# humansensinglab/AGenDA

Measured on AMD Instinct MI355X. Metric: 512x512 images/sec + DAAM heatmaps, 50 DDIM steps, SD-1.5, higher is better.
Workload: dtype bf16

## Files before the change

### agenda_amd/_lib.py

```python
from __future__ import annotations

import ctypes as C
import os

_HERE = os.path.dirname(os.path.abspath(__file__))
LIB_PATH = os.environ.get("AGD_LIB") or os.path.join(_HERE, "libagenda_hip.so")
AGD_MAX_LEVELS = 8
AGD_N_CLASSES = 11


class AgdConfig(C.Structure):
    _fields_ = [
        ("struct_size", C.c_int),
        ("in_channels", C.c_int), ("out_channels", C.c_int), ("n_levels", C.c_int),
        ("block_out_channels", C.c_int * AGD_MAX_LEVELS),
        ("down_cross", C.c_int * AGD_MAX_LEVELS),
        ("num_heads", C.c_int * AGD_MAX_LEVELS),
        ("layers_per_block", C.c_int), ("cross_attention_dim", C.c_int),
        ("use_linear_projection", C.c_int), ("norm_num_groups", C.c_int),
        ("vae_latent_channels", C.c_int), ("vae_out_channels", C.c_int), ("vae_n_levels", C.c_int),
        ("vae_block_out_channels", C.c_int * AGD_MAX_LEVELS),
        ("vae_layers_per_block", C.c_int), ("vae_norm_num_groups", C.c_int),
        ("vae_scaling_factor", C.c_float),
        ("max_tokens", C.c_int),
# ... 135 lines not shown
    "agd_cfg_ddim_step": (C.c_int, [_P, _P, _P, C.c_int, C.c_int, C.c_float, C.c_float, C.c_float, _P]),
    "agd_denoise": (C.c_int, [_P, _P, C.c_int, C.c_int, C.c_int, C.POINTER(C.c_float), C.POINTER(C.c_float),
                              C.POINTER(C.c_float), C.c_float, _P]),
    "agd_denoise_plms": (C.c_int, [_P, _P, C.c_int, C.c_int, C.c_int, C.POINTER(C.c_float), C.POINTER(C.c_float),
                                   C.POINTER(C.c_float), C.c_float, _P]),
    "agd_denoise_dpm": (C.c_int, [_P, _P, C.c_int, C.c_int, C.c_int, C.POINTER(C.c_float), C.POINTER(C.c_float), C.c_float, _P]),
    "agd_vae_decode": (C.c_int, [_P, _P, C.c_int, C.c_int, _P, _P, _P]),
    "agd_vae_encode": (C.c_int, [_P, _P, C.c_int, C.c_int, _P, _P, _P]),
    "agd_safety_scores_hw": (C.c_int, [_P, _P, C.c_int, C.c_int, C.c_int, _P, _P, _P]),
    "agd_controlnet_set_cond_hw": (C.c_int, [_P, _P, C.c_int, C.c_int, C.c_int, C.c_int, _P]),
    "agd_controlnet_residuals_hw": (C.c_int, [_P, _P, C.c_int, C.c_int, C.c_int, C.c_float, C.c_float, C.c_int, _P, C.POINTER(C.c_longlong), _P]),
    "agd_inpaint_prepare_hw": (C.c_int, [_P, _P, C.c_int, _P, C.c_int, C.c_int, C.c_int, C.c_int, _P, _P, _P, _P]),
    "agd_inpaint_set_hw": (C.c_int, [_P, _P, C.c_int, _P, C.c_int, _P, C.c_int, C.c_int, C.c_int, _P]),
    "agd_unet_forward_hw": (C.c_int, [_P, _P, C.c_int, C.c_int, C.c_int, C.c_float, _P, _P]),
    "agd_unet_forward_ts_hw": (C.c_int, [_P, _P, C.c_int, C.c_int, C.c_int, C.POINTER(C.c_float), _P, _P]),
    "agd_cfg_ddim_step_hw": (C.c_int, [_P, _P, _P, C.c_int, C.c_int, C.c_int, C.c_float, C.c_float, C.c_float, _P]),
    "agd_denoise_hw": (C.c_int, [_P, _P, C.c_int, C.c_int, C.c_int, C.c_int, C.POINTER(C.c_float), C.POINTER(C.c_float),
                                 C.POINTER(C.c_float), C.c_float, _P]),
    "agd_denoise_plms_hw": (C.c_int, [_P, _P, C.c_int, C.c_int, C.c_int, C.c_int, C.POINTER(C.c_float), C.POINTER(C.c_float),
                                      C.POINTER(C.c_float), C.c_float, _P]),
    "agd_denoise_dpm_hw": (C.c_int, [_P, _P, C.c_int, C.c_int, C.c_int, C.c_int, C.POINTER(C.c_float), C.POINTER(C.c_float), C.c_float, _P]),
    "agd_vae_decode_hw": (C.c_int, [_P, _P, C.c_int, C.c_int, C.c_int, _P, _P, _P]),
    "agd_vae_encode_hw": (C.c_int, [_P, _P, C.c_int, C.c_int, C.c_int, _P, _P, _P]),
    "agd_record_reset_hw": (C.c_int, [_P, C.c_int, C.c_int, C.c_int, _P]),
    "agd_set_option": (C.c_int, [_P, C.c_char_p, C.c_int]),
    "agd_record_config": (C.c_int, [_P, C.c_int, C.c_int, C.c_int]),
    "agd_record_reset": (C.c_int, [_P, C.c_int, C.c_int, _P]),
    "agd_daam_global": (C.c_int, [_P, C.c_int, C.c_int, _P, _P]),
    "agd_hook_global": (C.c_int, [_P, _P, _P]),
    "agd_hook_count": (C.c_int, [_P]),
    "agd_hook_last_map": (C.c_int, [_P, _P, C.c_int, _P]),
    "agd_cross_attn": (C.c_int, [_P, C.c_char_p, _P, _P, C.c_int, C.c_int, C.c_int, _P, C.c_int, _P]),
    "agd_attn_processor": (C.c_int, [_P, C.c_char_p, _P, _P, _P, C.c_int, C.c_int, C.c_int, _P, C.c_int, _P]),
    "agd_hook_reset": (C.c_int, [_P, C.c_int, C.c_int, _P]),
    "agd_hook_num_maps": (C.c_int, [_P]),
    "agd_hook_map_dims": (C.c_int, [_P, C.c_int, C.POINTER(C.c_int)]),
    "agd_hook_map": (C.c_int, [_P, C.c_int, _P, _P]),
    "agd_op_attn_reg_loss": (C.c_int, [_P, C.c_int, C.c_int, C.c_int, _P, _P, _P, C.c_float, _P, _P, _P]),
    "agd_attn_processor_backward": (C.c_int, [_P, C.c_char_p, _P, _P, _P, _P, C.c_int, C.c_int, C.c_int, C.c_int, _P, _P, _P]),
    "agd_op_conv2d": (C.c_int, [_P, _P, _P, _P] + [C.c_int] * 9 + [_P]),
    "agd_op_conv2d_ex": (C.c_int, [_P, _P, _P, _P] + [C.c_int] * 10 + [_P]),
    "agd_op_linear": (C.c_int, [_P, _P, _P, _P, _P, C.c_int, C.c_int, C.c_int, C.c_int, _P]),
    "agd_op_groupnorm": (C.c_int, [_P, _P, _P, _P, C.c_int, C.c_int, C.c_int, C.c_int, C.c_float, C.c_int, _P]),
    "agd_op_groupnorm_ex": (C.c_int, [_P] * 5 + [C.c_int] * 5 + [C.c_float, C.c_int, _P, C.c_int, _P, C.c_int, C.POINTER(C.c_int), _P]),
    "agd_op_gn_fold": (C.c_int, [_P, _P] + [C.c_int] * 5 + [C.c_float] + [_P] * 4 + [C.c_int, C.c_int] + [_P] * 5 + [_P]),
    "agd_op_conv_groupnorm": (C.c_int, [_P] * 6 + [C.c_int] * 6 + [C.c_float, C.c_int, C.c_int, _P]),
    "agd_op_igemm": (C.c_int, [C.POINTER(AgdIgemmDesc), _P]),
    "agd_op_layernorm": (C.c_int, [_P, _P, _P, _P, C.c_int, C.c_int, C.c_float, _P]),
    "agd_op_layernorm_ex": (C.c_int, [_P, _P, _P, _P, C.c_int, C.c_int, C.c_float, C.POINTER(C.c_int), _P]),
    "agd_op_ff_fused": (C.c_int, [_P] * 8 + [C.c_int, C.c_int, C.c_float, _P]),
    "agd_op_attn_chain": (C.c_int, [_P] * 9 + [C.c_int] * 5 + [C.c_float, _P]),
    "agd_op_ff_fused_ex": (C.c_int, [_P] * 8 + [C.c_int, C.c_int, C.c_float, _P, _P, _P, C.c_int, _P, C.c_int, _P, C.c_int, _P]),
    "agd_op_attn_chain_ex": (C.c_int, [_P] * 8 + [C.c_int] * 5 + [C.c_float] + [_P] * 4 + [C.c_int, _P, _P] + [C.c_int] * 6 + [_P]),
    "agd_op_qkv_chain": (C.c_int, [_P] * 3 + [C.c_int, C.c_float, _P, C.c_int] + [_P] * 4 + [C.c_float] + [_P] * 3 + [C.c_int] * 4 + [_P]),
    "agd_op_xattn_premul": (C.c_int, [_P] * 9 + [C.c_int] * 5 + [C.c_float, _P]),
    "agd_op_attention": (C.c_int, [_P, _P, _P, _P, C.c_int, C.c_int, C.c_int, C.c_int, C.c_int, C.c_float, _P, _P]),
    "agd_op_attention_ex": (C.c_int, [_P, _P, _P, _P] + [C.c_int] * 5 + [C.c_float, C.c_int, _P, _P, _P, C.c_int, C.c_int, _P, C.c_int, C.c_int, C.c_int, _P]),
    "agd_op_attention_long": (C.c_int, [_P, _P, _P, _P] + [C.c_int] * 5 + [C.c_float, C.c_int, _P, C.c_int, C.c_int, _P]),
    "agd_op_attention_headsum": (C.c_int, [_P, _P, _P, _P, C.c_int, C.c_int, C.c_int, C.c_int, C.c_int, C.c_float, _P, _P]),
    "agd_op_attention_backward": (C.c_int, [_P, _P, _P, _P] + [C.c_int] * 6 + [C.c_float, _P, _P, _P]),
    "agd_op_hook_headmean": (C.c_int, [_P, C.c_int, C.c_int, C.c_int, C.c_int, _P, _P]),
    "agd_op_bicubic_clamp_mean": (C.c_int, [_P, C.c_int, C.c_int, C.c_int, C.c_int, _P, _P]),
    "agd_op_heatmap_u8": (C.c_int, [_P, C.c_int, C.c_int, _P, _P]),
    "agd_op_resize_u8_pil": (C.c_int, [_P, C.c_int, C.c_int, C.c_int, C.c_int, C.c_int, C.c_int, _P, _P]),
    "agd_op_stack_heatmaps": (C.c_int, [_P, _P, _P, C.c_longlong, _P, _P, _P]),
    "agd_op_window_gather": (C.c_int, [_P, _P] + [C.c_int] * 8 + [_P]),
    "agd_op_window_mean": (C.c_int, [_P, _P] + [C.c_int] * 6 + [_P]),
    "agd_denoise_panorama": (C.c_int, [_P, _P] + [C.c_int] * 7 + [C.POINTER(C.c_float)] * 3 + [C.c_float, _P]),
    "agd_daam_global_panorama": (C.c_int, [_P, C.c_int, C.c_int, _P, _P]),
    "agd_op_region_masks": (C.c_int, [_P, C.c_int, C.c_int, _P] + [C.c_int] * 6 + [_P]),
    "agd_op_region_spread": (C.c_int, [_P] * 5 + [C.c_int] * 6 + [C.POINTER(C.c_int), C.c_float, C.c_float, _P]),
    "agd_op_region_mean": (C.c_int, [_P, _P, _P] + [C.c_int] * 5 + [_P]),
    "agd_denoise_regions": (C.c_int, [_P, _P, C.c_int, C.c_int, C.c_int, C.POINTER(AgdRegionsDesc), C.c_int] + [C.POINTER(C.c_float)] * 3 + [C.c_float, _P]),
    "agd_freeu_set": (C.c_int, [_P] + [C.c_float] * 4),
    "agd_freeu_clear": (C.c_int, [_P]),
    "agd_freeu_counts": (C.c_int, [_P, C.POINTER(C.c_longlong)]),
    "agd_op_freeu": (C.c_int, [_P, _P, _P, _P] + [C.c_int] * 5 + [C.c_float, C.c_float, _P]),
    "agd_guidance_rescale_set": (C.c_int, [_P, C.c_float]),
    "agd_guidance_rescale_clear": (C.c_int, [_P]),
    "agd_guidance_rescale_counts": (C.c_int, [_P, C.POINTER(C.c_longlong)]),
    "agd_op_guidance_rescale": (C.c_int, [_P, _P] + [C.c_int] * 4 + [C.c_float, C.c_float, _P, _P]),
    "agd_pag_set": (C.c_int, [_P, C.POINTER(C.c_float), C.c_int, C.POINTER(C.c_char_p), C.c_int]),
    "agd_pag_clear": (C.c_int, [_P]),
    "agd_pag_counts": (C.c_int, [_P, C.POINTER(C.c_longlong), C.POINTER(C.c_longlong)]),
    "agd_op_pag_v_rows": (C.c_int, [_P, _P, _P, C.c_int, C.c_int, _P]),
    "agd_op_pag_fold": (C.c_int, [_P, _P, C.c_longlong, C.c_float, _P]),
    "agd_sega_set": (C.c_int, [_P, C.POINTER(AgdSegaDesc)]),
    "agd_sega_clear": (C.c_int, [_P]),
    "agd_sega_counts": (C.c_int, [_P, C.POINTER(C.c_longlong), C.POINTER(C.c_longlong)]),
    "agd_op_sega_threshold": (C.c_int, [_P, _P, C.c_int, C.c_int, C.c_int, C.POINTER(C.c_float), C.POINTER(C.c_double), _P, _P]),
    "agd_op_sega_fold": (C.c_int, [_P, _P, _P, _P, C.c_int, C.c_int, C.c_int, C.POINTER(C.c_float), C.POINTER(C.c_float), C.POINTER(C.c_float),
                                   C.c_float, C.c_float, C.c_float, _P]),
    "agd_deepcache_set": (C.c_int, [_P, C.POINTER(C.c_int), C.c_int, C.c_int]),
    "agd_deepcache_clear": (C.c_int, [_P]),
    "agd_deepcache_counts": (C.c_int, [_P, C.POINTER(C.c_longlong)]),
    "agd_deepcache_forward_hw": (C.c_int, [_P, _P, C.c_int, C.c_int, C.c_int, C.c_float, C.c_int, C.c_int, _P, _P]),
    "agd_op_deepcache_capture": (C.c_int, [_P, _P, _P, C.c_longlong, _P, _P, C.c_longlong, _P]),
    "agd_profile_begin": (C.c_int, [_P]),
    "agd_profile_end": (C.c_int, [_P, C.POINTER(C.c_double), C.POINTER(C.c_double), C.POINTER(C.c_longlong)]),
    "agd_profile_end_ex": (C.c_int, [_P, C.c_double, C.c_double] + [C.POINTER(C.c_double)] * 5 + [C.POINTER(C.c_longlong)]),
    "agd_profile_class_name": (C.c_char_p, [C.c_int]),
    "agd_version": (C.c_char_p, []),
}

EXPORTS = tuple(_SIGS.keys())
_lib = None
# ... 36 lines not shown
```

### agenda_amd/csrc/kernels.h

```cpp
#pragma once
#include "common.h"
#include "../../include/agenda_hip.h"

#define AGD_MAX_DEVICES 16
struct SplitKWs { float* p = nullptr; size_t cap = 0; };

struct IgemmP {
  const bf16_t* sc0 = nullptr; const bf16_t* sc1 = nullptr; int sc_C0 = 0, sc_C1 = 0;
  int ups4 = 0;
  const bf16_t* src0; const bf16_t* src1;
  int C0, C1;
  int Hin, Win, Hout, Wout;
  int ksize, stride, pad, up;
  const bf16_t* W;
  const float* bias; int bias_mode;
  const float* rowadd; int rowadd_ld;
  const bf16_t* residual; int ldr;
  void* out; int out_f32; int ldo;
  int M, N, K;
  float alpha;
  int geglu;
  int act;
  int batch;
  long long sA0, sA1, sW, sO, sR;
// ... 20 lines not shown
  int pc;
  int stagger;
  int dbg;
  int* ran;
};
enum { IGEMM_RAN_NONE = 0, IGEMM_RAN_GENERAL = 1, IGEMM_RAN_HALO = 2, IGEMM_RAN_PCH = 3, IGEMM_RAN_PC = 4, IGEMM_RAN_8P = 5, IGEMM_RAN_SMAP = 6, IGEMM_RAN_WREG = 7 };
enum { IGEMM_SLAB_NONE = 0, IGEMM_SLAB_PLAIN = 1, IGEMM_SLAB_GN = 2 };
int launch_igemm(const IgemmP& p, hipStream_t st);
int igemm_query(const IgemmP& p, int* cfg3);

struct AttnP {
  const bf16_t* q; const bf16_t* k; const bf16_t* v; bf16_t* o;
  int ldq, ldk, ldv, ldo;
  long long sq, sk, sv, so;
  int B, H, D, Nq, Nk;
  float scale;
  int record_mode; int rec_b0;
  float* rec; long long rec_img_stride; long long rec_head_stride;
  int rec_T;
  int rec_hpb;
  int nqt;
  int causal;
  const float* mask;
  const bf16_t* k2; const bf16_t* v2; int ldk2, ldv2; long long sk2, sv2; int Nk2;
};
int launch_attention(const AttnP& p, hipStream_t st);
constexpr int ATTN_LONG_MAX_KEYS = 320;
int launch_attention_long(const AttnP& p, hipStream_t st);

struct FFusedP {
  const bf16_t* h; bf16_t* out;
  const bf16_t* w1f;
  const float* cs1; const float* b1;
  const bf16_t* w2f;
  const float* b2;
  int M; float ln_eps;
  const bf16_t* wpf; const float* bp; const bf16_t* xres; bf16_t* pout; float* colstat;
  int xres_rows;
  int premul;
};
int launch_ff_fused(const FFusedP& p, int C, hipStream_t st);
struct AttnChainP {
  const bf16_t* h; bf16_t* out;
  const float* gamma; const float* beta; float ln_eps;
  const bf16_t* wqf;
  const bf16_t* wof; const float* bo;
  const bf16_t* kv; int ldkv; long long skv;
  int M, HW, T; float scale;
  int record; float* rec; long long rec_img_stride, rec_head_stride; int rec_T, rec_b0, rec_hpb;
  float* rowstat_out;
  const bf16_t* o1; const bf16_t* wo1f; const float* bo1;
  int rows32;
  int src_rows;
};
int launch_attn_chain(const AttnChainP& p, int C, int heads, hipStream_t st);
struct QkvChainP {
  const bf16_t* x;
  const bf16_t* wbf; long long wb_stride; const float* rowadd;
  bf16_t* h;
  const float* gamma; const float* beta; float ln_eps;
  const bf16_t* wqkvf;
  bf16_t* qkv;
  int M, HW;
  long long rowadd_stride;
  const float* gn_part; int gn_bm, gn_groups; float gn_eps; const float* gn_gamma; const float* gn_beta;
  int rows64;
  int sched2;
};
int launch_qkv_chain(const QkvChainP& p, int C, hipStream_t st);
int launch_frag_order_w1(const bf16_t* src, bf16_t* dst, int C, int HID, hipStream_t st);
int launch_frag_order_w(const bf16_t* src, bf16_t* dst, int N, int K, int NI, int KC, hipStream_t st);

#define XATTN_TP 80
struct XattnPremulP {
  const bf16_t* kv; int ldkv; long long skv;
  const bf16_t* wqT;
  const bf16_t* wo;
  const float* gamma; const float* wqb;
  int B, T, C, H; float scale;
  bf16_t* kpp; float* kcs; float* kbs; bf16_t* vpp;
};
int launch_xattn_premul(const XattnPremulP& p, hipStream_t st);
struct XattnSP {
  const bf16_t* x;
  const float* ln_stats; int ln_slots; float ln_invC, ln_eps;
  const bf16_t* kpp; const float* kcs; const float* kbs;
  bf16_t* P;
  int M, HW, C, H, T;
  float* rec; long long rec_img_stride, rec_head_stride; int rec_T, rec_b0;
};
int launch_xattn_s(const XattnSP& p, hipStream_t st);
int launch_matvec_bf16(const bf16_t* W, const float* v, float* out, int N, int K, hipStream_t st);
int launch_rowstat_bf16(const bf16_t* x, float* out, int M, int C, hipStream_t st);

struct GroupNormP {
  const bf16_t* x0; const bf16_t* x1; int C0, C1;
  bf16_t* y;
  const float* gamma; const float* beta;
  int B, HW, groups; float eps; int silu;
  float* ws;
  const float* part0; const float* part1; int bm0, bm1;
  int* path;
};
int groupnorm_check(int B, int C0, int C1, int HW, int groups);
int layernorm_check(int rows, int C);
int launch_groupnorm(const GroupNormP& p, hipStream_t st);
int launch_gn_fold_weight(const float* part, int bm, int B, int HW, int C, int groups, float eps, const float* gamma, const float* beta,
                          const bf16_t* W, const float* bias, int N, bf16_t* Wb, float* rowadd, hipStream_t st, int frag_ni = 0);
// ... 129 lines not shown
```

### agenda_amd/csrc/model.hip

```cpp
#include "../../include/agenda_hip.h"
#include "kernels.h"

#include <algorithm>
#include <cmath>
#include <cstdarg>
#include <cstdio>
#include <cstring>
#include <functional>
#include <string>
#include <unordered_map>
#include <unordered_set>
#include <vector>

static thread_local char g_err[2048] = "";
#define AGD_API extern "C" __attribute__((visibility("default")))
extern "C" void agd_set_error(const char* fmt, ...) {
  va_list ap; va_start(ap, fmt); vsnprintf(g_err, sizeof(g_err), fmt, ap); va_end(ap);
}
#define CK(expr) do { if ((expr) != 0) return -1; } while (0)
#define FAIL(...) do { agd_set_error(__VA_ARGS__); return -1; } while (0)

struct WMat { bf16_t* w = nullptr; int N = 0, Cin = 0, Cpad = 0, taps = 0;
              int sc_cols = 0;
              bf16_t* wfrag = nullptr; int wfrag_ni = 0; };
struct Act { bf16_t* p = nullptr; int B = 0, H = 0, W = 0, C = 0; float* cpart = nullptr; int cpart_bm = 0;
             bf16_t* normed = nullptr; const float* normed_gamma = nullptr;
             long long n() const { return (long long)B * H * W * C; } };
struct NextGn { const float* gamma = nullptr; const float* beta = nullptr; float eps = 0.f; int silu = 0; };

struct Arena {
  char* base = nullptr; size_t cap = 0, off = 0, peak = 0;
  void* alloc(size_t bytes) {
    size_t a = (off + 255) & ~(size_t)255;
    if (a + bytes > cap) { agd_set_error("activation arena exhausted: need %zu + %zu > %zu bytes (raise workspace_bytes)", a, bytes, cap); return nullptr; }
    off = a + bytes; if (off > peak) peak = off;
    return base + a;
  }
  size_t mark() const { return off; }
  void release(size_t m) { off = m; }
};

enum { PC_CONV3 = 0, PC_GEMM, PC_ATTN_SELF, PC_ATTN_CROSS, PC_GN, PC_LN, PC_ELEM, PC_HEAT, PC_VAE_ATTN, PC_OTHER, PC_TOUCH };
static const char* kClassNames[AGD_N_CLASSES] = {"igemm_conv3x3", "igemm_linear_1x1", "attn_self_flash", "attn_cross_daam",
                                                 "groupnorm", "layernorm", "elementwise", "heatmap", "vae_attn_softmax", "other", "weight_touch"};

struct DBuf {
  void* p = nullptr; size_t cap = 0;
  template <typename T> T* as() const { return (T*)p; }
  int ensure(size_t bytes) {
    if (p && bytes <= cap) return 0;
    if (p) { (void)hipDeviceSynchronize(); (void)hipFree(p); p = nullptr; cap = 0; }
    const size_t want = bytes ? bytes : 256;
    if (hipMalloc(&p, want) != hipSuccess) { p = nullptr; agd_set_error("hipMalloc(%zu) failed", want); return -1; }
    cap = want;
    return 0;
  }
  void release() { if (p) (void)hipFree(p); p = nullptr; cap = 0; }
};

struct XLayer {
  std::string name; int C = 0, heads = 0, level = 0; bool mid = false;
  bool cn = false;
  WMat wkv; DBuf kvb; bf16_t* kv = nullptr; DBuf accb; float* acc = nullptr; int acc_h = 0, acc_w = 0;
  int acc_heads = 0;
  DBuf wqTb, wkvTb, woTb; WMat wqT, wkvT, woT;
  bf16_t* pm_wqT = nullptr; float* pm_wqb = nullptr; bool pm_ready = false;
  DBuf pm_kppb, pm_vppb, pm_csb; bf16_t* pm_kpp = nullptr; bf16_t* pm_vpp = nullptr; float* pm_kcs = nullptr; float* pm_kbs = nullptr;
};

struct Fuser {
  std::string pre; int C = 0, heads = 0;
  WMat wqkv, wkv; float ta = 0.f, td = 0.f; float* bo_s = nullptr; float* b2_s = nullptr;
  DBuf gkvb;
};

struct IpaLayer {
  std::string pre; int C = 0, heads = 0, cols = 0;
  DBuf wk, wv, kppb, vppb, csbsb;
};

enum : int {
  TBF_FF            = 1 << 0,
  TBF_ATTN2         = 1 << 1,
  TBF_ATTN1_OUT     = 1 << 2,
  TBF_FF_PROJ       = 1 << 3,
  TBF_QKV           = 1 << 4,
  TBF_ATTN2_640     = 1 << 5,
  TBF_LAZY_DUP      = 1 << 6,
  TBF_QKV_GN        = 1 << 7,
  TBF_QKV_640       = 1 << 8,
  TBF_FF_PREMUL     = 1 << 9,
  TBF_ATTN2_ROWS32  = 1 << 10,
  TBF_QKV_ROWS64    = 1 << 11,
  TBF_QKV_SCHED2    = 1 << 12,
  TBF_DEFAULT       = 0x1fff & ~TBF_QKV_640,
};

struct ProfEv { int cls; double flops, bytes; hipEvent_t a, b; };

struct EvalCond {
  float cn_scale = 0.f;
  bool grounded = false;
  float ad_scale = 0.f;
  bool ipa = false;
  bool pag = false;
  int dc = 0;
  int dc_branch = 0;
};
enum : int { DC_CAPTURE = 1, DC_SHALLOW = 2 };

struct agd_ctx {
  int device = 0; agd_config cfg{}; std::string err;
  std::unordered_map<std::string, WMat> W;
  std::unordered_map<std::string, float*> V;
  std::unordered_map<std::string, int> Vn;
  std::vector<void*> owned;
  Arena arena; bf16_t* zero_page = nullptr;
  float* stage = nullptr; size_t stage_bytes = 0;
  bool finalized = false;
  WMat tproj_all; float* tproj_bias = nullptr; float* tproj_out = nullptr; int tproj_total = 0;
  const float* tproj_cur = nullptr;
  int tproj_cur_ld = 0;
  float* tsteps_buf = nullptr; int tsteps_cap = 0;
  std::unordered_map<std::string, int> tproj_off;
  float* temb_buf = nullptr;
  float* t_dev = nullptr;
  std::vector<XLayer> xl; std::unordered_map<std::string, int> xl_idx;
  DBuf ctxb; bf16_t* ctx_bf16 = nullptr; int ctx_B2 = 0, ctx_T = 0;
  int rec_mode = 0, rec_is_train = 0, rec_T_cfg = 0, rec_T = 0, rec_B = 0, rec_L = 0, rec_Lh = 0, rec_Lw = 0;
  DBuf hook_sumb, hook_scratchb, hook_headsb, hook_storeb;
  struct HookRec { size_t off; int Bp, T, N; };
  std::vector<HookRec> hook_recs; size_t hook_store_used = 0;
  DBuf bwd_wsb;
  float* hook_sum = nullptr; float* hook_scratch = nullptr; int hook_count = 0, hook_Bp = 0, hook_T = 0;
  int rec_base = 0, rec_call = 0;
  int pano_B = 0, pano_Lh = 0, pano_Lw = 0, pano_stride = 0;
  DBuf pano_ctxb;
  DBuf reg_xb;
  DBuf pano_viewb, pano_hmb;
  DBuf latb, epsb, vae_imgb, plmsb, dpmb;
  bf16_t* lat_bf16 = nullptr; float* eps_nhwc = nullptr;
  SplitKWs splitk;
  int opt_cfg_share = 1;
  int opt_ln_fold = 1;
  int opt_gn_fused = 1;
  int opt_warm = 3;
  int opt_gn_proj_fold = 1;
  int opt_p8 = 1;
// ... 402 lines not shown
  if (B != c->gl_B2) FAIL("gligen: the grounding objects are set for %d rows, this forward has %d (agd_gligen_set)", c->gl_B2, B);
  const std::string t = f.pre + "transformer_blocks.0.fuser.";
  bf16_t* n = (bf16_t*)c->arena.alloc((size_t)M * C * 2); bf16_t* ff = (bf16_t*)c->arena.alloc((size_t)M * 4 * C * 2);
  if (!n || !ff) return -1;
  GETV(g1, t + "norm1.weight"); GETV(b1, t + "norm1.bias"); GETV(g2, t + "norm2.weight"); GETV(b2, t + "norm2.bias");
  GETW(wo, t + "attn.to_out.0.weight"); GETW(w1, t + "ff.net.0.proj.weight"); GETV(bb1, t + "ff.net.0.proj.bias"); GETW(w2, t + "ff.net.2.weight");
  { ProfScope ps(c, st, PC_LN, 0, 4.0 * M * (double)C); CK(launch_layernorm(h, n, g1, b1, M, C, 1e-5f, st)); }
  { GemmOpt o; CK(run_conv(c, st, n, C, nullptr, 0, 1, 1, M, f.wqkv, 1, qkv, o, c->zero_page)); }
  AttnP a{}; a.q = qkv; a.k = qkv + C; a.v = qkv + 2 * C; a.o = att;
  a.ldq = a.ldk = a.ldv = 3 * C; a.ldo = C; a.sq = a.sk = a.sv = (long long)HW * 3 * C; a.so = (long long)HW * C;
  a.B = B; a.H = f.heads; a.D = D; a.Nq = HW; a.Nk = HW; a.scale = 1.0f / sqrtf((float)D);
  a.k2 = f.gkvb.as<bf16_t>(); a.v2 = a.k2 + C; a.ldk2 = a.ldv2 = 2 * C; a.sk2 = a.sv2 = (long long)NO * 2 * C; a.Nk2 = NO;
  { const double fl = 4.0 * B * f.heads * (double)HW * (HW + NO) * D, by = 2.0 * B * (double)C * (4.0 * HW + 2.0 * NO);
    ProfScope ps(c, st, PC_ATTN_SELF, fl, by); CK(launch_attention(a, st)); }
  { GemmOpt o; o.bias = f.bo_s; o.alpha = f.ta; o.residual = h; CK(run_conv(c, st, att, C, nullptr, 0, 1, 1, M, *wo, 1, h, o, c->zero_page)); }
  { ProfScope ps(c, st, PC_LN, 0, 4.0 * M * (double)C); CK(launch_layernorm(h, n, g2, b2, M, C, 1e-5f, st)); }
  { GemmOpt o; o.bias = bb1; o.geglu = 1; CK(run_conv(c, st, n, C, nullptr, 0, 1, 1, M, *w1, 1, ff, o, c->zero_page)); }
  GemmOpt o; o.bias = f.b2_s; o.alpha = f.td; o.residual = h;
  return last(ff, 4 * C, *w2, o);
}

static int dup_half(agd_ctx* c, hipStream_t st, bf16_t* p, long long half_elems) {
  ProfScope ps(c, st, PC_ELEM, 0);
  if (hipMemcpyAsync(p + half_elems, p, (size_t)half_elems * 2, hipMemcpyDeviceToDevice, st) != hipSuccess) FAIL("dup_half copy failed");
  return 0;
}

enum TbHead  { HEAD_GN,
               HEAD_FOLD,
               HEAD_QKV,
               HEAD_QKV_GN };
enum TbDup   { DUP_NONE, DUP_COPY,
               DUP_LAZY };
enum TbAttn2 { ATTN2_CHAIN,
               ATTN2_PREMUL,
               ATTN2_KERNELS };
enum TbFf    { FF_FUSED,
               FF_FUSED_PROJ,
               FF_FUSED_PREMUL,
               FF_FFPROJ,
               FF_PLAIN };

struct TBlockPlan {
  bool fold;
  bool x_normed;
  bool gfold;
  TbHead head; int qkv_rows64, qkv_sched2;
  bool attn1_in_chain;
  TbDup dup;
  const Fuser* fuser;
  const IpaLayer* ipa;
  XLayer* xl;
  TbAttn2 attn2; int chain_rows32;
  bool daam;
  TbFf ff;
  bool wreg_proj;
  bool stats_head, stats_attn1, stats_attn2;
  bool stats_ipa;
};

static const float kTbLnEps = 1e-5f;

struct TBlock {
  agd_ctx* c; hipStream_t st; const std::string& pre; const std::string t; const Act& x; Act& out; int heads, groups;
  int C, HW, Bs, B;
  const float* gn_g = nullptr; const float* gn_b = nullptr; const WMat* w_in = nullptr; const float* b_in = nullptr;
  bf16_t* ln = nullptr;
  bf16_t* h = nullptr; bf16_t* qkv = nullptr; bf16_t* att = nullptr;
  const bf16_t* xres;
  int M; const int Mshared;
  float* stats = nullptr; int slots = 0;
  bf16_t* ipaP = nullptr;
  TBlock(agd_ctx* c_, hipStream_t st_, const std::string& pre_, const Act& x_, Act& out_, int heads_, int groups_, int dup)
    : c(c_), st(st_), pre(pre_), t(pre_ + "transformer_blocks.0."), x(x_), out(out_), heads(heads_), groups(groups_), C(x_.C), HW(x_.H * x_.W),
      Bs(x_.B), B(dup ? 2 * x_.B : x_.B), xres(x_.p), M(x_.B * x_.H * x_.W), Mshared(M) {}

  int produce(const bf16_t* A, int K, const WMat& w, GemmOpt o, bool shaped, bool want_stats) {
    const int gb_ = shaped ? M / HW : 1, gh_ = shaped ? x.H : 1, gw_ = shaped ? x.W : M;
    stats = nullptr; slots = 0;
    if (want_stats) {
      int cfg[3] = {0, 0, 0}; GemmOpt qo = o; qo.query_cfg = cfg; qo.want_rowstat = 1;
      CK(run_conv(c, st, A, K, nullptr, 0, gb_, gh_, gw_, w, 1, h, qo, c->zero_page));
      slots = (w.N + cfg[1] - 1) / cfg[1];
      stats = (float*)c->arena.alloc((size_t)B * HW * slots * 2 * sizeof(float)); if (!stats) return -1;
      o.rowstat_out = stats; o.rowstat_slots = slots;
    }
    return run_conv(c, st, A, K, nullptr, 0, gb_, gh_, gw_, w, 1, h, o, c->zero_page);
  }
  int consume(bool fold, const std::string& lnkey, const std::string& wkey, const float* bias, int geglu, bf16_t* outp) {
    if (fold) {
      const std::string k = wkey + ".lnfold";
      GETW(wf, k); GETV(cs, k + ".cs"); GETV(bf, k + ".bias");
      GemmOpt o; o.bias = bf; o.geglu = geglu; o.ln_stats = stats; o.ln_slots = slots; o.ln_cs = cs; o.ln_invC = 1.0f / (float)C; o.ln_eps = kTbLnEps;
      if (geglu && C == 1280 && M >= 1024 && M <= 4096 && (c->opt_wreg & 1) && wf->wfrag) o.wreg = 2;
      return run_conv(c, st, h, C, nullptr, 0, 1, 1, M, *wf, 1, outp, o, c->zero_page);
    }
    GETV(g, lnkey + ".weight"); GETV(b, lnkey + ".bias");
    { ProfScope ps(c, st, PC_LN, 0, 4.0 * M * (double)C); CK(launch_layernorm(h, ln, g, b, M, C, kTbLnEps, st)); }
    GETW(w, wkey); GemmOpt o; o.bias = bias; o.geglu = geglu;
    return run_conv(c, st, ln, C, nullptr, 0, 1, 1, M, *w, 1, outp, o, c->zero_page);
  }
};

static TBlockPlan tblock_plan(const TBlock& s, int dup) {
  agd_ctx* c = s.c; const Act& x = s.x; const std::string& pre = s.pre; const std::string& t = s.t;
  const int C = s.C, HW = s.HW, heads = s.heads, groups = s.groups;
  auto tb = [c](int bit) { return (c->opt_tb_fuse & bit) != 0; };
  auto has = [c](const std::string& key) { return c->W.count(key) != 0; };
  TBlockPlan p{};
  p.fold = c->opt_ln_fold == 1 || (c->opt_ln_fold == 2 && C <= 320) || (c->opt_ln_fold == 3 && C <= 640);
  p.x_normed = x.normed && x.normed_gamma == s.gn_g;
  p.wreg_proj = C == 640 && (c->opt_wreg & 2);
  const bool sums = c->opt_gn_fused && x.cpart && x.cpart_bm > 0 && HW % x.cpart_bm == 0;
  p.gfold = c->opt_gn_proj_fold && sums && C <= (c->opt_gn_proj_fold >= 2 ? 640 : 320) && HW % 128 == 0;
  if (p.gfold) {
    const bool qkv = tb(TBF_QKV) && C == 320 && s.w_in->N == C && has(t + "attn1.qkv.frag");
    const bool gn_inside = qkv && tb(TBF_QKV_GN) && groups <= 32 && has(pre + "proj_in.frag");
    p.head = gn_inside ? HEAD_QKV_GN : qkv ? HEAD_QKV : HEAD_FOLD;
    p.qkv_rows64 = qkv && tb(TBF_QKV_ROWS64) && HW % 64 == 0;
  } else if (C == 640 && tb(TBF_QKV) && tb(TBF_QKV_640) && tb(TBF_QKV_GN) && sums && HW % 64 == 0 && groups <= 32 && !p.x_normed && !dup &&
             has(pre + "proj_in.frag") && has(t + "attn1.qkv.frag")) {
    p.head = HEAD_QKV_GN;
  } else p.head = HEAD_GN;
  p.qkv_sched2 = tb(TBF_QKV_SCHED2);
  const bool ff_fused = tb(TBF_FF) && p.fold && C == 320 && has(t + "ff.w1.frag");
  if (ff_fused) {
    const bool proj = tb(TBF_FF_PROJ) && has(pre + "proj_out.frag");
    p.ff = !proj ? FF_FUSED : tb(TBF_FF_PREMUL) && has(t + "ff.w2p.frag") ? FF_FUSED_PREMUL : FF_FUSED_PROJ;
  } else p.ff = c->opt_ffproj && has(pre + "ffproj.weight") ? FF_FFPROJ : FF_PLAIN;
  auto itx = c->xl_idx.find(t + "attn2");
  p.xl = itx == c->xl_idx.end() ? nullptr : &c->xl[itx->second];
  p.daam = p.xl && daam_records(c, *p.xl, s.B, x.H, x.W);
  const bool premul = p.xl && p.xl->pm_ready && c->opt_xpre && p.fold && HW % 64 == 0 && c->rec_mode != 2 && c->ctx_T <= XATTN_TP && !dup &&
                      (!p.daam || p.xl->acc_heads == p.xl->heads);
  const bool chain = !premul && tb(TBF_ATTN2) && (C == 320 || (C == 640 && tb(TBF_ATTN2_640))) && heads == 8 && HW % (C == 320 ? 128 : 64) == 0 &&
                     c->ctx_T <= 96 && c->rec_mode != 2 && has(t + "attn2.to_q.frag");
  p.attn2 = premul ? ATTN2_PREMUL : chain ? ATTN2_CHAIN : ATTN2_KERNELS;
  p.chain_rows32 = tb(TBF_ATTN2_ROWS32);
  if (c->cur.grounded) { auto itf = c->gl_idx.find(pre); if (itf != c->gl_idx.end()) p.fuser = &c->gl_f[itf->second]; }
  if (c->cur.ipa) { auto iti = c->ipa_idx.find(pre); if (iti != c->ipa_idx.end()) p.ipa = &c->ipa_l[iti->second]; }
  const bool lazy = dup && tb(TBF_LAZY_DUP) && chain && C == 320 && (p.ff == FF_FUSED_PROJ || p.ff == FF_FUSED_PREMUL) && !p.fuser && !p.ipa;
  p.dup = !dup ? DUP_NONE : lazy ? DUP_LAZY : DUP_COPY;
  p.attn1_in_chain = chain && tb(TBF_ATTN1_OUT) && p.dup != DUP_COPY && has(t + "attn1.to_out.frag") && !p.fuser && !p.ipa;
  p.stats_head = p.fold; p.stats_attn1 = p.fold && !chain; p.stats_attn2 = p.fold && !ff_fused && !p.ipa; p.stats_ipa = p.fold && !ff_fused && p.ipa;
  return p;
}

static int qkv_chain_params(const TBlock& s, const TBlockPlan& p, const bf16_t* wb, const float* radd, QkvChainP& qp) {
  agd_ctx* c = s.c; const Act& x = s.x; const int C = s.C;
  GETW(fqkv, s.t + "attn1.qkv.frag"); GETV(g1, s.t + "norm1.weight"); GETV(b1, s.t + "norm1.bias");
  qp.x = x.p; qp.wbf = wb; qp.wb_stride = (long long)s.w_in->N * C; qp.rowadd = radd; qp.rowadd_stride = C; qp.h = s.h; qp.gamma = g1; qp.beta = b1; qp.ln_eps = kTbLnEps;
  qp.wqkvf = fqkv->w; qp.qkv = s.qkv; qp.M = s.M; qp.HW = s.HW; qp.rows64 = p.qkv_rows64; qp.sched2 = p.qkv_sched2;
  if (p.head == HEAD_QKV_GN) {
    GETW(fpi, s.pre + "proj_in.frag");
    if (!s.b_in) FAIL("proj_in without bias");
    qp.wbf = fpi->w; qp.wb_stride = 0; qp.rowadd = s.b_in; qp.rowadd_stride = 0;
    qp.gn_part = x.cpart; qp.gn_bm = x.cpart_bm; qp.gn_groups = s.groups; qp.gn_eps = 1e-6f; qp.gn_gamma = s.gn_g; qp.gn_beta = s.gn_b;
  }
  return 0;
}

static int tb_head(TBlock& s, const TBlockPlan& p) {
  agd_ctx* c = s.c; hipStream_t st = s.st; const Act& x = s.x; const WMat* w = s.w_in; const int C = s.C;
  if (p.head == HEAD_GN) {
    if (p.x_normed) s.ln = x.normed;
    else CK(run_gn(c, st, x.p, C, nullptr, 0, s.Bs, s.HW, s.gn_g, s.gn_b, s.groups, 1e-6f, 0, s.ln, &x));
    GemmOpt o; o.bias = s.b_in;
    if (p.wreg_proj) o.wreg = 1;
    return s.produce(s.ln, C, *w, o, false, p.stats_head);
  }
  if (p.gfold) { if (w->taps != 1 || w->Cpad != C) FAIL("gn_proj_fold: proj_in weight [N=%d taps=%d Cpad=%d] is not a 1x1 over %d channels", w->N, w->taps, w->Cpad, C); }
  else if (w->taps != 1 || w->Cpad != C || w->N != C || !s.b_in) FAIL("qkv chain: proj_in weight [N=%d taps=%d Cpad=%d] is not a biased 1x1 over %d channels", w->N, w->taps, w->Cpad, C);
  bf16_t* wb = nullptr; float* radd = nullptr;
  if (p.head != HEAD_QKV_GN) {
    wb = (bf16_t*)c->arena.alloc((size_t)s.Bs * w->N * C * 2);
    radd = (float*)c->arena.alloc((size_t)s.Bs * w->N * sizeof(float));
    if (!wb || !radd) return -1;
    ProfScope ps(c, st, PC_GN, 0, 2.0 * s.Bs * (double)w->N * C * 2);
    CK(launch_gn_fold_weight(x.cpart, x.cpart_bm, s.Bs, s.HW, C, s.groups, 1e-6f, s.gn_g, s.gn_b, w->w, s.b_in, w->N, wb, radd, st, p.head == HEAD_QKV ? C / 64 : 0));
  }
  if (p.head == HEAD_FOLD) {
    WMat wi = *w; wi.w = wb;
    GemmOpt o; o.rowadd = radd; o.rowadd_ld = w->N; o.w_per_image = 1;
    return s.produce(x.p, C, wi, o, true, p.stats_head);
  }
  QkvChainP qp{}; CK(qkv_chain_params(s, p, wb, radd, qp));
  s.stats = nullptr; s.slots = 0;
  ProfScope ps(c, st, PC_GEMM, 8.0 * s.M * (double)C * C, 2.0 * s.M * (double)C * 5.0 + 2.0 * (p.gfold ? s.Bs + 3.0 : 4.0) * C * (double)C);
  return launch_qkv_chain(qp, C, st);
}

// ... 43 lines not shown
  const double M = (double)B * HW;
  ProfScope ps(c, st, PC_ATTN_CROSS, 2.0 * M * l.cols * l.C, 2.0 * M * l.C + 2.0 * B * (double)l.cols * l.C + 2.0 * M * l.cols);
  return launch_ipa_scores(sp, st);
}
static int ipa_add_rows(agd_ctx* c, hipStream_t st, const IpaLayer& l, bf16_t* h, int B, int HW, const bf16_t* P) {
  IpaAddP ap{}; ap.h = h; ap.P = P; ap.vpp = l.vppb.as<bf16_t>(); ap.B = B; ap.HW = HW; ap.C = l.C; ap.colsP = l.cols; ap.s = c->ipa_scale;
  const double M = (double)B * HW;
  ProfScope ps(c, st, PC_ATTN_CROSS, 2.0 * M * l.cols * l.C, 4.0 * M * l.C + 2.0 * B * (double)l.cols * l.C + 2.0 * M * l.cols);
  return launch_ipa_add(ap, st);
}
static int tb_ip_adapter_scores(TBlock& s, const TBlockPlan& p) {
  agd_ctx* c = s.c;
  if (s.C != p.ipa->C) FAIL("ip_adapter: %s has %d channels, its to_k_ip / to_v_ip were loaded for %d", s.pre.c_str(), s.C, p.ipa->C);
  s.ipaP = (bf16_t*)c->arena.alloc((size_t)s.M * p.ipa->cols * 2); if (!s.ipaP) return -1;
  CK(ipa_scores_rows(c, s.st, *p.ipa, s.h, s.B, s.HW, s.ipaP));
  c->ipa_counts[0]++;
  return 0;
}
static int tb_ip_adapter_add(TBlock& s, const TBlockPlan& p) {
  agd_ctx* c = s.c;
  CK(ipa_add_rows(c, s.st, *p.ipa, s.h, s.B, s.HW, s.ipaP));
  c->ipa_counts[1]++;
  if (p.stats_ipa) {
    s.slots = 1; s.stats = (float*)c->arena.alloc((size_t)s.M * 2 * sizeof(float)); if (!s.stats) return -1;
    ProfScope ps(c, s.st, PC_LN, 0, 2.0 * s.M * (double)s.C);
    CK(launch_rowstat_bf16(s.h, s.stats, s.M, s.C, s.st));
  }
  return 0;
}

static int tb_attn2_chain(TBlock& s, const TBlockPlan& p) {
  agd_ctx* c = s.c; const std::string& t = s.t; const XLayer& xl = *p.xl; const int C = s.C, HW = s.HW, B = s.B, M = s.M, heads = s.heads;
  GETW(fq, t + "attn2.to_q.frag"); GETW(fo, t + "attn2.to_out.frag");
  GETV(g2, t + "norm2.weight"); GETV(b2, t + "norm2.bias"); GETV(bo, t + "attn2.to_out.0.bias");
  const int T = c->ctx_T, D = C / heads;
  AttnChainP ap{}; ap.h = s.h; ap.out = s.h; ap.gamma = g2; ap.beta = b2; ap.ln_eps = kTbLnEps; ap.wqf = fq->w; ap.wof = fo->w; ap.bo = bo;
  ap.kv = xl.kv; ap.ldkv = 2 * C; ap.skv = (long long)T * 2 * C; ap.M = M; ap.HW = HW; ap.T = T; ap.scale = 1.0f / sqrtf((float)D);
  double rec_bytes = 0;
  if (p.daam) {
    ap.record = 1; ap.rec_b0 = B / 2; ap.rec_T = c->rec_T; ap.rec_hpb = heads / xl.acc_heads;
    ap.rec_head_stride = (long long)c->rec_T * HW; ap.rec_img_stride = ap.rec_head_stride * xl.acc_heads;
    ap.rec = xl.acc + (size_t)c->rec_base * ap.rec_img_stride;
    rec_bytes = 8.0 * (B - ap.rec_b0) * xl.acc_heads * (double)c->rec_T * HW;
  }
  if (p.attn1_in_chain || p.dup == DUP_LAZY) {
    ap.out = (bf16_t*)c->arena.alloc((size_t)M * C * 2); if (!ap.out) return -1;
  }
  if (p.attn1_in_chain) {
    GETW(f1o, t + "attn1.to_out.frag"); GETV(bo1, t + "attn1.to_out.0.bias");
    ap.o1 = s.att; ap.wo1f = f1o->w; ap.bo1 = bo1;
  }
  if (p.dup == DUP_LAZY) ap.src_rows = s.Mshared;
  ap.rows32 = p.chain_rows32;
  if (p.stats_attn2) {
    s.slots = 1; s.stats = (float*)c->arena.alloc((size_t)M * 2 * sizeof(float)); if (!s.stats) return -1;
    ap.rowstat_out = s.stats;
  }
  const double gemms = p.attn1_in_chain ? 6.0 : 4.0;
  ProfScope ps(c, s.st, PC_ATTN_CROSS, gemms * M * (double)C * C + 4.0 * B * heads * (double)HW * T * D, gemms * M * (double)C + gemms * C * (double)C + 4.0 * B * (double)T * C + rec_bytes);
  CK(launch_attn_chain(ap, C, heads, s.st));
  s.h = ap.out;
  return 0;
}

static int tb_attn2_premul(TBlock& s, const TBlockPlan& p) {
  agd_ctx* c = s.c; const XLayer& xl = *p.xl; const int C = s.C, HW = s.HW, B = s.B, M = s.M, heads = s.heads;
  if (!s.stats || s.slots <= 0) FAIL("attn2_premul: the GEMM in front of attn2 left no row statistics for norm2");
  GETV(bo, s.t + "attn2.to_out.0.bias");
  const int HT = heads * XATTN_TP;
  bf16_t* P = (bf16_t*)c->arena.alloc((size_t)M * HT * 2); if (!P) return -1;
  XattnSP sp{}; sp.x = s.h; sp.ln_stats = s.stats; sp.ln_slots = s.slots; sp.ln_invC = 1.0f / (float)C; sp.ln_eps = kTbLnEps;
  sp.kpp = xl.pm_kpp; sp.kcs = xl.pm_kcs; sp.kbs = xl.pm_kbs; sp.P = P; sp.M = M; sp.HW = HW; sp.C = C; sp.H = heads; sp.T = c->ctx_T;
  double rec_bytes = 0;
  if (p.daam) {
    sp.rec_b0 = B / 2; sp.rec_T = c->rec_T; sp.rec_head_stride = (long long)c->rec_T * HW; sp.rec_img_stride = sp.rec_head_stride * xl.acc_heads;
    sp.rec = xl.acc + (size_t)c->rec_base * sp.rec_img_stride;
    rec_bytes = 8.0 * (B - sp.rec_b0) * heads * (double)c->rec_T * HW;
  }
  { ProfScope ps(c, s.st, PC_ATTN_CROSS, 2.0 * M * (double)HT * C, 2.0 * M * (double)C + 2.0 * B * (double)HT * C + 2.0 * M * (double)HT + rec_bytes);
    CK(launch_xattn_s(sp, s.st)); }
  WMat wv; wv.w = xl.pm_vpp; wv.N = C; wv.Cin = HT; wv.Cpad = HT; wv.taps = 1;
  GemmOpt oo; oo.bias = bo; oo.residual = s.h; oo.w_per_image = 1;
  return s.produce(P, HT, wv, oo, true, p.stats_attn2);
}

static int tb_attn2(TBlock& s, const TBlockPlan& p) {
  agd_ctx* c = s.c; const std::string& t = s.t;
  if (!p.xl) FAIL("cross-attn layer %s not registered", (t + "attn2").c_str());
  if (c->ctx_B2 != s.B) FAIL("context batch %d != unet batch %d (call agd_set_context)", c->ctx_B2, s.B);
  if (p.attn2 == ATTN2_CHAIN) return tb_attn2_chain(s, p);
  if (p.attn2 == ATTN2_PREMUL) return tb_attn2_premul(s, p);
  CK(s.consume(p.fold, t + "norm2", t + "attn2.to_q.weight", nullptr, 0, s.qkv));
  CK(cross_attention(c, s.st, *p.xl, s.qkv, s.B, s.HW, s.x.H, s.x.W, s.att, true));
  GETW(wo, t + "attn2.to_out.0.weight"); GETV(bo, t + "attn2.to_out.0.bias");
  GemmOpt oo; oo.bias = bo; oo.residual = s.h;
  return s.produce(s.att, s.C, *wo, oo, false, p.stats_attn2);
}

static int tb_ff_fused(TBlock& s, const TBlockPlan& p) {
  agd_ctx* c = s.c; const std::string& t = s.t; Act& out = s.out; const int C = s.C, M = s.M;
  GETW(f1, t + "ff.w1.frag"); GETW(f2, t + "ff.w2.frag");
  const std::string k = t + "ff.net.0.proj.weight.lnfold";
  GETV(cs, k + ".cs"); GETV(bf, k + ".bias"); GETV(b2, t + "ff.net.2.bias");
  FFusedP fp{}; fp.h = s.h; fp.out = s.h; fp.w1f = f1->w; fp.cs1 = cs; fp.b1 = bf; fp.w2f = f2->w; fp.b2 = b2; fp.M = M; fp.ln_eps = kTbLnEps;
  const bool proj = p.ff != FF_FUSED;
  if (proj) {
// ... 427 lines not shown
      const std::string k = v + "encoder.down_blocks." + std::to_string(i) + ".downsamplers.0.conv.";
      GETW(w, k + "weight"); GETV(b, k + "bias");
      Act d = alloc_act(c, B, h.H / 2, h.W / 2, co, true); if (!d.p) return -1;
      GemmOpt o; o.bias = b; o.stride = 2; o.pad = 0; o.hout = h.H / 2; o.wout = h.W / 2; o.out_act = &d;
      CK(run_conv(c, st, h.p, co, nullptr, 0, B, h.H, h.W, *w, 3, d.p, o, c->zero_page));
      h = d;
    }
  }
  const int top = g.vae_block_out_channels[nl - 1], Lh = h.H, Lw = h.W;
  { Act r; CK(resnet(c, st, v + "encoder.mid_block.resnets.0.", h, nullptr, top, 1e-6f, false, G, r)); h = r; }
  CK(vae_mid_attention(c, st, v + "encoder.mid_block.attentions.0.", G, B, Lh, Lw, top, h));
  { Act r; CK(resnet(c, st, v + "encoder.mid_block.resnets.1.", h, nullptr, top, 1e-6f, false, G, r)); h = r; }
  Act n = alloc_act(c, B, Lh, Lw, top); if (!n.p) return -1;
  GETV(gg, v + "encoder.conv_norm_out.weight"); GETV(gb, v + "encoder.conv_norm_out.bias");
  CK(run_gn(c, st, h.p, top, nullptr, 0, B, Lh * Lw, gg, gb, G, 1e-6f, 1, n.p, &h));
  bf16_t* co64 = (bf16_t*)c->arena.alloc((size_t)B * Lh * Lw * 64 * 2); if (!co64) return -1;
  if (hipMemsetAsync(co64, 0, (size_t)B * Lh * Lw * 64 * 2, st) != hipSuccess) FAIL("memset enc");
  { GETW(w, v + "encoder.conv_out.weight"); GETV(b, v + "encoder.conv_out.bias"); GemmOpt o; o.bias = b; o.ldo = 64;
    CK(run_conv(c, st, n.p, top, nullptr, 0, B, Lh, Lw, *w, 3, co64, o, c->zero_page)); }
  { GETW(w, v + "quant_conv.weight"); GETV(b, v + "quant_conv.bias"); GemmOpt o; o.bias = b; o.out_f32 = 1; o.ldo = 2 * lc;
    CK(run_conv(c, st, co64, 64, nullptr, 0, B, Lh, Lw, *w, 1, moments, o, c->zero_page)); }
  return 0;
}

AGD_API const char* agd_version(void) { return "agenda_hip 0.1 (gfx950)"; }
AGD_API const char* agd_last_error(agd_ctx* c) { return (c && !c->err.empty()) ? c->err.c_str() : g_err; }
AGD_API const char* agd_profile_class_name(int cls) { return (cls >= 0 && cls < AGD_N_CLASSES) ? kClassNames[cls] : ""; }

AGD_API agd_ctx* agd_create(int device_id, const agd_config* cfg) {
  if (!cfg || cfg->struct_size != (int)sizeof(agd_config)) { agd_set_error("agd_create: bad config (struct_size %d != %zu)", cfg ? cfg->struct_size : -1, sizeof(agd_config)); return nullptr; }
  if (cfg->n_levels < 1 || cfg->n_levels > AGD_MAX_LEVELS || cfg->vae_n_levels < 1 || cfg->vae_n_levels > AGD_MAX_LEVELS) { agd_set_error("agd_create: bad level count"); return nullptr; }
  for (int i = 0; i < cfg->n_levels; ++i)
    if (cfg->block_out_channels[i] % 64) { agd_set_error("agd_create: UNet channels must be multiples of 64"); return nullptr; }
  for (int i = 0; i < cfg->vae_n_levels; ++i)
    if (cfg->vae_block_out_channels[i] % 64) { agd_set_error("agd_create: VAE channels must be multiples of 64"); return nullptr; }
  if (cfg->cross_attention_dim % 64) { agd_set_error("agd_create: cross_attention_dim must be a multiple of 64"); return nullptr; }
  if (hipSetDevice(device_id) != hipSuccess) { agd_set_error("hipSetDevice(%d) failed", device_id); return nullptr; }
  agd_ctx* c = new agd_ctx(); c->device = device_id; c->cfg = *cfg;
  const size_t ws = cfg->workspace_bytes > 0 ? (size_t)cfg->workspace_bytes : ((size_t)8 << 30);
  if (hipMalloc((void**)&c->arena.base, ws) != hipSuccess) { agd_set_error("arena hipMalloc(%zu) failed", ws); delete c; return nullptr; }
  c->arena.cap = ws;
  c->zero_page = dmalloc<bf16_t>(c, 2048);
  c->t_dev = dmalloc<float>(c, 64);
  if (!c->zero_page || !c->t_dev) { delete c; return nullptr; }
  hipMemset(c->zero_page, 0, 4096);
  return c;
}

AGD_API void agd_destroy(agd_ctx* c) {
  if (!c) return;
  hipSetDevice(c->device);
  hipDeviceSynchronize();
  for (void* p : c->owned) hipFree(p);
  for (auto& xl : c->xl) { xl.kvb.release(); xl.accb.release(); }
  c->pano_viewb.release(); c->pano_hmb.release(); c->reg_xb.release(); c->pano_ctxb.release(); c->i2_latb.release();
  c->ctxb.release(); c->hook_sumb.release(); c->hook_scratchb.release(); c->hook_headsb.release(); c->hook_storeb.release(); c->bwd_wsb.release();
  for (auto& xl : c->xl) { xl.wqTb.release(); xl.wkvTb.release(); xl.woTb.release(); xl.pm_kppb.release(); xl.pm_vppb.release(); xl.pm_csb.release(); }
  c->latb.release(); c->epsb.release(); c->vae_imgb.release(); c->plmsb.release(); c->dpmb.release(); c->gr_factb.release(); c->sega_momb.release(); c->sega_thrb.release(); c->dc_buf.release(); c->cn_embb.release(); c->lora_descb.release();
  for (auto& f : c->gl_f) f.gkvb.release();
  c->gl_objb.release();
  for (auto& b : c->ad_featb) b.release();
  ipa_release(c);
  if (c->side) { hipStreamDestroy(c->side); hipEventDestroy(c->ev_fork); hipEventDestroy(c->ev_join); }
  if (c->splitk.p) hipFree(c->splitk.p);
  if (c->arena.base) hipFree(c->arena.base);
  if (c->stage) hipFree(c->stage);
  if (c->tsteps_buf) hipFree(c->tsteps_buf);
  for (auto e : c->ev_pool) hipEventDestroy(e);
  delete c;
}

static bool ends_with(const std::string& s, const char* suf) { const size_t n = strlen(suf); return s.size() >= n && s.compare(s.size() - n, n, suf) == 0; }

AGD_API int agd_load_tensor(agd_ctx* c, const char* name, const void* ptr, int dtype, int ndim, const long long* shape) {
  if (!c || !name || !ptr || !shape) { agd_set_error("agd_load_tensor: null argument"); return fail_ctx(c); }
  if (dtype != 0) { agd_set_error("agd_load_tensor: only float32 (dtype 0) supported"); return fail_ctx(c); }
  hipSetDevice(c->device);
  long long n = 1; for (int i = 0; i < ndim; ++i) n *= shape[i];
  const size_t bytes = (size_t)n * 4;
  if (bytes > c->stage_bytes) {
    if (c->stage) hipFree(c->stage);
    if (hipMalloc((void**)&c->stage, bytes) != hipSuccess) { c->stage = nullptr; c->stage_bytes = 0; agd_set_error("stage alloc failed"); return fail_ctx(c); }
    c->stage_bytes = bytes;
  }
  if (hipMemcpy(c->stage, ptr, bytes, hipMemcpyDefault) != hipSuccess) { agd_set_error("copy of '%s' failed", name); return fail_ctx(c); }
  const std::string k(name);
  if (k.compare(0, 11, "controlnet.") == 0 && !c->cn_on) { agd_set_error("'%s': call agd_controlnet_configure before loading ControlNet weights", name); return fail_ctx(c); }
  if (k.compare(0, 8, "adapter.") == 0 && !c->ad_on) { agd_set_error("'%s': call agd_adapter_configure before loading T2I-Adapter weights", name); return fail_ctx(c); }
  if ((k.compare(0, 18, "unet.position_net.") == 0 || k.find(".fuser.") != std::string::npos) && !c->gl_on) {
    agd_set_error("'%s': call agd_gligen_configure before loading GLIGEN weights", name); return fail_ctx(c); }
  const bool vis_f32 = (k.compare(0, 7, "safety.") == 0 || k.compare(0, 14, "image_encoder.") == 0) && !(ndim == 2 && k.find(".encoder.layers.") != std::string::npos);
  if (ndim == 1 || vis_f32 || (ndim == 0 && c->gl_on)) {
    float* d = dmalloc<float>(c, (size_t)n); if (!d) return fail_ctx(c);
    hipMemcpy(d, c->stage, bytes, hipMemcpyDeviceToDevice);
    c->V[k] = d; c->Vn[k] = (int)n;
  } else if (ndim == 2 || ndim == 4) {
    WMat w; w.N = (int)shape[0]; w.Cin = (int)shape[1]; w.taps = ndim == 4 ? (int)(shape[2] * shape[3]) : 1;
    if (w.taps != 1 && w.taps != 9) { agd_set_error("'%s': only 1x1 / 3x3 kernels", name); return fail_ctx(c); }
    w.Cpad = (w.Cin + 63) / 64 * 64;
    const bool is_tok_emb = ends_with(k, "token_embedding.weight");
    w.w = dmalloc<bf16_t>(c, (size_t)(w.N + (is_tok_emb ? kTextExtraRows : 0)) * w.taps * w.Cpad); if (!w.w) return fail_ctx(c);
    if (is_tok_emb) hipMemset(w.w + (size_t)w.N * w.Cpad, 0, (size_t)kTextExtraRows * w.Cpad * 2);
    const int geglu_bn = ends_with(k, "ff.net.0.proj.weight") ? 16 : 0;
    if (geglu_bn && (w.N % 256)) { agd_set_error("'%s': GEGLU projection rows %d not a multiple of 256", name, w.N); return fail_ctx(c); }
    API_CK(c, launch_convert_weight(c->stage, w.w, w.N, w.Cin, w.taps, w.Cpad, geglu_bn, 0));
    hipDeviceSynchronize();
    c->W[k] = w;
// ... 452 lines not shown
    if (cn && !c->cn_on) break;
    WMat& all = cn ? c->cn_tproj_all : c->tproj_all; float*& bias = cn ? c->cn_tproj_bias : c->tproj_bias;
    float*& out = cn ? c->cn_tproj_out : c->tproj_out; int& total_out = cn ? c->cn_tproj_total : c->tproj_total;
    std::vector<const WMat*> parts; std::vector<std::string> pres; int total = 0;
    for (auto& kv : c->W)
      if (ends_with(kv.first, "time_emb_proj.weight") && (kv.first.compare(0, 11, "controlnet.") == 0) == cn) pres.push_back(kv.first.substr(0, kv.first.size() - strlen("time_emb_proj.weight")));
    std::sort(pres.begin(), pres.end());
    for (auto& p : pres) { const WMat* w = getW(c, p + "time_emb_proj.weight"); parts.push_back(w); c->tproj_off[p] = total; total += w->N; }
    if (!parts.empty()) {
      API_CK(c, concat_rows(c, parts, all)); total_out = total;
      bias = dmalloc<float>(c, total); out = dmalloc<float>(c, total);
      if (!bias || !out) return fail_ctx(c);
      for (auto& p : pres) { const float* b = getV(c, p + "time_emb_proj.bias"); if (!b) return fail_ctx(c);
        hipMemcpy(bias + c->tproj_off[p], b, (size_t)c->Vn[p + "time_emb_proj.bias"] * 4, hipMemcpyDeviceToDevice); }
    } else if (cn) { agd_set_error("finalize: the ControlNet has no time_emb_proj weights"); return fail_ctx(c); }
  }
  { const int dim = g.block_out_channels[0];
    c->temb_buf = dmalloc<float>(c, (size_t)dim * 9); if (!c->temb_buf) return fail_ctx(c); }
  API_CK(c, fuse_clip_qkv(c, "text.encoder.layers.", g.text_layers));
  if (c->vis_on) API_CK(c, finalize_safety(c));
  if (c->cn_on) API_CK(c, finalize_controlnet(c));
  if (c->gl_on) API_CK(c, finalize_gligen(c));
  if (c->ad_on) API_CK(c, finalize_adapter(c));
  hipDeviceSynchronize();
  c->finalized = true;
  return 0;
}

static hipStream_t S(void* s) { return (hipStream_t)s; }
static int need_final(agd_ctx* c) { if (!c) { agd_set_error("null ctx"); return -1; } if (!c->finalized) { agd_set_error("agd_finalize not called"); return -1; } hipSetDevice(c->device); return 0; }

static int project_context(agd_ctx* c, hipStream_t st, int batch2, int tokens);
AGD_API int agd_set_context(agd_ctx* c, const float* ctx_emb, int batch2, int tokens, void* stream) {
  API_CK(c, need_final(c));
  hipStream_t st = S(stream);
  const int Dc = c->cfg.cross_attention_dim;
  if (tokens > AGD_MAX_CONTEXT_TOKENS) { agd_set_error("set_context: tokens %d > %d unsupported", tokens, AGD_MAX_CONTEXT_TOKENS); return fail_ctx(c); }
  if (batch2 < 1 || tokens < 1) { agd_set_error("set_context: batch2 %d tokens %d", batch2, tokens); return fail_ctx(c); }
  API_CK(c, c->ctxb.ensure((size_t)batch2 * tokens * Dc * 2)); c->ctx_bf16 = c->ctxb.as<bf16_t>();
  for (auto& xl : c->xl) { API_CK(c, xl.kvb.ensure((size_t)batch2 * tokens * 2 * xl.C * 2)); xl.kv = xl.kvb.as<bf16_t>(); }
  c->ctx_B2 = batch2; c->ctx_T = tokens;
  deepcache_invalidate(c);
  API_CK(c, launch_f32_to_bf16(ctx_emb, c->ctx_bf16, (long long)batch2 * tokens * Dc, st));
  API_CK(c, project_context(c, st, batch2, tokens));
  return 0;
}
static int project_context(agd_ctx* c, hipStream_t st, int batch2, int tokens) {
  const int Dc = c->cfg.cross_attention_dim;
  for (auto& xl : c->xl) { API_CK(c, xl.kvb.ensure((size_t)batch2 * tokens * 2 * xl.C * 2)); xl.kv = xl.kvb.as<bf16_t>(); }
  c->ctx_B2 = batch2; c->ctx_T = tokens;
  for (auto& xl : c->xl) {
    GemmOpt o;
    API_CK(c, run_conv(c, st, c->ctx_bf16, Dc, nullptr, 0, 1, 1, batch2 * tokens, xl.wkv, 1, xl.kv, o, c->zero_page));
    xl.pm_ready = false;
    if (c->opt_xpre && xl.pm_wqT && tokens <= XATTN_TP && ((c->opt_xpre & 2) || xl.heads * XATTN_TP * 2 <= xl.C)) {
      const std::string t = xl.name.substr(0, xl.name.size() - 5);
      const WMat* wo2 = getW(c, t + "attn2.to_out.0.weight"); const float* g2 = getV(c, t + "norm2.weight");
      if (!wo2 || !g2) { agd_set_error("%s: pre-multiplied form without attn2.to_out.0.weight / norm2.weight", xl.name.c_str()); return fail_ctx(c); }
      const size_t HT = (size_t)xl.heads * XATTN_TP;
      API_CK(c, xl.pm_kppb.ensure((size_t)batch2 * HT * xl.C * 2)); API_CK(c, xl.pm_vppb.ensure((size_t)batch2 * HT * xl.C * 2)); API_CK(c, xl.pm_csb.ensure((size_t)batch2 * HT * 2 * sizeof(float)));
      xl.pm_kpp = xl.pm_kppb.as<bf16_t>(); xl.pm_vpp = xl.pm_vppb.as<bf16_t>(); xl.pm_kcs = xl.pm_csb.as<float>(); xl.pm_kbs = xl.pm_kcs + (size_t)batch2 * HT;
      XattnPremulP pm{}; pm.kv = xl.kv; pm.ldkv = 2 * xl.C; pm.skv = (long long)tokens * 2 * xl.C; pm.wqT = xl.pm_wqT; pm.wo = wo2->w; pm.gamma = g2; pm.wqb = xl.pm_wqb;
      pm.B = batch2; pm.T = tokens; pm.C = xl.C; pm.H = xl.heads; pm.scale = 1.0f / sqrtf((float)(xl.C / xl.heads));
      pm.kpp = xl.pm_kpp; pm.kcs = xl.pm_kcs; pm.kbs = xl.pm_kbs; pm.vpp = xl.pm_vpp;
      { ProfScope ps(c, st, PC_ATTN_CROSS, 8.0 * batch2 * (double)HT * xl.C * (xl.C / xl.heads) / 2.0, 4.0 * batch2 * (double)HT * xl.C);
        API_CK(c, launch_xattn_premul(pm, st)); }
      xl.pm_ready = true;
    }
  }
  c->ctx_stale = false;
  return 0;
}

static int ensure_lat(agd_ctx* c, int B2, int Lh, int Lw) {
  const size_t need = (size_t)B2 * Lh * Lw * 64;
  const int oc = c->cfg.out_channels > 4 ? c->cfg.out_channels : 4;
  CK(c->latb.ensure(need * 2)); CK(c->epsb.ensure((size_t)B2 * Lh * Lw * oc * 4));
  c->lat_bf16 = c->latb.as<bf16_t>(); c->eps_nhwc = c->epsb.as<float>();
  return 0;
}

static int embed_all_timesteps(agd_ctx* c, hipStream_t st, const float* timesteps, int n, const float** out);
struct CallCond {
  const float* cn = nullptr; const int* gl = nullptr; const float* ad = nullptr; const float* blend = nullptr; bool ipa = false;
  const float* pag = nullptr;
  const int* dc = nullptr; int dc_n = 0, dc_b = 0;
  bool sega = false;
  EvalCond at(int i) const {
    EvalCond e; e.cn_scale = cn ? cn[i] : 0.f; e.grounded = gl && gl[i]; e.ad_scale = ad ? ad[i] : 0.f; e.ipa = ipa;
    if (dc) { e.dc = !dc[i] ? DC_SHALLOW : (i + 1 < dc_n && !dc[i + 1]) ? DC_CAPTURE : 0; e.dc_branch = dc_b; }
    return e;
  }
};
enum Caller { CALL_UNET_FORWARD, CALL_UNET_FORWARD_TS, CALL_EVAL_LOOP, CALL_IP2P_LOOP, CALL_PANORAMA, CALL_DC_FORWARD, CALL_REGIONS };
enum CondState { ST_CN, ST_GL, ST_INP, ST_I2P, ST_AD, ST_IPA, ST_PAG, ST_DC, ST_SEGA, N_COND_STATES };
struct ConflictRow { int self; unsigned callers; const char* with[N_COND_STATES]; };
static const ConflictRow kConflicts[] = {
  { ST_INP, 1u << CALL_EVAL_LOOP, {
    "inpaint: a ControlNet schedule is set; ControlNet inpainting is not implemented", nullptr, nullptr, nullptr, nullptr, nullptr } },
  { ST_I2P, 1u << CALL_IP2P_LOOP, {
    "ip2p: a ControlNet schedule is set; ControlNet with InstructPix2Pix is not implemented (clear it first)",
    "ip2p: a GLIGEN schedule is set; GLIGEN with InstructPix2Pix is not implemented (clear it first)",
    "ip2p: an inpainting state is set; inpainting with InstructPix2Pix is not implemented (agd_inpaint_clear first)",
    nullptr,
    "ip2p: a T2I-Adapter schedule is set; the T2I-Adapter with InstructPix2Pix is not implemented (clear it first)",
    "ip2p: an IP-Adapter image is set; ip2p runs without it (agd_ip_adapter_clear first)" } },
// ... 1281 lines not shown
AGD_API int agd_op_layernorm(const float* x, const float* gamma, const float* beta, float* y, int rows, int C, float eps, void* stream) {
  return agd_op_layernorm_ex(x, gamma, beta, y, rows, C, eps, nullptr, stream);
}

AGD_API int agd_op_ff_fused(const float* x, const float* gamma, const float* beta, const float* w1, const float* b1, const float* w2,
                            const float* b2, float* y, int M, int C, float eps, void* stream) {
  return agd_op_ff_fused_ex(x, gamma, beta, w1, b1, w2, b2, y, M, C, eps, nullptr, nullptr, nullptr, 0, nullptr, 0, nullptr, 0, stream);
}
AGD_API int agd_op_ff_fused_ex(const float* x, const float* gamma, const float* beta, const float* w1, const float* b1, const float* w2,
                               const float* b2, float* y, int M, int C, float eps, const float* wp, const float* bp, const float* xres,
                               int xres_rows, float* pout, int premul, float* colstat, int inplace, void* stream) {
  hipStream_t st = S(stream); Tmp tmp;
  if (C != 320) { agd_set_error("op_ff_fused: C = %d (320 only)", C); return -1; }
  if (M < 1 || xres_rows < 0 || !x || !gamma || !beta || !w1 || !b1 || !w2 || !b2 || (!wp && !y)) { agd_set_error("op_ff_fused: bad arguments (M %d xres_rows %d)", M, xres_rows); return -1; }
  if (colstat && !wp) { agd_set_error("op_ff_fused: colstat belongs to the proj_out stage"); return -1; }
  const int H8 = 8 * C, H4 = 4 * C;
  const long long xr_rows = xres_rows > 0 ? xres_rows : M;
  bf16_t* xb = tmp.get<bf16_t>((size_t)M * C); bf16_t* yb = tmp.get<bf16_t>((size_t)M * C);
  bf16_t* w1b = tmp.get<bf16_t>((size_t)H8 * C); bf16_t* w1l = tmp.get<bf16_t>((size_t)H8 * C); bf16_t* w1f = tmp.get<bf16_t>((size_t)H8 * C);
  bf16_t* w2b = tmp.get<bf16_t>((size_t)C * H4); bf16_t* w2f = tmp.get<bf16_t>((size_t)C * H4);
  float* cs = tmp.get<float>(H8); float* bf = tmp.get<float>(H8);
  if (!xb || !yb || !w1b || !w1l || !w1f || !w2b || !w2f || !cs || !bf) return -1;
  CK(launch_f32_to_bf16(x, xb, (long long)M * C, st));
  CK(launch_convert_weight(w1, w1b, H8, C, 1, C, 16, st));
  CK(launch_ln_fold_weight(w1b, gamma, beta, b1, H8, C, 16, w1l, cs, bf, st));
  CK(launch_frag_order_w1(w1l, w1f, C, H4, st));
  CK(launch_convert_weight(w2, w2b, C, H4, 1, H4, 0, st));
  CK(launch_frag_order_w(w2b, w2f, C, H4, C / 64, 128, st));
  FFusedP fp{}; fp.h = xb; fp.out = inplace ? xb : yb; fp.w1f = w1f; fp.cs1 = cs; fp.b1 = bf; fp.w2f = w2f; fp.b2 = b2; fp.M = M; fp.ln_eps = eps;
  bf16_t* pb = nullptr;
  fp.premul = premul ? 1 : 0; fp.xres_rows = xres_rows; fp.colstat = colstat; fp.bp = bp;
  if (wp) {
    bf16_t* wpb = tmp.get<bf16_t>((size_t)C * C); bf16_t* wpf = tmp.get<bf16_t>((size_t)C * C); pb = tmp.get<bf16_t>((size_t)M * C);
    if (!wpb || !wpf || !pb) return -1;
    CK(launch_convert_weight(wp, wpb, C, C, 1, C, 0, st));
    CK(launch_frag_order_w(wpb, wpf, C, C, C / 64, C, st));
    fp.wpf = wpf; fp.pout = pout ? pb : nullptr;
    if (xres) {
      bf16_t* xrb = tmp.get<bf16_t>((size_t)xr_rows * C); if (!xrb) return -1;
      CK(launch_f32_to_bf16(xres, xrb, xr_rows * C, st));
      fp.xres = xrb;
    }
  }
  CK(launch_ff_fused(fp, C, st));
  if (wp) CK(launch_bf16_to_f32(pb, pout, (long long)M * C, st));
  else CK(launch_bf16_to_f32(fp.out, y, (long long)M * C, st));
  hipStreamSynchronize(st);
  return 0;
}

AGD_API int agd_op_attn_chain(const float* x, const float* gamma, const float* beta, const float* wq, const float* kv, const float* wo,
                              const float* bo, float* y, float* probs_sum, int B, int HW, int T, int C, int heads, float eps, void* stream) {
  hipStream_t st = S(stream);
  const int rows32 = (heads >> 8) & 1; heads &= 255;
  if (probs_sum && B > 0 && T > 0 && HW > 0 && hipMemsetAsync(probs_sum, 0, (size_t)B * T * HW * 4, st) != hipSuccess) { agd_set_error("memset probs"); return -1; }
  return agd_op_attn_chain_ex(x, gamma, beta, wq, kv, wo, bo, y, B, HW, T, C, heads, eps, nullptr, nullptr, nullptr, nullptr, 0, nullptr, probs_sum, 8, 0, T, T,
                              rows32, 0, stream);
}
AGD_API int agd_op_attn_chain_ex(const float* x, const float* gamma, const float* beta, const float* wq, const float* kv, const float* wo,
                                 const float* bo, float* y, int B, int HW, int T, int C, int heads, float eps, const float* o1, const float* wo1,
                                 const float* bo1, float* h1, int src_rows, float* rowstat, float* rec, int rec_hpb, int rec_b0, int rec_T,
                                 int rec_rows, int rows32, int inplace, void* stream) {
  hipStream_t st = S(stream); Tmp tmp;
  if (C != 320 && C != 640) { agd_set_error("op_attn_chain: C %d", C); return -1; }
  if (B < 1 || HW < 1 || (long long)B * HW >= (1LL << 31) || T < 0 || src_rows < 0 || !x || !gamma || !beta || !wq || !kv || !wo || !bo || !y) { agd_set_error("op_attn_chain: bad arguments (B %d HW %d T %d src_rows %d)", B, HW, T, src_rows); return -1; }
  if (o1 && (!wo1 || !bo1)) { agd_set_error("op_attn_chain: the prologue needs wo1 and bo1"); return -1; }
  if (h1 && !o1) { agd_set_error("op_attn_chain: h1 is the prologue's"); return -1; }
  if (rec && (rec_b0 < 0 || rec_b0 > B || rec_T < 1 || rec_T > rec_rows)) { agd_set_error("op_attn_chain: recorder rows b0 %d T %d of %d", rec_b0, rec_T, rec_rows); return -1; }
  const long long M = (long long)B * HW, Min = src_rows > 0 ? src_rows : M;
  bf16_t* xb = tmp.get<bf16_t>((size_t)Min * C); bf16_t* yb = tmp.get<bf16_t>((size_t)M * C); bf16_t* kvb = tmp.get<bf16_t>((size_t)B * T * 2 * C);
  bf16_t* wqb = tmp.get<bf16_t>((size_t)C * C); bf16_t* wqf = tmp.get<bf16_t>((size_t)C * C);
  bf16_t* wob = tmp.get<bf16_t>((size_t)C * C); bf16_t* wof = tmp.get<bf16_t>((size_t)C * C);
  if (!xb || !yb || !kvb || !wqb || !wqf || !wob || !wof) return -1;
  CK(launch_f32_to_bf16(x, xb, Min * C, st));
  if (T > 0) CK(launch_f32_to_bf16(kv, kvb, (long long)B * T * 2 * C, st));
  CK(launch_convert_weight(wq, wqb, C, C, 1, C, 0, st)); CK(launch_frag_order_w(wqb, wqf, C, C, 5, C, st));
  CK(launch_convert_weight(wo, wob, C, C, 1, C, 0, st)); CK(launch_frag_order_w(wob, wof, C, C, 5, C, st));
  AttnChainP ap{}; ap.h = xb; ap.out = inplace ? xb : yb; ap.gamma = gamma; ap.beta = beta; ap.ln_eps = eps; ap.wqf = wqf; ap.wof = wof; ap.bo = bo;
  ap.rows32 = rows32; ap.src_rows = src_rows;
  ap.kv = kvb; ap.ldkv = 2 * C; ap.skv = (long long)T * 2 * C; ap.M = (int)M; ap.HW = HW; ap.T = T; ap.scale = 1.0f / sqrtf((float)(heads > 0 ? C / heads : C));
  if (o1) {
    bf16_t* o1b = tmp.get<bf16_t>((size_t)Min * C); bf16_t* w1b = tmp.get<bf16_t>((size_t)C * C); bf16_t* w1f = tmp.get<bf16_t>((size_t)C * C);
    if (!o1b || !w1b || !w1f) return -1;
    CK(launch_f32_to_bf16(o1, o1b, Min * C, st));
    CK(launch_convert_weight(wo1, w1b, C, C, 1, C, 0, st)); CK(launch_frag_order_w(w1b, w1f, C, C, 5, C, st));
    ap.o1 = o1b; ap.wo1f = w1f; ap.bo1 = bo1;
  }
  if (h1) {
    bf16_t* zw = tmp.get<bf16_t>((size_t)C * C); float* zb = tmp.get<float>(C); bf16_t* hb = tmp.get<bf16_t>((size_t)M * C);
    if (!zw || !zb || !hb) return -1;
    if (hipMemsetAsync(zw, 0, (size_t)C * C * 2, st) != hipSuccess || hipMemsetAsync(zb, 0, (size_t)C * 4, st) != hipSuccess) { agd_set_error("op_attn_chain: memset"); return -1; }
    AttnChainP a1 = ap; a1.wof = zw; a1.bo = zb; a1.out = inplace ? xb : hb;
    CK(launch_attn_chain(a1, C, heads, st));
    CK(launch_bf16_to_f32(a1.out, h1, M * C, st));
  }
  ap.rowstat_out = rowstat;
  if (rec) {
    const int slices = (rec_hpb >= 1 && rec_hpb <= 8 && 8 % rec_hpb == 0) ? 8 / rec_hpb : 1;
    ap.record = 1; ap.rec = rec; ap.rec_b0 = rec_b0; ap.rec_T = rec_T; ap.rec_hpb = rec_hpb;
    ap.rec_head_stride = (long long)rec_rows * HW; ap.rec_img_stride = ap.rec_head_stride * slices;
  }
  CK(launch_attn_chain(ap, C, heads, st));
  CK(launch_bf16_to_f32(ap.out, y, M * C, st));
  hipStreamSynchronize(st);
  return 0;
}

AGD_API int agd_op_qkv_chain(const float* x, const float* gn_gamma, const float* gn_beta, int groups, float gn_eps, const float* part, int bm,
                             const float* w_in, const float* b_in, const float* gamma, const float* beta, float ln_eps, const float* wqkv, float* h,
                             float* qkv, int M, int HW, int C, int flags, void* stream) {
  hipStream_t st = S(stream); Tmp tmp;
  if (M < 1 || HW < 1 || groups < 1 || bm < 1 || C < 64 || C > 1280 || C % 64) { agd_set_error("op_qkv_chain: bad shape (M %d HW %d C %d groups %d bm %d)", M, HW, C, groups, bm); return -1; }
  if (!x || !gn_gamma || !gn_beta || !part || !w_in || !b_in || !gamma || !beta || !wqkv || !h || !qkv) { agd_set_error("op_qkv_chain: bad arguments"); return -1; }
  const int B = M / HW > 0 ? M / HW : 1;
  const size_t MC = (size_t)M * C;
  bf16_t* xb = tmp.get<bf16_t>(MC); bf16_t* hb = tmp.get<bf16_t>(MC); bf16_t* qb = tmp.get<bf16_t>(3 * MC);
  bf16_t* wib = tmp.get<bf16_t>((size_t)C * C); bf16_t* wqb = tmp.get<bf16_t>((size_t)3 * C * C); bf16_t* wqf = tmp.get<bf16_t>((size_t)3 * C * C);
  if (!xb || !hb || !qb || !wib || !wqb || !wqf) return -1;
  CK(launch_f32_to_bf16(x, xb, (long long)MC, st));
  CK(launch_convert_weight(w_in, wib, C, C, 1, C, 0, st));
  CK(launch_convert_weight(wqkv, wqb, 3 * C, C, 1, C, 0, st));
  QkvChainP qp{}; qp.x = xb; qp.h = hb; qp.qkv = qb; qp.gamma = gamma; qp.beta = beta; qp.ln_eps = ln_eps; qp.M = M; qp.HW = HW;
  qp.rows64 = (flags >> 1) & 1; qp.sched2 = (flags >> 2) & 1;
  if (C != 320 && C != 640) return launch_qkv_chain(qp, C, st);
  CK(launch_frag_order_w(wqb, wqf, 3 * C, C, 5, C, st));
  qp.wqkvf = wqf;
  if (flags & 1) {
    bf16_t* wif = tmp.get<bf16_t>((size_t)C * C); if (!wif) return -1;
    CK(launch_frag_order_w(wib, wif, C, C, 5, C, st));
    qp.wbf = wif; qp.wb_stride = 0; qp.rowadd = b_in; qp.rowadd_stride = 0;
    qp.gn_part = part; qp.gn_bm = bm; qp.gn_groups = groups; qp.gn_eps = gn_eps; qp.gn_gamma = gn_gamma; qp.gn_beta = gn_beta;
  } else {
    bf16_t* wb = tmp.get<bf16_t>((size_t)B * C * C); float* radd = tmp.get<float>((size_t)B * C); if (!wb || !radd) return -1;
    CK(launch_gn_fold_weight(part, bm, B, HW, C, groups, gn_eps, gn_gamma, gn_beta, wib, b_in, C, wb, radd, st, 5));
    qp.wbf = wb; qp.wb_stride = (long long)C * C; qp.rowadd = radd; qp.rowadd_stride = C;
  }
  CK(launch_qkv_chain(qp, C, st));
  CK(launch_bf16_to_f32(hb, h, (long long)MC, st));
  CK(launch_bf16_to_f32(qb, qkv, (long long)(3 * MC), st));
  hipStreamSynchronize(st);
  return 0;
}

AGD_API int agd_op_xattn_premul(const float* x, const float* gamma, const float* beta, const float* wq, const float* kv, const float* wo,
                                const float* bo, float* y, float* probs, int B, int HW, int T, int C, int heads, float eps, void* stream) {
  hipStream_t st = S(stream); Tmp tmp;
  const long long M = (long long)B * HW;
  if (heads < 1 || C % heads || (C / heads) % 8 || C % 160 || C % 64 || HW % 64 || T < 1 || T > XATTN_TP || (heads * XATTN_TP) % 64) { agd_set_error("op_xattn_premul: C %d heads %d HW %d T %d", C, heads, HW, T); return -1; }
  const size_t HT = (size_t)heads * XATTN_TP;
  bf16_t* xb = tmp.get<bf16_t>((size_t)M * C); bf16_t* yb = tmp.get<bf16_t>((size_t)M * C); bf16_t* kvb = tmp.get<bf16_t>((size_t)B * T * 2 * C);
  bf16_t* wqb = tmp.get<bf16_t>((size_t)C * C); bf16_t* wqT = tmp.get<bf16_t>((size_t)C * C); bf16_t* wob = tmp.get<bf16_t>((size_t)C * C);
  float* wqbeta = tmp.get<float>(C); float* rst = tmp.get<float>((size_t)M * 2);
  bf16_t* kpp = tmp.get<bf16_t>((size_t)B * HT * C); bf16_t* vpp = tmp.get<bf16_t>((size_t)B * HT * C); float* kcs = tmp.get<float>((size_t)B * HT * 2);
  bf16_t* P = tmp.get<bf16_t>((size_t)M * HT);
  if (!xb || !yb || !kvb || !wqb || !wqT || !wob || !wqbeta || !rst || !kpp || !vpp || !kcs || !P) return -1;
  CK(launch_f32_to_bf16(x, xb, M * C, st));
// ... 290 lines not shown
  hipEvent_t a, b; hipEventCreate(&a); hipEventCreate(&b);
  for (int i = 0; i < 2; ++i) CK(run_conv(nullptr, 0, x0, C0, x1, C1, B, H, W, wm, ksize, y, o, op_zero_page()));
  hipEventRecord(a, 0);
  for (int i = 0; i < iters; ++i) CK(run_conv(nullptr, 0, x0, C0, x1, C1, B, H, W, wm, ksize, y, o, op_zero_page()));
  hipEventRecord(b, 0); hipEventSynchronize(b);
  float t = 0; hipEventElapsedTime(&t, a, b);
  *ms_out = t / iters;
  hipEventDestroy(a); hipEventDestroy(b);
  return 0;
}

AGD_API int agd_bench_conv_cold(int B, int H, int W, int C0, int Cout, int ksize, int geglu, int with_residual, int warm, int iters, double* ms_out) {
  Tmp tmp;
  const int taps = ksize * ksize;
  const long long M = (long long)B * H * W;
  const int Nout = geglu ? Cout / 2 : Cout;
  const size_t xn = (size_t)M * C0, wn = (size_t)Cout * taps * C0, flush_bytes = (size_t)1 << 30;
  bf16_t* x0 = tmp.get<bf16_t>(xn); bf16_t* xs = tmp.get<bf16_t>(xn); bf16_t* w = tmp.get<bf16_t>(wn); bf16_t* y = tmp.get<bf16_t>((size_t)M * Nout);
  bf16_t* r = with_residual ? tmp.get<bf16_t>((size_t)M * Nout) : nullptr;
  float* bias = tmp.get<float>(Cout); char* scratch = tmp.get<char>(flush_bytes); unsigned* sink = tmp.get<unsigned>(64);
  if (!x0 || !xs || !w || !y || !bias || !scratch || !sink || (with_residual && !r)) return -1;
  fill_rand(xs, (long long)xn, 1, 1.0f); fill_rand(w, (long long)wn, 3, 0.05f); if (r) fill_rand(r, M * Nout, 4, 1.0f);
  hipMemset(bias, 0, Cout * 4);
  WMat wm; wm.w = w; wm.N = Cout; wm.Cin = C0; wm.Cpad = C0; wm.taps = taps;
  GemmOpt o; o.bias = bias; o.geglu = geglu; o.residual = r; o.warm = warm == 3 ? 3 : 0;
  o.halo = 1; o.p8 = 1; o.smap = 1;
  bf16_t* ix = tmp.get<bf16_t>((size_t)8 * 1024 * 640); bf16_t* iy = tmp.get<bf16_t>((size_t)8 * 1024 * 640); bf16_t* iw = tmp.get<bf16_t>((size_t)640 * 9 * 640);
  if (!ix || !iy || !iw) return -1;
  fill_rand(ix, (long long)8 * 1024 * 640, 11, 1.0f); fill_rand(iw, (long long)640 * 9 * 640, 12, 0.05f);
  WMat iwm; iwm.w = iw; iwm.N = 640; iwm.Cin = 640; iwm.Cpad = 640; iwm.taps = 9;
  GemmOpt io; io.bias = bias;
  hipEvent_t a, b; hipEventCreate(&a); hipEventCreate(&b);
  double tot = 0;
  for (int i = 0; i < iters + 1; ++i) {
    hipMemsetAsync(scratch, i, flush_bytes, 0);
    hipMemcpyAsync(x0, xs, xn * 2, hipMemcpyDeviceToDevice, 0);
    if (r) hipMemcpyAsync(y, r, (size_t)M * Nout * 2, hipMemcpyDeviceToDevice, 0);
    if (warm == 2 || warm >= 4) hipLaunchKernelGGL(touch_kernel, dim3(1024), dim3(256), 0, 0, (const u32x4*)w, (long long)(wn * 2 / 16), sink);
    for (int k = 0; k < (warm == 4 ? 1 : warm == 5 ? 2 : warm == 6 ? 4 : 0); ++k) CK(run_conv(nullptr, 0, ix, 640, nullptr, 0, 8, 32, 32, iwm, 3, iy, io, op_zero_page()));
    hipEventRecord(a, 0);
    if (warm == 1) hipLaunchKernelGGL(touch_kernel, dim3(1024), dim3(256), 0, 0, (const u32x4*)w, (long long)(wn * 2 / 16), sink);
    CK(run_conv(nullptr, 0, x0, C0, nullptr, 0, B, H, W, wm, ksize, y, o, op_zero_page()));
    hipEventRecord(b, 0); hipEventSynchronize(b);
    float t = 0; hipEventElapsedTime(&t, a, b);
    if (i > 0) tot += t;
  }
  *ms_out = tot / iters;
  hipEventDestroy(a); hipEventDestroy(b);
  return 0;
}

AGD_API int agd_bench_tblock(int kind, int B, int HW, int iters, double* ms_out) {
  Tmp tmp;
  const int C = (kind == 4 || kind == 5) ? 640 : 320, T = 77; const long long M = (long long)B * HW;
  if (kind == 4 || kind == 5) kind = kind == 4 ? 1 : 3;
  bf16_t* h = tmp.get<bf16_t>((size_t)M * C); bf16_t* o = tmp.get<bf16_t>((size_t)M * C);
  bf16_t* w1 = tmp.get<bf16_t>((size_t)8 * C * C); bf16_t* w1f = tmp.get<bf16_t>((size_t)8 * C * C);
  bf16_t* w2 = tmp.get<bf16_t>((size_t)4 * C * C); bf16_t* w2f = tmp.get<bf16_t>((size_t)4 * C * C);
  bf16_t* kv = tmp.get<bf16_t>((size_t)B * T * 2 * C);
  const int rslices = C == 640 ? 8 : 1;
  float* vec = tmp.get<float>((size_t)16 * C + 64); float* rec = tmp.get<float>((size_t)B * rslices * T * HW);
  if (!h || !o || !w1 || !w1f || !w2 || !w2f || !kv || !vec || !rec) return -1;
  fill_rand(h, M * C, 1, 1.0f); fill_rand(w1, 8LL * C * C, 2, 0.05f); fill_rand(w2, 4LL * C * C, 3, 0.03f); fill_rand(kv, (long long)B * T * 2 * C, 4, 1.0f);
  hipMemset(vec, 0, ((size_t)16 * C + 64) * 4); hipMemset(rec, 0, (size_t)B * rslices * T * HW * 4);
  FFusedP fp{}; AttnChainP ap{};
  if (kind == 0) {
    CK(launch_frag_order_w1(w1, w1f, C, 4 * C, 0)); CK(launch_frag_order_w(w2, w2f, C, 4 * C, C / 64, 128, 0));
    fp.h = h; fp.out = o; fp.w1f = w1f; fp.cs1 = vec; fp.b1 = vec + 8 * C; fp.w2f = w2f; fp.b2 = vec; fp.M = (int)M; fp.ln_eps = 1e-5f;
  } else {
    CK(launch_frag_order_w(w1, w1f, C, C, 5, C, 0)); CK(launch_frag_order_w(w2, w2f, C, C, 5, C, 0));
    ap.h = h; ap.out = o; ap.gamma = vec; ap.beta = vec; ap.ln_eps = 1e-5f; ap.wqf = w1f; ap.wof = w2f; ap.bo = vec; ap.kv = kv; ap.ldkv = 2 * C; ap.skv = (long long)T * 2 * C;
    ap.M = (int)M; ap.HW = HW; ap.T = T; ap.scale = 1.0f / sqrtf((float)(C / 8));
    ap.record = 1; ap.rec = rec; ap.rec_b0 = B / 2; ap.rec_T = T; ap.rec_hpb = 8 / rslices; ap.rec_head_stride = (long long)T * HW; ap.rec_img_stride = (long long)rslices * T * HW;
  }
  bf16_t* o2 = nullptr; float* cst = nullptr;
  if (kind == 2) {
    o2 = tmp.get<bf16_t>((size_t)M * C); cst = tmp.get<float>((size_t)(M / 128 + 1) * C * 2); if (!o2 || !cst) return -1;
    bf16_t* wpf = tmp.get<bf16_t>((size_t)C * C); if (!wpf) return -1;
    CK(launch_frag_order_w(w2, wpf, C, C, C / 64, C, 0));
    CK(launch_frag_order_w1(w1, w1f, C, 4 * C, 0)); CK(launch_frag_order_w(w2, w2f, C, 4 * C, C / 64, 128, 0));
    fp.h = h; fp.out = o; fp.w1f = w1f; fp.cs1 = vec; fp.b1 = vec + 8 * C; fp.w2f = w2f; fp.b2 = vec; fp.M = (int)M; fp.ln_eps = 1e-5f;
    fp.wpf = wpf; fp.bp = vec; fp.xres = o2; fp.pout = o; fp.colstat = cst;
  }
  if (kind == 3) {
    o2 = tmp.get<bf16_t>((size_t)M * C); bf16_t* wo1f = tmp.get<bf16_t>((size_t)C * C); if (!o2 || !wo1f) return -1;
    fill_rand(o2, M * C, 9, 1.0f);
    CK(launch_frag_order_w(w2, wo1f, C, C, 5, C, 0));
    ap.o1 = o2; ap.wo1f = wo1f; ap.bo1 = vec;
  }
  QkvChainP qp{};
  const bool qkvk = kind >= 6 && kind <= 9;
  if (qkvk) {
    bf16_t* qkv = tmp.get<bf16_t>((size_t)M * 3 * C); float* part = tmp.get<float>((size_t)B * (HW / 128) * C * 2); float* gv = tmp.get<float>((size_t)4 * C);
    if (!qkv || !part || !gv) return -1;
    hipMemset(part, 0x3C, (size_t)B * (HW / 128) * C * 2 * 4); hipMemset(gv, 0x3C, (size_t)4 * C * 4);
    CK(launch_frag_order_w(w2, w2f, C, C, 5, C, 0)); CK(launch_frag_order_w(w1, w1f, 3 * C, C, 5, C, 0));
    qp.x = h; qp.wbf = w2f; qp.wb_stride = 0; qp.rowadd = gv; qp.rowadd_stride = 0; qp.h = o; qp.gamma = gv + C; qp.beta = gv + 2 * C; qp.ln_eps = 1e-5f;
    qp.wqkvf = w1f; qp.qkv = qkv; qp.M = (int)M; qp.HW = HW; qp.rows64 = kind == 7 || kind == 9; qp.sched2 = kind >= 8;
    qp.gn_part = part; qp.gn_bm = 128; qp.gn_groups = 32; qp.gn_eps = 1e-6f; qp.gn_gamma = gv + 3 * C; qp.gn_beta = gv;
  }
  auto run = [&]() { return qkvk ? launch_qkv_chain(qp, C, 0) : (kind == 0 || kind == 2) ? launch_ff_fused(fp, C, 0) : launch_attn_chain(ap, C, 8, 0); };
  hipEvent_t a, b; hipEventCreate(&a); hipEventCreate(&b);
  for (int i = 0; i < 2; ++i) CK(run());
  hipEventRecord(a, 0);
  for (int i = 0; i < iters; ++i) CK(run());
  hipEventRecord(b, 0); hipEventSynchronize(b);
  float t = 0; hipEventElapsedTime(&t, a, b);
  *ms_out = t / iters;
  hipEventDestroy(a); hipEventDestroy(b);
  return 0;
}

AGD_API int agd_bench_attention(int B, int H, int D, int Nq, int Nk, int record, int iters, double* ms_out) {
  Tmp tmp;
  const int C = H * D;
  const bool self = (Nq == Nk);
  bf16_t* q = tmp.get<bf16_t>((size_t)B * Nq * (self ? 3 * C : C)); bf16_t* kv = self ? nullptr : tmp.get<bf16_t>((size_t)B * Nk * 2 * C);
  bf16_t* o = tmp.get<bf16_t>((size_t)B * Nq * C);
  float* rec = record ? tmp.get<float>((size_t)B * H * Nk * Nq) : nullptr;
  if (!q || !o || (!self && !kv) || (record && !rec)) return -1;
  fill_rand(q, (long long)B * Nq * (self ? 3 * C : C), 5, 1.0f); if (kv) fill_rand(kv, (long long)B * Nk * 2 * C, 6, 1.0f);
  if (rec) hipMemset(rec, 0, (size_t)B * H * Nk * Nq * 4);
  AttnP a{};
  if (self) { a.q = q; a.k = q + C; a.v = q + 2 * C; a.ldq = a.ldk = a.ldv = 3 * C; a.sq = a.sk = a.sv = (long long)Nq * 3 * C; }
  else { a.q = q; a.k = kv; a.v = kv + C; a.ldq = C; a.ldk = a.ldv = 2 * C; a.sq = (long long)Nq * C; a.sk = a.sv = (long long)Nk * 2 * C; }
  a.o = o; a.ldo = C; a.so = (long long)Nq * C; a.B = B; a.H = H; a.D = D; a.Nq = Nq; a.Nk = Nk; a.scale = 1.0f / sqrtf((float)D);
// ... 1311 lines not shown
```

### agenda_amd/csrc/tblock.hip

```cpp
#include "kernels.h"
#include <type_traits>

typedef __attribute__((ext_vector_type(2))) float f32x2_t;
#ifdef AGD_EXPERIMENTS
int g_tb_variant = 0;
extern "C" __attribute__((visibility("default"))) void agd_set_tb_variant(int v) { g_tb_variant = v; }
#endif
#ifdef AGD_STAMPS
__device__ unsigned long long g_tb_ts[256];
__device__ int g_tb_ts_sel[2] = {-1, 0};
extern "C" __attribute__((visibility("default"))) int agd_tb_ts(int wg, int wave, unsigned long long* out) {
  if (out) return hipMemcpyFromSymbol(out, HIP_SYMBOL(g_tb_ts), 256 * 8) == hipSuccess ? 0 : -1;
  const int sel[2] = {wg, wave};
  return hipMemcpyToSymbol(HIP_SYMBOL(g_tb_ts_sel), sel, 8) == hipSuccess ? 0 : -1;
}
#define TB_TS_DECL const bool ts_on = (int)blockIdx.x == g_tb_ts_sel[0] && (int)threadIdx.x == g_tb_ts_sel[1] * 64; int ts_n = 0; if (ts_on) g_tb_ts[250] = __builtin_amdgcn_s_memrealtime();
#define TB_TS(k) do { if (ts_on && ts_n < 240) g_tb_ts[ts_n++] = ((unsigned long long)(k) << 56) | (__builtin_amdgcn_s_memtime() & 0x00FFFFFFFFFFFFFFull); } while (0)
#define TB_TS_END do { if (ts_on) { asm volatile("s_waitcnt vmcnt(0)" ::: "memory"); TB_TS(99); g_tb_ts[255] = ts_n; g_tb_ts[251] = __builtin_amdgcn_s_memrealtime(); } } while (0)
#else
#define TB_TS_DECL
#define TB_TS(k) do { } while (0)
#define TB_TS_END do { } while (0)
#endif

__global__ __launch_bounds__(256) void frag_order_w1_kernel(const bf16_t* __restrict__ src, bf16_t* __restrict__ dst, int C, int HID) {
  const int KS1 = C / 32, NCH = HID / 128;
  const long long total = (long long)NCH * 4 * KS1 * 4 * 64;
  for (long long idx = (long long)blockIdx.x * 256 + threadIdx.x; idx < total; idx += (long long)gridDim.x * 256) {
    const int l = (int)(idx & 63); long long f = idx >> 6;
    const int j = (int)(f & 3); f >>= 2;
    const int ks = (int)(f % KS1); f /= KS1;
    const int nq = (int)(f & 3); const int c = (int)(f >> 2);
    const int rho = l & 15, g = l >> 4, qp = rho >> 2, rp = rho & 3;
    const int gate = j >> 1, jj = j & 1;
    const int hcol = 128 * c + 32 * nq + 8 * qp + 4 * jj + rp;
    const long long row = 16LL * (hcol >> 3) + 8 * gate + (hcol & 7);
    *(u32x4*)(dst + idx * 8) = *(const u32x4*)(src + row * C + 32 * ks + 8 * g);
  }
}
__global__ __launch_bounds__(256) void frag_order_w_kernel(const bf16_t* __restrict__ src, bf16_t* __restrict__ dst, int N, int K, int NI, int KC) {
  const int NQ = N / (NI * 16), KSC = KC / 32, NCH = K / KC;
  const long long total = (long long)NCH * NQ * KSC * NI * 64;
  for (long long idx = (long long)blockIdx.x * 256 + threadIdx.x; idx < total; idx += (long long)gridDim.x * 256) {
    const int l = (int)(idx & 63); long long f = idx >> 6;
    const int j = (int)(f % NI); f /= NI;
    const int ks = (int)(f % KSC); f /= KSC;
    const int nq = (int)(f % NQ); const int c = (int)(f / NQ);
    const int rho = l & 15, g = l >> 4, qp = rho >> 2, rp = rho & 3;
    const long long n = (long long)nq * NI * 16 + qp * 4 * NI + 4 * j + rp;
    *(u32x4*)(dst + idx * 8) = *(const u32x4*)(src + n * K + (long long)c * KC + 32 * ks + 8 * g);
  }
}
int launch_frag_order_w1(const bf16_t* src, bf16_t* dst, int C, int HID, hipStream_t st) {
  if (C % 32 || HID % 128) { agd_set_error("frag_order_w1: C %d / hidden %d", C, HID); return -1; }
  hipLaunchKernelGGL(frag_order_w1_kernel, dim3(1024), dim3(256), 0, st, src, dst, C, HID);
  HIP_CHECK_RET(hipGetLastError());
  return 0;
}
int launch_frag_order_w(const bf16_t* src, bf16_t* dst, int N, int K, int NI, int KC, hipStream_t st) {
  if (N % (NI * 16) || K % KC || KC % 32) { agd_set_error("frag_order_w: N %d K %d NI %d KC %d", N, K, NI, KC); return -1; }
  hipLaunchKernelGGL(frag_order_w_kernel, dim3(1024), dim3(256), 0, st, src, dst, N, K, NI, KC);
  HIP_CHECK_RET(hipGetLastError());
  return 0;
}

#define TB_OOB 0x80000000u
template <int C> AGD_DEV int panel_swz(int ch, int row) {
  if constexpr ((C * 2) % 256 == 128) return (ch & ~7) | ((ch & 7) ^ ((row >> 1) & 7));
  else return (ch & ~15) | ((ch & 15) ^ (row & 15));
}
template <int C> struct XOff {
  static constexpr int XG = ((C * 2) % 256 == 128) ? 2 : 4;
  int xo[4];
  AGD_DEV XOff(int q, int px) {
#pragma unroll
    for (int t = 0; t < 4; ++t) xo[t] = ((C * 2) % 256 == 128) ? (((4 * (t & 1) + q) ^ ((px >> 1) & 7)) << 4) : (((4 * t + q) ^ px) << 4);
  }
  AGD_DEV int at(int ks) const { return (ks / XG) * (XG * 64) + xo[ks % XG]; }
};

template <int C, int BM = 128, int NW = 8>
AGD_DEV void panel_load_dma(const bf16_t* src, int m0, int M, char* panel, int wid, int lane) {
  constexpr int CHR = C / 8, PIECES = BM * CHR / 64;
  static_assert(PIECES % NW == 0, "pieces split evenly over the workgroup's waves");
#pragma unroll
  for (int i = 0; i < PIECES / NW; ++i) {
    const int piece = i * NW + wid, pos = piece * 64 + lane;
    const int row = pos / CHR, pc = pos - row * CHR;
    const int lc = panel_swz<C>(pc, row);
    const int m = m0 + row;
    const unsigned voff = m < M ? (unsigned)(((long long)m * C + lc * 8) * 2) : TB_OOB;
    bufdma16(src, panel + piece * 1024, voff, 0u);
  }
}

template <int C, int BM = 128>
AGD_DEV void panel_row_stats(const char* panel, float* lnst, int tid, float eps) {
  constexpr int CHR = C / 8, TPR = 512 / BM, PER = CHR / TPR;
  static_assert(CHR % TPR == 0, "chunks per row split over the row's threads");
  const int row = tid / TPR, part = tid % TPR;
  float S = 0.f, Q = 0.f;
#pragma unroll
  for (int cc = 0; cc < PER; ++cc) {
    const u32x4 v = *(const u32x4*)(panel + row * (C * 2) + panel_swz<C>(part * PER + cc, row) * 16);
#pragma unroll
    for (int e = 0; e < 4; ++e) {
      const float a = __uint_as_float(v[e] << 16), b = __uint_as_float(v[e] & 0xFFFF0000u);
      S += a + b; Q += a * a + b * b;
    }
  }
#pragma unroll
  for (int o = 1; o < TPR; o <<= 1) { S += __shfl_xor(S, o); Q += __shfl_xor(Q, o); }
  if (part == 0) {
    const float mu = S * (1.0f / C);
// ... 325 lines not shown
      pkk[t] = pk;
      if (live) {
        const float a0 = __uint_as_float(pk[0] << 16), a1 = __uint_as_float(pk[0] & 0xFFFF0000u), a2 = __uint_as_float(pk[1] << 16), a3 = __uint_as_float(pk[1] & 0xFFFF0000u);
        cs[4 * t] += a0; cs[4 * t + 1] += a1; cs[4 * t + 2] += a2; cs[4 * t + 3] += a3;
        cq[4 * t] += a0 * a0; cq[4 * t + 1] += a1 * a1; cq[4 * t + 2] += a2 * a2; cq[4 * t + 3] += a3 * a3;
      }
    }
    if (live) store_row_chunk<NI2>(p.pout + mo, pkk);
  }
  if (p.colstat) {
#pragma unroll
    for (int e = 0; e < NI2 * 4; ++e) {
#pragma unroll
      for (int o = 1; o < 16; o <<= 1) { cs[e] += __shfl_xor(cs[e], o); cq[e] += __shfl_xor(cq[e], o); }
    }
    float* stg = (float*)hbuf;
    if (px == 0) {
#pragma unroll
      for (int e = 0; e < NI2 * 4; ++e) { stg[(mh * C + ncol0 + e) * 2] = cs[e]; stg[(mh * C + ncol0 + e) * 2 + 1] = cq[e]; }
    }
    __syncthreads();
    if (tid < C) {
      float* op = p.colstat + ((long long)blockIdx.x * C + tid) * 2;
      op[0] = stg[tid * 2] + stg[(C + tid) * 2]; op[1] = stg[tid * 2 + 1] + stg[(C + tid) * 2 + 1];
    }
  }
  }
  TB_TS_END;
}

int launch_ff_fused(const FFusedP& p, int C, hipStream_t st) {
  if (C != 320) { agd_set_error("ff_fused: C = %d is not built (320 only)", C); return -1; }
  if (p.M < 1 || !p.h || !p.out || !p.w1f || !p.w2f || !p.cs1 || !p.b1 || !p.b2) { agd_set_error("ff_fused: bad arguments"); return -1; }
  if ((long long)p.M * C * 2 >= (1LL << 31)) { agd_set_error("ff_fused: activation too large for 32-bit offsets"); return -1; }
  constexpr int lds = 128 * 320 * 2 + 2 * 128 * 128 * 2 + 128 * 8 + 3 * 4 * 128 * 4;
  const void* kfn = p.wpf ? (p.premul ? (const void*)ff_fused_kernel<320, 0, 2> : (const void*)ff_fused_kernel<320, 0, 1>) : (const void*)ff_fused_kernel<320>;
  if (p.wpf && (!p.bp || !p.xres || !p.pout)) { agd_set_error("ff_fused: the proj_out stage needs bias, residual and output"); return -1; }
  if (p.premul && !p.wpf) { agd_set_error("ff_fused: the pre-multiplied form is the proj_out stage's"); return -1; }
#ifdef AGD_EXPERIMENTS
  static const void* const vars[16] = {(const void*)ff_fused_kernel<320, 0>, (const void*)ff_fused_kernel<320, 1>, (const void*)ff_fused_kernel<320, 2>, (const void*)ff_fused_kernel<320, 3>,
                                       (const void*)ff_fused_kernel<320, 4>, nullptr, (const void*)ff_fused_kernel<320, 6>, (const void*)ff_fused_kernel<320, 7>,
                                       (const void*)ff_fused_kernel<320, 8>, nullptr, (const void*)ff_fused_kernel<320, 10>, nullptr, nullptr, nullptr, (const void*)ff_fused_kernel<320, 14>, nullptr};
  if (!p.wpf && g_tb_variant > 0 && g_tb_variant < 16 && vars[g_tb_variant]) kfn = vars[g_tb_variant];
#endif
  int dev = 0; HIP_CHECK_RET(hipGetDevice(&dev));
  if (dev < 0 || dev >= AGD_MAX_DEVICES) { agd_set_error("ff_fused: device ordinal %d out of range", dev); return -1; }
  HIP_CHECK_RET(hipFuncSetAttribute(kfn, hipFuncAttributeMaxDynamicSharedMemorySize, lds));
  FFusedP pp = p;
  void* args[] = {&pp};
  HIP_CHECK_RET(hipLaunchKernel(kfn, dim3((p.M + 127) / 128), dim3(512), args, lds, st));
  return 0;
}

template <int C, int PRE, int MI = 4>
__global__ __launch_bounds__(512, 2) void attn_chain_kernel(const AttnChainP p) {
  TB_TS_DECL
  TB_TS(0);
  constexpr int NQ = C / 80, MH = 8 / NQ, BM = 16 * MI * MH, QBN = BM / 32;
  static_assert(MI == 4 || (MI == 2 && C == 640), "32-row panels: C = 640 only");
  constexpr int H = 8, D = C / H, KS = C / 32, NI = 5, PITCH = C * 2, CHR = C / 8;
  static_assert(C == 320 || C == 640, "8 heads of 40 / 80");
  constexpr int KB = 3, KEYS = 96, KSTEPS = (D + 15) / 16, DBLK = (D + 31) / 32, CH = D / 8;
  constexpr int KPITCH = ((2 * KSTEPS) | 1) * 16, VPITCH = (DBLK | 1) * 64;
  constexpr int KVSTAGE = KEYS * (KPITCH + VPITCH);
  constexpr int NCHUNK = KEYS * CH, LD_IT = (NCHUNK + 255) / 256;
  extern __shared__ __attribute__((aligned(16))) char smem[];
  char* panel = smem;
  char* kvs = smem + BM * PITCH;
  float* lnst = (float*)(kvs + 2 * KVSTAGE);
  float* pst = lnst + BM * 2;
  float* gbs = pst + NQ * BM * 2;

  const int tid = threadIdx.x, lane = tid & 63;
  const int wid = __builtin_amdgcn_readfirstlane(tid >> 6);
  const int mh = wid / NQ, nq = wid % NQ;
  const int q = lane >> 4, px = lane & 15;
  const int qb = wid & (QBN - 1), hhalf = wid >> 2;
  const bool attn_wave = QBN == 4 || (wid & 3) < QBN;
  const int c = lane & 31, hh = lane >> 5;
  const int m0 = blockIdx.x * BM;
  const int b = m0 / p.HW, pix0 = m0 - b * p.HW;
  const int m0s = p.src_rows > 0 ? m0 % p.src_rows : m0;
  TB_TS(1);
  const int gbi = tid < C / 2 ? tid : 0;
  const f32x4 gbv = *(const f32x4*)((gbi < C / 4 ? p.gamma : p.beta - C) + 4 * gbi);
  panel_load_dma<C, BM>(PRE ? p.o1 : p.h, m0s, p.src_rows > 0 ? p.src_rows : p.M, panel, wid, lane);
  TB_TS(40);

  char* sK = kvs + hhalf * KVSTAGE;
  char* sV = sK + KEYS * KPITCH;
  const int t4 = tid & 255;
  constexpr int KPADC = KPITCH / 16 - CH;
  for (int i = t4; i < KEYS * KPADC; i += 256) { const int r = i / KPADC, cc = CH + i % KPADC; *(u32x4*)(sK + r * KPITCH + cc * 16) = u32x4{0, 0, 0, 0}; }
  TB_TS(41);
  u32x4 kreg[LD_IT], vreg[LD_IT];
  unsigned kvoff[LD_IT];
#pragma unroll
  for (int it = 0; it < LD_IT; ++it) {
    const int idx = t4 + it * 256, r = idx / CH, cc = idx - r * CH;
    kvoff[it] = idx < NCHUNK ? (unsigned)((r * p.ldkv + cc * 8) * 2) : TB_OOB;
  }
  const unsigned kv_bytes = (unsigned)(((long long)(p.T - 1) * p.ldkv + D) * 2);
  const bf16_t* kvb = p.kv + (long long)b * p.skv;
  auto kv_load = [&](int h) {
    const auto krs = __builtin_amdgcn_make_buffer_rsrc((void*)(kvb + h * D), 0, kv_bytes, 0x00020000);
    const auto vrs = __builtin_amdgcn_make_buffer_rsrc((void*)(kvb + C + h * D), 0, kv_bytes, 0x00020000);
#pragma unroll
    for (int it = 0; it < LD_IT; ++it) {
      kreg[it] = __builtin_bit_cast(u32x4, __builtin_amdgcn_raw_buffer_load_b128(krs, kvoff[it], 0, 0));
      vreg[it] = __builtin_bit_cast(u32x4, __builtin_amdgcn_raw_buffer_load_b128(vrs, kvoff[it], 0, 0));
    }
  };
  auto kv_store = [&]() {
#pragma unroll
    for (int it = 0; it < LD_IT; ++it) {
      const int idx = t4 + it * 256, r = idx / CH, cc = idx - r * CH;
      if (idx < NCHUNK) { *(u32x4*)(sK + r * KPITCH + cc * 16) = kreg[it]; *(u32x4*)(sV + r * VPITCH + cc * 16) = vreg[it]; }
    }
  };
  kv_load(4 * hhalf);
  TB_TS(42);

  const int rbase = 16 * MI * mh + px;
  const XOff<C> xo(q, px);
  const char* xrow = panel + rbase * PITCH;
  f32x4 acc[MI][NI];
  u32x4 ring[TB_F];
  const unsigned lane16 = (unsigned)lane * 16u;
  const unsigned wbase = __builtin_amdgcn_readfirstlane((unsigned)(nq * KS * NI) * 1024u);
  auto gemm_head = [&](const bf16_t* wf) { panel_gemm_head<C>(ring, wf, wbase, lane16); };
  auto gemm_body = [&](const bf16_t* wf) { panel_gemm_body<C, true, MI>(ring, acc, wf, wbase, lane16, xrow, xo); };
  auto gemm_body_late = [&](const bf16_t* wf, auto&& late) __attribute__((always_inline)) { panel_gemm_body<C, true, MI>(ring, acc, wf, wbase, lane16, xrow, xo, (unsigned)(C * C * 2), late); };
  const int ncol0 = 16 * NI * nq + 4 * NI * q;

  if constexpr (PRE) gemm_head(p.wo1f);
  TB_TS(2);
  asm volatile("s_waitcnt vmcnt(0)" ::: "memory");
  if (tid < C / 2) *(f32x4*)(gbs + 4 * tid) = gbv;
  __syncthreads();
  TB_TS(3);
  kv_store();
  if constexpr (!PRE) {
    panel_row_stats<C, BM>(panel, lnst, tid, p.ln_eps);
    __syncthreads();
    gemm_head(p.wqf);
  }

  if constexpr (PRE) {
    u32x2 hr[MI][NI];
    auto ld_hr = [&]() __attribute__((always_inline)) {
#pragma unroll
      for (int i = 0; i < MI; ++i) load_row_chunk<NI>(p.h + (long long)(m0s + rbase + 16 * i) * C + ncol0, hr[i]);
    };
    gemm_body_late(p.wo1f, ld_hr);
    TB_TS(4);
    gemm_head(p.wqf);
    float bv1[NI * 4];
#pragma unroll
    for (int t = 0; t < NI; ++t) *(f32x4*)&bv1[4 * t] = *(const f32x4*)(p.bo1 + ncol0 + 4 * t);
    float rs1[MI], rq1[MI];
#pragma unroll
    for (int i = 0; i < MI; ++i) {
      const int m = m0 + rbase + 16 * i;
      bf16_t* op = p.out + (long long)m * C + ncol0;
      u32x2 pkk[NI];
      const u32x2 (&r)[NI] = hr[i];
      rs1[i] = 0.f; rq1[i] = 0.f;
#pragma unroll
      for (int t = 0; t < NI; ++t) {
        u32x2 pk;
        pk[0] = pack_bf2(acc[i][t][0] + bv1[4 * t] + __uint_as_float(r[t][0] << 16), acc[i][t][1] + bv1[4 * t + 1] + __uint_as_float(r[t][0] & 0xFFFF0000u));
        pk[1] = pack_bf2(acc[i][t][2] + bv1[4 * t + 2] + __uint_as_float(r[t][1] << 16), acc[i][t][3] + bv1[4 * t + 3] + __uint_as_float(r[t][1] & 0xFFFF0000u));
        pkk[t] = pk;
        acc[i][t] = f32x4{__uint_as_float(pk[0] << 16), __uint_as_float(pk[0] & 0xFFFF0000u), __uint_as_float(pk[1] << 16), __uint_as_float(pk[1] & 0xFFFF0000u)};
        rs1[i] += (acc[i][t][0] + acc[i][t][1]) + (acc[i][t][2] + acc[i][t][3]);
        rq1[i] += (acc[i][t][0] * acc[i][t][0] + acc[i][t][1] * acc[i][t][1]) + (acc[i][t][2] * acc[i][t][2] + acc[i][t][3] * acc[i][t][3]);
      }
      store_row_chunk<NI>(op, pkk);
      rs1[i] += __shfl_xor(rs1[i], 16); rs1[i] += __shfl_xor(rs1[i], 32);
      rq1[i] += __shfl_xor(rq1[i], 16); rq1[i] += __shfl_xor(rq1[i], 32);
      if (q == 0) *(f32x2_t*)(pst + (nq * BM + rbase + 16 * i) * 2) = f32x2_t{rs1[i], rq1[i]};
    }
    TB_TS(5);
    __syncthreads();
    float g2[NI * 4], b2[NI * 4];
#pragma unroll
    for (int t = 0; t < NI; ++t) { *(f32x4*)&g2[4 * t] = *(const f32x4*)(gbs + ncol0 + 4 * t); *(f32x4*)&b2[4 * t] = *(const f32x4*)(gbs + C + ncol0 + 4 * t); }
#pragma unroll
    for (int i = 0; i < MI; ++i) {
      const int row = rbase + 16 * i;
      float S = 0.f, Q = 0.f;
#pragma unroll
      for (int w = 0; w < NQ; ++w) { const f32x2_t v = *(const f32x2_t*)(pst + (w * BM + row) * 2); S += v[0]; Q += v[1]; }
      const float mu = S * (1.0f / C);
      float var = Q * (1.0f / C) - mu * mu; var = var < 0.f ? 0.f : var;
      const float rstd = rsqrtf(var + p.ln_eps);
#pragma unroll
      for (int t = 0; t < NI; ++t) {
        const int n = ncol0 + 4 * t;
        u32x2 pk;
        pk[0] = pack_bf2((acc[i][t][0] - mu) * rstd * g2[4 * t] + b2[4 * t], (acc[i][t][1] - mu) * rstd * g2[4 * t + 1] + b2[4 * t + 1]);
        pk[1] = pack_bf2((acc[i][t][2] - mu) * rstd * g2[4 * t + 2] + b2[4 * t + 2], (acc[i][t][3] - mu) * rstd * g2[4 * t + 3] + b2[4 * t + 3]);
        *(u32x2*)(panel + row * PITCH + panel_swz<C>(n >> 3, row) * 16 + (n & 7) * 2) = pk;
      }
    }
  } else {
#pragma unroll 2
  for (int i = 0; i < BM * CHR / 512; ++i) {
    const int pos = i * 512 + tid, row = pos / CHR, pc = pos - row * CHR, lc = panel_swz<C>(pc, row);
    u32x4 v = *(u32x4*)(panel + row * PITCH + pc * 16);
    const f32x2_t st = *(const f32x2_t*)(lnst + row * 2);
    const f32x4 g0 = *(const f32x4*)(gbs + lc * 8), g1 = *(const f32x4*)(gbs + lc * 8 + 4);
    const f32x4 b0 = *(const f32x4*)(gbs + C + lc * 8), b1 = *(const f32x4*)(gbs + C + lc * 8 + 4);
    float x[8];
#pragma unroll
    for (int e = 0; e < 4; ++e) { x[2 * e] = __uint_as_float(v[e] << 16); x[2 * e + 1] = __uint_as_float(v[e] & 0xFFFF0000u); }
#pragma unroll
    for (int e = 0; e < 4; ++e) { x[e] = (x[e] - st[0]) * st[1] * g0[e] + b0[e]; x[4 + e] = (x[4 + e] - st[0]) * st[1] * g1[e] + b1[e]; }
    v[0] = pack_bf2(x[0], x[1]); v[1] = pack_bf2(x[2], x[3]); v[2] = pack_bf2(x[4], x[5]); v[3] = pack_bf2(x[6], x[7]);
    *(u32x4*)(panel + row * PITCH + pc * 16) = v;
  }
  }
  TB_TS(6);
  __syncthreads();

  TB_TS(7);
  gemm_body(p.wqf);
  TB_TS(8);
  __syncthreads();
#pragma unroll
  for (int i = 0; i < MI; ++i) {
    const int row = rbase + 16 * i;
#pragma unroll
    for (int t = 0; t < NI; ++t) {
      const int n = ncol0 + 4 * t;
      u32x2 pk; pk[0] = pack_bf2(acc[i][t][0], acc[i][t][1]); pk[1] = pack_bf2(acc[i][t][2], acc[i][t][3]);
      *(u32x2*)(panel + row * PITCH + panel_swz<C>(n >> 3, row) * 16 + (n & 7) * 2) = pk;
    }
  }
  __syncthreads();
  TB_TS(9);

  {
    const int qr = 32 * qb + c;
    char* prow = panel + qr * PITCH;
    const float sc = p.scale * 1.44269504088896340736f;
    const bool recb = p.record && b >= p.rec_b0;
    const int hpb = p.rec_hpb;
    f32x16 pacc[KB];
#pragma unroll
    for (int kb = 0; kb < KB; ++kb)
#pragma unroll
      for (int j = 0; j < 16; ++j) pacc[kb][j] = 0.f;
    const int gi = lane & 15;
    const int tr_row = (gi >> 2) + 4 * hh;
    const int tr_col = ((lane >> 4) & 1) * 16 + (gi & 3) * 4;
    auto rec_rmw = [&](int slice, const f32x16 (&pa)[KB]) {
      float* base = p.rec + (long long)(b - p.rec_b0) * p.rec_img_stride + (long long)slice * p.rec_head_stride;
      const unsigned nbytes = (unsigned)p.rec_T * (unsigned)p.HW * 4u;
      const auto rsrc = __builtin_amdgcn_make_buffer_rsrc(base, 0, nbytes, 0x00020000);
      const unsigned rowb = (unsigned)p.HW * 4u;
      const unsigned voff0 = (unsigned)(pix0 + qr) * 4u + (unsigned)(4 * hh) * rowb;
      float old[KB][16];
#pragma unroll
      for (int kb = 0; kb < KB; ++kb)
#pragma unroll
        for (int i = 0; i < 16; ++i)
          old[kb][i] = __builtin_bit_cast(float, __builtin_amdgcn_raw_buffer_load_b32(rsrc, voff0 + (unsigned)(kb * 32 + (i & 3) + 8 * (i >> 2)) * rowb, 0, 0));
#pragma unroll
      for (int kb = 0; kb < KB; ++kb)
#pragma unroll
        for (int i = 0; i < 16; ++i)
          __builtin_amdgcn_raw_buffer_store_b32(__builtin_bit_cast(unsigned, old[kb][i] + pa[kb][i]), rsrc,
                                                voff0 + (unsigned)(kb * 32 + (i & 3) + 8 * (i >> 2)) * rowb, 0, 0);
    };

    for (int hi = 0; hi < 4; ++hi) {
      const int h = 4 * hhalf + hi;
      if (hi + 1 < 4) kv_load(h + 1);
      if (attn_wave) {
      bf16x8 qf[KSTEPS];
#pragma unroll
      for (int s = 0; s < KSTEPS; ++s) {
        const int d0 = 16 * s + 8 * hh;
        u32x4 v = u32x4{0, 0, 0, 0};
        if (d0 < D) v = *(const u32x4*)(prow + panel_swz<C>(CH * h + 2 * s + hh, qr) * 16);
        qf[s] = __builtin_bit_cast(bf16x8, v);
      }
      f32x16 sacc[KB];
#pragma unroll
      for (int kb = 0; kb < KB; ++kb)
#pragma unroll
        for (int s = 0; s < KSTEPS; ++s) {
          const bf16x8 a = *(const bf16x8*)(sK + (kb * 32 + c) * KPITCH + (2 * s + hh) * 16);
          if (s == 0) { const f32x16 z = {0.f, 0.f, 0.f, 0.f, 0.f, 0.f, 0.f, 0.f, 0.f, 0.f, 0.f, 0.f, 0.f, 0.f, 0.f, 0.f};
                        sacc[kb] = __builtin_amdgcn_mfma_f32_32x32x16_bf16(a, qf[s], z, 0, 0, 0); }
          else sacc[kb] = __builtin_amdgcn_mfma_f32_32x32x16_bf16(a, qf[s], sacc[kb], 0, 0, 0);
        }
#pragma unroll
      for (int kb = 0; kb < KB; ++kb)
#pragma unroll
        for (int i = 0; i < 16; ++i) {
          const int key = kb * 32 + (i & 3) + 8 * (i >> 2) + 4 * hh;
          if (key >= p.T) sacc[kb][i] = -INFINITY;
        }
      float mx = sacc[0][0];
#pragma unroll
      for (int kb = 0; kb < KB; ++kb)
#pragma unroll
        for (int i = 0; i < 16; ++i) mx = fmaxf(mx, sacc[kb][i]);
      mx = xhalf_max(mx) * sc;
      float rsum = 0.f;
#pragma unroll
      for (int kb = 0; kb < KB; ++kb)
#pragma unroll
        for (int i = 0; i < 16; ++i) { const float pv = __builtin_amdgcn_exp2f(fmaf(sacc[kb][i], sc, -mx)); sacc[kb][i] = pv; rsum += pv; }
      const float inv = 1.0f / xhalf_sum(rsum);
      if (recb) {
#pragma unroll
        for (int kb = 0; kb < KB; ++kb)
#pragma unroll
          for (int i = 0; i < 16; ++i) pacc[kb][i] += sacc[kb][i] * inv;
      }
      f32x16 oacc[DBLK];
#pragma unroll
      for (int db = 0; db < DBLK; ++db)
#pragma unroll
        for (int j = 0; j < 16; ++j) oacc[db][j] = 0.f;
#pragma unroll
      for (int kb = 0; kb < KB; ++kb)
#pragma unroll
        for (int s = 0; s < 2; ++s) {
          bf16x8 pf;
#pragma unroll
          for (int j = 0; j < 8; ++j) pf[j] = (__bf16)sacc[kb][8 * s + j];
          const char* vb = sV + (kb * 32 + 16 * s + tr_row) * VPITCH + tr_col * 2;
#pragma unroll
          for (int db = 0; db < DBLK; ++db) {
            const s16x4 lo = __builtin_amdgcn_ds_read_tr16_b64_v4i16((__attribute__((address_space(3))) s16x4*)(vb + db * 64));
            const s16x4 hi2 = __builtin_amdgcn_ds_read_tr16_b64_v4i16((__attribute__((address_space(3))) s16x4*)(vb + 8 * VPITCH + db * 64));
            const u32x2 l2 = __builtin_bit_cast(u32x2, lo), h2 = __builtin_bit_cast(u32x2, hi2);
            const u32x4 a4 = u32x4{l2[0], l2[1], h2[0], h2[1]};
            oacc[db] = __builtin_amdgcn_mfma_f32_32x32x16_bf16(__builtin_bit_cast(bf16x8, a4), pf, oacc[db], 0, 0, 0);
          }
        }
#pragma unroll
      for (int db = 0; db < DBLK; ++db)
#pragma unroll
        for (int g = 0; g < 4; ++g) {
          const int d0 = db * 32 + 8 * g + 4 * hh;
          if (d0 < D) {
            u32x2 pk;
            pk[0] = pack_bf2(oacc[db][4 * g + 0] * inv, oacc[db][4 * g + 1] * inv);
            pk[1] = pack_bf2(oacc[db][4 * g + 2] * inv, oacc[db][4 * g + 3] * inv);
            *(u32x2*)(prow + panel_swz<C>(CH * h + (d0 >> 3), qr) * 16 + (d0 & 7) * 2) = pk;
          }
        }
      if (recb && hpb < H && ((hi + 1) % hpb) == 0) {
        rec_rmw(h / hpb, pacc);
#pragma unroll
        for (int kb = 0; kb < KB; ++kb)
#pragma unroll
          for (int j = 0; j < 16; ++j) pacc[kb][j] = 0.f;
      }
      }
      TB_TS(10 + hi);
      __syncthreads();
      if (hi + 1 < 4) { kv_store(); __syncthreads(); }
      TB_TS(20 + hi);
    }
    gemm_head(p.wof);
    if (p.record && hpb == H) {
      float* xch = (float*)kvs + (qb * 48) * 64 + lane;
      if (hhalf == 1 && recb && attn_wave) {
#pragma unroll
        for (int kb = 0; kb < KB; ++kb)
#pragma unroll
          for (int i = 0; i < 16; ++i) xch[(kb * 16 + i) * 64] = pacc[kb][i];
      }
      __syncthreads();
      if (hhalf == 0 && recb && attn_wave) {
#pragma unroll
        for (int kb = 0; kb < KB; ++kb)
#pragma unroll
          for (int i = 0; i < 16; ++i) pacc[kb][i] += xch[(kb * 16 + i) * 64];
        rec_rmw(0, pacc);
      }
    }
  }
  TB_TS(30);
  __syncthreads();
  TB_TS(31);

  u32x2 fr[MI][NI];
  auto ld_fr = [&]() __attribute__((always_inline)) {
#pragma unroll
    for (int i = 0; i < MI; ++i) load_row_chunk<NI>((PRE ? (const bf16_t*)p.out : p.h) + (long long)((PRE ? m0 : m0s) + rbase + 16 * i) * C + ncol0, fr[i]);
  };
  gemm_body_late(p.wof, ld_fr);
  TB_TS(32);
  float bv[NI * 4];
#pragma unroll
  for (int t = 0; t < NI; ++t) *(f32x4*)&bv[4 * t] = *(const f32x4*)(p.bo + ncol0 + 4 * t);
  float rs[MI], rq[MI];
  char* const ostg = kvs + 4096 + wid * 5120;
#pragma unroll
  for (int i = 0; i < MI; ++i) {
    rs[i] = 0.f; rq[i] = 0.f;
    u32x2 pkk[NI];
    const u32x2 (&r)[NI] = fr[i];
#pragma unroll
    for (int t = 0; t < NI; ++t) {
      const float v0 = acc[i][t][0] + bv[4 * t] + __uint_as_float(r[t][0] << 16), v1 = acc[i][t][1] + bv[4 * t + 1] + __uint_as_float(r[t][0] & 0xFFFF0000u);
      const float v2 = acc[i][t][2] + bv[4 * t + 2] + __uint_as_float(r[t][1] << 16), v3 = acc[i][t][3] + bv[4 * t + 3] + __uint_as_float(r[t][1] & 0xFFFF0000u);
      u32x2 pk; pk[0] = pack_bf2(v0, v1); pk[1] = pack_bf2(v2, v3);
      pkk[t] = pk;
      const float a0 = __uint_as_float(pk[0] << 16), a1 = __uint_as_float(pk[0] & 0xFFFF0000u), a2 = __uint_as_float(pk[1] << 16), a3 = __uint_as_float(pk[1] & 0xFFFF0000u);
      rs[i] += (a0 + a1) + (a2 + a3); rq[i] += (a0 * a0 + a1 * a1) + (a2 * a2 + a3 * a3);
    }
#pragma unroll
    for (int t = 0; t < NI; ++t) *(u32x2*)(ostg + (16 * (i & 1) + px) * 160 + 40 * q + 8 * t) = pkk[t];
    if (i & 1) {
#pragma unroll
      for (int it = 0; it < 5; ++it) {
        const int id = 64 * it + lane, row = id / 10, pc = id - row * 10;
        const u32x4 v = *(const u32x4*)(ostg + 16 * id);
        *(u32x4*)(p.out + (long long)(m0 + 16 * MI * mh + 16 * (i - 1) + row) * C + 80 * nq + 8 * pc) = v;
      }
    }
  }
  if (p.rowstat_out) {
#pragma unroll
    for (int i = 0; i < MI; ++i) {
      rs[i] += __shfl_xor(rs[i], 16); rs[i] += __shfl_xor(rs[i], 32);
      rq[i] += __shfl_xor(rq[i], 16); rq[i] += __shfl_xor(rq[i], 32);
    }
    float* stg = (float*)kvs;
    if (q == 0) {
#pragma unroll
      for (int i = 0; i < MI; ++i) { stg[(nq * BM + rbase + 16 * i) * 2] = rs[i]; stg[(nq * BM + rbase + 16 * i) * 2 + 1] = rq[i]; }
    }
    __syncthreads();
    if (tid < BM) {
      float S = 0.f, Q = 0.f;
#pragma unroll
      for (int w = 0; w < NQ; ++w) { S += stg[(w * BM + tid) * 2]; Q += stg[(w * BM + tid) * 2 + 1]; }
      *(f32x2_t*)(p.rowstat_out + (long long)(m0 + tid) * 2) = f32x2_t{S, Q};
    }
  }
  TB_TS_END;
}

int launch_attn_chain(const AttnChainP& p, int C, int heads, hipStream_t st) {
  if ((C != 320 && C != 640) || heads != 8) { agd_set_error("attn_chain: C = %d / heads = %d is not built (320 or 640 / 8 only)", C, heads); return -1; }
  const bool r32 = C == 640 && p.rows32 && p.M / 64 < 200 && p.HW % 32 == 0;
  const int BM = C == 320 ? 128 : r32 ? 32 : 64;
  if (p.M < BM || p.M % BM || p.HW % BM || p.M % p.HW) { agd_set_error("attn_chain: M %d / HW %d must be multiples of %d (whole images)", p.M, p.HW, BM); return -1; }
  if (p.T < 1 || p.T > 96) { agd_set_error("attn_chain: %d keys (1..96)", p.T); return -1; }
  if ((long long)p.M * C * 2 >= (1LL << 31)) { agd_set_error("attn_chain: activation too large for 32-bit offsets"); return -1; }
  if (p.record && (p.rec_hpb < 1 || 8 % p.rec_hpb || !p.rec)) { agd_set_error("attn_chain: recorder head group %d", p.rec_hpb); return -1; }
  const int D = C / 8, ks = (D + 15) / 16, db = (D + 31) / 32;
  const int lds = BM * C * 2 + 2 * 96 * ((((2 * ks) | 1) * 16) + ((db | 1) * 64)) + BM * 8 + (C / 80) * BM * 8 + 2 * C * 4;
  const bool pre = p.o1 != nullptr;
  if (pre && (!p.wo1f || !p.bo1 || p.out == p.h)) { agd_set_error("attn_chain: the to_out prologue needs its weights and out != h"); return -1; }
  if (p.src_rows > 0 && (p.src_rows % BM || p.M % p.src_rows || p.out == p.h)) { agd_set_error("attn_chain: src_rows %d must divide M, be a multiple of %d and out != h", p.src_rows, BM); return -1; }
  const void* kfn = C == 320 ? (pre ? (const void*)attn_chain_kernel<320, 1> : (const void*)attn_chain_kernel<320, 0>)
                    : r32    ? (pre ? (const void*)attn_chain_kernel<640, 1, 2> : (const void*)attn_chain_kernel<640, 0, 2>)
                             : (pre ? (const void*)attn_chain_kernel<640, 1> : (const void*)attn_chain_kernel<640, 0>);
  static std::atomic<bool> attr[AGD_MAX_DEVICES][6] = {};
  int dev = 0; HIP_CHECK_RET(hipGetDevice(&dev));
  if (dev < 0 || dev >= AGD_MAX_DEVICES) { agd_set_error("attn_chain: device ordinal %d out of range", dev); return -1; }
  const int slot = (C == 640 ? (r32 ? 4 : 2) : 0) + (pre ? 1 : 0);
  if (!attr[dev][slot]) { HIP_CHECK_RET(hipFuncSetAttribute(kfn, hipFuncAttributeMaxDynamicSharedMemorySize, lds)); attr[dev][slot] = true; }
  AttnChainP pp = p;
  void* args[] = {&pp};
  HIP_CHECK_RET(hipLaunchKernel(kfn, dim3(p.M / BM), dim3(512), args, lds, st));
  return 0;
}

template <int C, int MH = 8 / (C / 80)>
__global__ __launch_bounds__(64 * MH * (C / 80), 2) void qkv_chain_kernel(const QkvChainP p) {
  constexpr int NQ = C / 80, BM = 64 * MH, KS = C / 32, NI = 5, PITCH = C * 2, NT = 64 * MH * NQ;
  extern __shared__ __attribute__((aligned(16))) char smem[];
  char* panel = smem;
  float* pst = (float*)(smem + BM * PITCH);
  const int tid = threadIdx.x, lane = tid & 63;
  const int wid = __builtin_amdgcn_readfirstlane(tid >> 6);
  const int mh = wid / NQ, nq = wid % NQ;
  const int q = lane >> 4, px = lane & 15;
  const int m0 = blockIdx.x * BM;
  const int img = m0 / p.HW;
  TB_TS_DECL
  TB_TS(1);

  panel_load_dma<C, BM, MH * NQ>(p.x, m0, p.M, panel, wid, lane);
  const int rbase = 64 * mh + px;
  const char* xrow = panel + rbase * PITCH;
  f32x4 acc[4][NI];
  u32x4 ring[TB_F];
  const unsigned lane16 = (unsigned)lane * 16u;
  const int ncol0 = 80 * nq + 4 * NI * q;
  const unsigned wbase = __builtin_amdgcn_readfirstlane((unsigned)(nq * KS * NI) * 1024u);
  const bf16_t* wimg = p.wbf + (long long)img * p.wb_stride;
  panel_gemm_head<C>(ring, wimg, wbase, lane16);
  TB_TS(2);
  if (p.gn_part) {
    double* csum = (double*)(smem + BM * PITCH + NQ * BM * 8);
    float* gst = (float*)(csum + 2 * C);
    float* ab = gst + 64;
    const int nt = p.HW / p.gn_bm, cpg = C / p.gn_groups;
    constexpr int CPT = (C + NT - 1) / NT;
    float gam[CPT], bet[CPT];
#pragma unroll
    for (int r = 0; r < CPT; ++r) {
      const int cch = tid + NT * r < C ? tid + NT * r : C - 1;
      gam[r] = p.gn_gamma[cch]; bet[r] = p.gn_beta[cch];
      const float* pp = p.gn_part + ((long long)img * nt * C + cch) * 2;
      double a = 0.0, qq = 0.0;
      for (int t0 = 0; t0 < nt; t0 += 16) {
        f32x2_t v[16];
#pragma unroll
        for (int u = 0; u < 16; ++u) { const int tc = t0 + u < nt ? t0 + u : nt - 1; v[u] = *(const f32x2_t*)(pp + (long long)tc * C * 2); }
#pragma unroll
        for (int u = 0; u < 16; ++u) if (t0 + u < nt) { a += (double)v[u][0]; qq += (double)v[u][1]; }
      }
// ... 363 lines not shown
```

### agenda_amd/ops.py

```python
from __future__ import annotations

import ctypes

import torch

from . import _lib


def _f32c(t):
    assert t.is_cuda, "ops run on the GPU only (no CPU fallback)"
    return t.detach().to(torch.float32).contiguous()


_P8 = {0: 0, 1: 2, 2: 4, 3: 8}


def conv2d(x, w, bias=None, stride=1, padding=None, upsample=False, halo=False, p8=0, smap=False, phases=False, pc=0, xcd_block=False):
    lib = _lib.load()
    x, w = _f32c(x), _f32c(w)
    b = _f32c(bias) if bias is not None else None
    B, Cin, H, W = x.shape
    Cout, _, k, _ = w.shape
    pad = (1 if k == 3 else 0) if padding is None else padding
    up = 2 if upsample else 1
# ... 140 lines not shown
    return (y, path.value) if return_path else y


def gn_fold(part, bm, groups, gamma, beta, w, bias=None, eps=1e-6, x=None, frag_ni=0, hw=None):
    lib = _lib.load()
    part, w = _f32c(part), _f32c(w)
    B, nt, Cc = part.shape[:3]
    HW = nt * bm if hw is None else hw
    N = w.shape[0]
    assert w.shape[1] == Cc and part.shape[3] == 2
    b = _f32c(bias) if bias is not None else None
    dev = part.device
    out = {"wb": torch.empty(B, N, Cc, device=dev), "rowadd": torch.empty(B, N, device=dev)}
    if frag_ni > 0:
        out["wb_frag"] = torch.empty(B, N * Cc, device=dev)
        out["wb_frag_ref"] = torch.empty(B, N * Cc, device=dev)
    if x is not None:
        x = _f32c(x)
        assert x.shape[0] == B and x.shape[1] == Cc and x[0, 0].numel() == HW
        out["y"] = torch.empty(B, HW, N, device=dev)
    _lib.check(lib.agd_op_gn_fold(_lib.ptr(x), _lib.ptr(part), int(bm), B, Cc, HW, groups, float(eps), _lib.ptr(_f32c(gamma)), _lib.ptr(_f32c(beta)),
                                  _lib.ptr(w), _lib.ptr(b), N, int(frag_ni), _lib.ptr(out["wb"]), _lib.ptr(out["rowadd"]), _lib.ptr(out.get("wb_frag")),
                                  _lib.ptr(out.get("wb_frag_ref")), _lib.ptr(out.get("y")), _lib.current_stream_ptr()), None, "agd_op_gn_fold")
    return out


def layer_norm(x, gamma, beta, eps=1e-5, return_path=False):
    lib = _lib.load()
    x = _f32c(x)
    Cc = x.shape[-1]
    rows = x.numel() // Cc
    y = torch.empty_like(x)
    if return_path:
        inst = ctypes.c_int(0)
        _lib.check(lib.agd_op_layernorm_ex(_lib.ptr(x), _lib.ptr(_f32c(gamma)), _lib.ptr(_f32c(beta)), _lib.ptr(y), rows, Cc,
                                           float(eps), ctypes.byref(inst), _lib.current_stream_ptr()), None, "agd_op_layernorm_ex")
        return y, divmod(inst.value, 100)
    _lib.check(lib.agd_op_layernorm(_lib.ptr(x), _lib.ptr(_f32c(gamma)), _lib.ptr(_f32c(beta)), _lib.ptr(y), rows, Cc,
                                    float(eps), _lib.current_stream_ptr()), None, "agd_op_layernorm")
    return y


def ff_fused(x, gamma, beta, w1, b1, w2, b2, eps=1e-5):
    lib = _lib.load()
    Cc = x.shape[-1]
    x2 = _f32c(x).reshape(-1, Cc)
    y = torch.empty_like(x2)
    _lib.check(lib.agd_op_ff_fused(_lib.ptr(x2), _lib.ptr(_f32c(gamma)), _lib.ptr(_f32c(beta)), _lib.ptr(_f32c(w1)), _lib.ptr(_f32c(b1)),
                                   _lib.ptr(_f32c(w2)), _lib.ptr(_f32c(b2)), _lib.ptr(y), x2.shape[0], Cc, float(eps),
                                   _lib.current_stream_ptr()), None, "agd_op_ff_fused")
    return y.reshape(x.shape)


def attn_chain(x, gamma, beta, wq, kv, wo, bo, heads=8, eps=1e-5, return_probs=False, rows32=False):
    lib = _lib.load()
    x, kv = _f32c(x), _f32c(kv)
    B, HW, Cc = x.shape
    T = kv.shape[1]
    y = torch.empty_like(x)
    pr = torch.empty(B, T, HW, device=x.device, dtype=torch.float32) if return_probs else None
    _lib.check(lib.agd_op_attn_chain(_lib.ptr(x), _lib.ptr(_f32c(gamma)), _lib.ptr(_f32c(beta)), _lib.ptr(_f32c(wq)), _lib.ptr(kv), _lib.ptr(_f32c(wo)),
                                     _lib.ptr(_f32c(bo)), _lib.ptr(y), _lib.ptr(pr), B, HW, T, Cc, heads | (256 if rows32 else 0), float(eps), _lib.current_stream_ptr()),
               None, "agd_op_attn_chain")
    return (y, pr) if return_probs else y


def ff_premul_weights(w2, b2, wp, bp):
    wpb = _f32c(wp).to(torch.bfloat16).float()
    w2p = linear(wpb, _f32c(w2).t().contiguous()).to(torch.bfloat16).float()
    bcp = (wpb.double() @ _f32c(b2).double() + _f32c(bp).double()).float()
    return w2p, bcp


def ff_fused_ex(x, gamma, beta, w1, b1, w2, b2, eps=1e-5, *, wp=None, bp=None, xres=None, xres_rows=0, premul=False, colstat=False, inplace=False):
    lib = _lib.load()
    x2 = _f32c(x)
    M, Cc = x2.shape
    y = pout = cst = xr = None
    w2_, bp_ = _f32c(w2), (None if bp is None else _f32c(bp))
    if wp is not None:
        pout = torch.empty_like(x2)
        if xres is not None:
            xr = _f32c(xres)
            assert tuple(xr.shape) == ((xres_rows if xres_rows > 0 else M), Cc), "xres [xres_rows or M, C]"
        if premul:
            w2_, bp_ = ff_premul_weights(w2, b2, wp, bp)
        if colstat:
            cst = torch.full(((M + 127) // 128, Cc, 2), float("nan"), device=x2.device, dtype=torch.float32)
    else:
        y = torch.empty_like(x2)
        if colstat:
            cst = torch.zeros(1, device=x2.device)
    _lib.check(lib.agd_op_ff_fused_ex(_lib.ptr(x2), _lib.ptr(_f32c(gamma)), _lib.ptr(_f32c(beta)), _lib.ptr(_f32c(w1)), _lib.ptr(_f32c(b1)),
                                      _lib.ptr(w2_), _lib.ptr(_f32c(b2)), _lib.ptr(y), M, Cc, float(eps), _lib.ptr(None if wp is None else _f32c(wp)),
                                      _lib.ptr(bp_), _lib.ptr(xr), int(xres_rows), _lib.ptr(pout), int(bool(premul)), _lib.ptr(cst), int(bool(inplace)),
                                      _lib.current_stream_ptr()), None, "agd_op_ff_fused_ex")
    out = y if wp is None else pout
    return (out, cst) if colstat else out


def attn_chain_ex(x, gamma, beta, wq, kv, wo, bo, heads=8, eps=1e-5, *, hw=None, o1=None, wo1=None, bo1=None, src_rows=0, rowstat=False, rec=None,
                  rec_hpb=8, rec_b0=0, rec_T=None, rows32=False, inplace=False):
    lib = _lib.load()
    x, kv = _f32c(x), _f32c(kv)
    Cc = x.shape[-1]
    B, T = kv.shape[:2]
    if src_rows > 0:
        assert x.dim() == 2 and x.shape[0] == src_rows and hw, "src_rows: x [src_rows, C] and hw"
        HW = int(hw)
    else:
        assert x.dim() == 3 and x.shape[0] == B, "x [B, HW, C]"
        HW = x.shape[1]
    dev = x.device
    out = {"y": torch.empty(B, HW, Cc, device=dev, dtype=torch.float32)}
    pre = o1 is not None
    if pre:
        o1 = _f32c(o1)
        assert o1.shape == x.shape, "o1 has x's shape"
        out["h1"] = torch.empty(B, HW, Cc, device=dev, dtype=torch.float32)
    if rowstat:
        out["rowstat"] = torch.full((B, HW, 2), float("nan"), device=dev, dtype=torch.float32)
    rec_rows = 0
    if rec is not None:
        assert rec.is_cuda and rec.dtype == torch.float32 and rec.is_contiguous() and rec.dim() == 4 and rec.shape[3] == HW, "rec [B - rec_b0, groups, rows, HW]"
        assert 0 <= rec_b0 <= B and rec.shape[0] == max(B - rec_b0, 0) and rec.shape[0] > 0, "one recorder image per recording batch row"
        assert rec_hpb not in (1, 2, 4, 8) or rec.shape[1] == 8 // rec_hpb, "one slice per head group"
        rec_rows = rec.shape[2]
        rec_T = rec_rows if rec_T is None else int(rec_T)
    _lib.check(lib.agd_op_attn_chain_ex(_lib.ptr(x), _lib.ptr(_f32c(gamma)), _lib.ptr(_f32c(beta)), _lib.ptr(_f32c(wq)), _lib.ptr(_given(kv)), _lib.ptr(_f32c(wo)),
                                        _lib.ptr(_f32c(bo)), _lib.ptr(out["y"]), B, HW, T, Cc, int(heads), float(eps), _lib.ptr(o1),
                                        _lib.ptr(_f32c(wo1) if pre else None), _lib.ptr(_f32c(bo1) if pre else None), _lib.ptr(out.get("h1")), int(src_rows),
                                        _lib.ptr(out.get("rowstat")), _lib.ptr(rec), int(rec_hpb), int(rec_b0), int(rec_T or 0), int(rec_rows), int(bool(rows32)),
                                        int(bool(inplace)), _lib.current_stream_ptr()), None, "agd_op_attn_chain_ex")
    return out


def qkv_chain(x, hw, gn_gamma, gn_beta, groups, part, bm, w_in, b_in, gamma, beta, wqkv, *, gn_eps=1e-6, ln_eps=1e-5, inside=False, rows64=False, sched2=False):
    lib = _lib.load()
    x, part = _f32c(x), _f32c(part)
    M, Cc = x.shape
    h = torch.empty(M, Cc, device=x.device, dtype=torch.float32)
    qkv = torch.empty(M, 3 * Cc, device=x.device, dtype=torch.float32)
    if hw > 0 and bm > 0:
        assert part.numel() >= max(M // hw, 1) * (hw // bm) * Cc * 2, "partial-sum table [M // hw, hw // bm, C, 2] fp32"
    _lib.check(lib.agd_op_qkv_chain(_lib.ptr(x), _lib.ptr(_f32c(gn_gamma)), _lib.ptr(_f32c(gn_beta)), int(groups), float(gn_eps), _lib.ptr(_given(part)), int(bm),
                                    _lib.ptr(_f32c(w_in)), _lib.ptr(_f32c(b_in)), _lib.ptr(_f32c(gamma)), _lib.ptr(_f32c(beta)), float(ln_eps),
                                    _lib.ptr(_f32c(wqkv)), _lib.ptr(h), _lib.ptr(qkv), M, int(hw), Cc, (1 if inside else 0) | (2 if rows64 else 0) | (4 if sched2 else 0),
                                    _lib.current_stream_ptr()), None, "agd_op_qkv_chain")
    return h, qkv


def xattn_premul(x, gamma, beta, wq, kv, wo, bo, heads=8, eps=1e-5, return_probs=False):
    lib = _lib.load()
    x, kv = _f32c(x), _f32c(kv)
    B, HW, Cc = x.shape
    T = kv.shape[1]
    y = torch.empty_like(x)
    pr = torch.empty(B, heads, T, HW, device=x.device, dtype=torch.float32) if return_probs else None
    _lib.check(lib.agd_op_xattn_premul(_lib.ptr(x), _lib.ptr(_f32c(gamma)), _lib.ptr(_f32c(beta)), _lib.ptr(_f32c(wq)), _lib.ptr(kv), _lib.ptr(_f32c(wo)),
                                       _lib.ptr(_f32c(bo)), _lib.ptr(y), _lib.ptr(pr), B, HW, T, Cc, heads, float(eps), _lib.current_stream_ptr()),
               None, "agd_op_xattn_premul")
    return (y, pr) if return_probs else y


def _given(t):
    t = _f32c(t)
    return t if t.numel() else torch.zeros(1, device=t.device, dtype=torch.float32)


def attention(q, k, v, heads, scale=None, return_probs=False, *, causal=False, mask=None, k2=None, v2=None, layout=0, head_sum=False,
              rec_b0=0, rec_T=None):
    lib = _lib.load()
    q, k, v = _f32c(q), _f32c(k), _f32c(v)
    B, Nq, Cc = q.shape
    Nk = k.shape[1]
    D = Cc // heads
    scale = D ** -0.5 if scale is None else scale
    o = torch.empty_like(q)
    if causal or mask is not None or k2 is not None or v2 is not None or layout != 0 or head_sum or rec_b0 != 0 or rec_T is not None:
        if k.shape != (B, Nk, Cc) or v.shape != k.shape:
            raise ValueError(f"attention: k {tuple(k.shape)} / v {tuple(v.shape)} must both be [B, Nk, H*D] = [{B}, Nk, {Cc}]")
        if mask is not None and tuple(mask.shape) != (B, Nk):
            raise ValueError(f"attention: mask {tuple(mask.shape)} must be {(B, Nk)}")
        if (k2 is None) != (v2 is None) or (k2 is not None and (k2.shape != v2.shape or k2.ndim != 3 or k2.shape[0] != B or k2.shape[2] != Cc)):
            raise ValueError("attention: k2 and v2 come together, both [B, Nk2, H*D]")
        if head_sum and not return_probs:
            raise ValueError("attention: head_sum is a form of return_probs")
# ... 310 lines not shown
```

### include/agenda_hip.h

```cpp
#ifndef AGENDA_HIP_H
#define AGENDA_HIP_H
#ifdef __cplusplus
extern "C" {
#endif

typedef struct agd_ctx agd_ctx;

#define AGD_MAX_LEVELS 8

typedef struct agd_config {
  int struct_size;
  int in_channels, out_channels, n_levels;
  int block_out_channels[AGD_MAX_LEVELS];
  int down_cross[AGD_MAX_LEVELS];
  int num_heads[AGD_MAX_LEVELS];
  int layers_per_block, cross_attention_dim, use_linear_projection, norm_num_groups;
  int vae_latent_channels, vae_out_channels, vae_n_levels;
  int vae_block_out_channels[AGD_MAX_LEVELS];
  int vae_layers_per_block, vae_norm_num_groups;
  float vae_scaling_factor;
  int max_tokens;
  int prediction_type;
  long long workspace_bytes;
  int text_hidden, text_layers, text_heads, text_intermediate, text_vocab, text_max_pos;
// ... 128 lines not shown
int agd_denoise_dpm_hw(agd_ctx* ctx, float* latents, int batch, int latent_h, int latent_w, int n_evals, const float* timesteps,
                       const float* coeffs, float guidance, void* stream);

int agd_vae_decode(agd_ctx* ctx, const float* latents, int batch, int latent_side, unsigned char* out_u8,
                   float* out_f32, void* stream);
int agd_vae_decode_hw(agd_ctx* ctx, const float* latents, int batch, int latent_h, int latent_w, unsigned char* out_u8,
                      float* out_f32, void* stream);

int agd_vae_encode(agd_ctx* ctx, const float* image, int batch, int side, float* mean_out, float* logvar_out, void* stream);
int agd_vae_encode_hw(agd_ctx* ctx, const float* image, int batch, int h, int w, float* mean_out, float* logvar_out, void* stream);

int agd_set_option(agd_ctx* ctx, const char* name, int value);

int agd_record_config(agd_ctx* ctx, int mode, int is_train, int rec_tokens);
int agd_record_reset(agd_ctx* ctx, int batch, int latent_side, void* stream);
int agd_record_reset_hw(agd_ctx* ctx, int batch, int latent_h, int latent_w, void* stream);
int agd_daam_global(agd_ctx* ctx, int img, int rows, float* out, void* stream);
int agd_hook_global(agd_ctx* ctx, float* out, void* stream);
int agd_hook_count(agd_ctx* ctx);
int agd_hook_last_map(agd_ctx* ctx, float* out, int n_query, void* stream);

int agd_attn_processor(agd_ctx* ctx, const char* layer, const float* hidden, const float* ctx_emb, const float* attn_mask,
                       int batch2, int n_query, int tokens, float* out, int record, void* stream);
int agd_cross_attn(agd_ctx* ctx, const char* layer, const float* hidden, const float* ctx_emb, int batch2,
                   int n_query, int tokens, float* out, int record, void* stream);

int agd_hook_reset(agd_ctx* ctx, int rows, int latent_side, void* stream);
int agd_hook_num_maps(agd_ctx* ctx);
int agd_hook_map_dims(agd_ctx* ctx, int k, int* dims3);
int agd_hook_map(agd_ctx* ctx, int k, float* out, void* stream);
int agd_op_attn_reg_loss(const float* map, int B, int T, int P, const int* obj_idx, const int* fg_idx, const int* bg_idx, float coef,
                         float* loss_out, float* dmap, void* stream);
int agd_attn_processor_backward(agd_ctx* ctx, const char* layer, const float* hidden, const float* ctx_emb, const float* d_out,
                                const float* d_map, int is_train, int batch2, int n_query, int tokens, float* d_hidden, float* d_ctx,
                                void* stream);

int agd_op_conv2d(const float* x_nchw, const float* w, const float* bias, float* y_nchw, int B, int Cin, int H, int W,
                  int Cout, int ksize, int stride, int pad, int upsample, void* stream);
int agd_op_conv2d_ex(const float* x, const float* w, const float* bias, float* y, int B, int Cin, int H, int W, int Cout,
                     int ksize, int stride, int pad, int upsample, int flags, void* stream);
int agd_op_linear(const float* x, const float* w, const float* bias, const float* residual, float* y, int M, int K,
                  int N, int geglu, void* stream);
int agd_op_ff_fused(const float* x, const float* gamma, const float* beta, const float* w1, const float* b1, const float* w2,
                    const float* b2, float* y, int M, int C, float eps, void* stream);
int agd_op_attn_chain(const float* x, const float* gamma, const float* beta, const float* wq, const float* kv, const float* wo,
                      const float* bo, float* y, float* probs_sum, int B, int HW, int T, int C, int heads, float eps, void* stream);
int agd_op_ff_fused_ex(const float* x, const float* gamma, const float* beta, const float* w1, const float* b1, const float* w2,
                       const float* b2, float* y, int M, int C, float eps, const float* wp, const float* bp, const float* xres,
                       int xres_rows, float* pout, int premul, float* colstat, int inplace, void* stream);
int agd_op_attn_chain_ex(const float* x, const float* gamma, const float* beta, const float* wq, const float* kv, const float* wo,
                         const float* bo, float* y, int B, int HW, int T, int C, int heads, float eps, const float* o1, const float* wo1,
                         const float* bo1, float* h1, int src_rows, float* rowstat, float* rec, int rec_hpb, int rec_b0, int rec_T,
                         int rec_rows, int rows32, int inplace, void* stream);
int agd_op_qkv_chain(const float* x, const float* gn_gamma, const float* gn_beta, int groups, float gn_eps, const float* part, int bm,
                     const float* w_in, const float* b_in, const float* gamma, const float* beta, float ln_eps, const float* wqkv, float* h,
                     float* qkv, int M, int HW, int C, int flags, void* stream);
int agd_op_xattn_premul(const float* x, const float* gamma, const float* beta, const float* wq, const float* kv, const float* wo,
                        const float* bo, float* y, float* probs, int B, int HW, int T, int C, int heads, float eps, void* stream);
int agd_op_groupnorm(const float* x_nchw, const float* gamma, const float* beta, float* y_nchw, int B, int C, int HW,
                     int groups, float eps, int silu, void* stream);
int agd_op_groupnorm_ex(const float* x0_nchw, const float* x1_nchw, const float* gamma, const float* beta, float* y_nchw, int B, int C0,
                        int C1, int HW, int groups, float eps, int silu, const float* part0, int bm0, const float* part1, int bm1,
                        int* path, void* stream);
int agd_op_gn_fold(const float* x_nchw, const float* part, int bm, int B, int C, int HW, int groups, float eps, const float* gamma,
                   const float* beta, const float* w, const float* bias, int N, int frag_ni, float* wb, float* rowadd, float* wb_frag,
                   float* wb_frag_ref, float* y, void* stream);
int agd_op_conv_groupnorm(const float* x_nchw, const float* w, const float* bias, const float* gamma, const float* beta, float* y_nchw,
                          int B, int Cin, int H, int W, int Cout, int groups, float eps, int silu, int fused, void* stream);
enum { AGD_IGEMM_NONE = 0, AGD_IGEMM_GENERAL = 1, AGD_IGEMM_HALO = 2, AGD_IGEMM_PCH = 3, AGD_IGEMM_PC = 4, AGD_IGEMM_8P = 5, AGD_IGEMM_SMAP = 6,
       AGD_IGEMM_WREG = 7 };
enum { AGD_IGEMM_SLAB_NONE = 0, AGD_IGEMM_SLAB_PLAIN = 1, AGD_IGEMM_SLAB_GN = 2 };
typedef struct agd_igemm_desc {
  int struct_size;
  int images, H, W, C0, C1;
  int ksize, stride, pad, up, hout, wout;
  int sc_C0, sc_C1;
  int N, K, w_per_image;
  int bias_mode, rowadd_ld, ldr, geglu, act, out_f32, ldo;
  int batch;
  int rowstat_slots, ln_slots, colstat_rows;
  int gn_groups, gn_silu, gn_keep_out;
  int halo, p8, smap, pc, kg2, wreg, xcd_block;
  float alpha, ln_invC, ln_eps, gn_eps;
  long long sA0, sA1, sW, sO, sR;
  long long n_src0, n_src1, n_sc0, n_sc1, n_w, n_res, n_out;
  const float* src0; const float* src1; const float* sc0; const float* sc1; const float* w;
  const float* bias; const float* rowadd; const float* residual;
  const float* ln_stats; const float* ln_cs; const float* gn_gamma; const float* gn_beta;
  float* out; float* gn_y; float* rowstat; float* colstat;
  int cfg[3]; int ran[2]; int gn_fused; int can_fuse_sc;
} agd_igemm_desc;
int agd_op_igemm(agd_igemm_desc* d, void* stream);
int agd_op_layernorm(const float* x, const float* gamma, const float* beta, float* y, int rows, int C, float eps,
                     void* stream);
int agd_op_layernorm_ex(const float* x, const float* gamma, const float* beta, float* y, int rows, int C, float eps, int* inst,
                        void* stream);
int agd_op_attention(const float* q, const float* k, const float* v, float* o, int B, int H, int D, int Nq, int Nk,
                     float scale, float* probs_out, void* stream);
int agd_op_attention_ex(const float* q, const float* k, const float* v, float* o, int B, int H, int D, int Nq, int Nk, float scale,
                        int causal, const float* mask, const float* k2, const float* v2, int Nk2, int layout, float* probs_out,
                        int record, int rec_b0, int rec_T, void* stream);
int agd_op_attention_long(const float* q, const float* k, const float* v, float* o, int B, int H, int D, int Nq, int Nk, float scale,
                          int layout, float* probs_inout, int rec_b0, int rec_T, void* stream);
int agd_op_attention_headsum(const float* q, const float* k, const float* v, float* o, int B, int H, int D, int Nq, int Nk,
                             float scale, float* probs_sum_out, void* stream);
int agd_op_attention_backward(const float* q, const float* kv, const float* d_o, const float* d_map, int b0, int B, int H, int D,
// ... 105 lines not shown
```

Before: 9.116.

## Pre-pack cross-attention K/V into MFMA fragment order, load directly to registers

```diff
diff --git a/agenda_amd/_lib.py b/agenda_amd/_lib.py
--- a/agenda_amd/_lib.py
+++ b/agenda_amd/_lib.py
@@ -211,6 +211,7 @@
     "agd_op_attn_chain": (C.c_int, [_P] * 9 + [C.c_int] * 5 + [C.c_float, _P]),
     "agd_op_ff_fused_ex": (C.c_int, [_P] * 8 + [C.c_int, C.c_int, C.c_float, _P, _P, _P, C.c_int, _P, C.c_int, _P, C.c_int, _P]),
     "agd_op_attn_chain_ex": (C.c_int, [_P] * 8 + [C.c_int] * 5 + [C.c_float] + [_P] * 4 + [C.c_int, _P, _P] + [C.c_int] * 6 + [_P]),
+    "agd_op_kv_fragments": (C.c_int, [_P, C.c_int, C.c_int, C.c_int, _P, _P, _P]),
     "agd_op_qkv_chain": (C.c_int, [_P] * 3 + [C.c_int, C.c_float, _P, C.c_int] + [_P] * 4 + [C.c_float] + [_P] * 3 + [C.c_int] * 4 + [_P]),
     "agd_op_xattn_premul": (C.c_int, [_P] * 9 + [C.c_int] * 5 + [C.c_float, _P]),
     "agd_op_attention": (C.c_int, [_P, _P, _P, _P, C.c_int, C.c_int, C.c_int, C.c_int, C.c_int, C.c_float, _P, _P]),
diff --git a/agenda_amd/csrc/kernels.h b/agenda_amd/csrc/kernels.h
--- a/agenda_amd/csrc/kernels.h
+++ b/agenda_amd/csrc/kernels.h
@@ -96,8 +96,11 @@
   const bf16_t* o1; const bf16_t* wo1f; const float* bo1;
   int rows32;
   int src_rows;
+  const bf16_t* kf; const bf16_t* vf;
 };
 int launch_attn_chain(const AttnChainP& p, int C, int heads, hipStream_t st);
+size_t kv_fragment_elems(int C, int heads, bool v);
+int launch_kv_fragments(const bf16_t* kv, int ldkv, long long skv, int B, int T, int C, int heads, bf16_t* kf, bf16_t* vf, hipStream_t st);
 struct QkvChainP {
   const bf16_t* x;
   const bf16_t* wbf; long long wb_stride; const float* rowadd;
diff --git a/agenda_amd/csrc/model.hip b/agenda_amd/csrc/model.hip
--- a/agenda_amd/csrc/model.hip
+++ b/agenda_amd/csrc/model.hip
@@ -63,6 +63,7 @@
   bool cn = false;
   WMat wkv; DBuf kvb; bf16_t* kv = nullptr; DBuf accb; float* acc = nullptr; int acc_h = 0, acc_w = 0;
   int acc_heads = 0;
+  DBuf kvfb; bf16_t* kf = nullptr; bf16_t* vf = nullptr;
   DBuf wqTb, wkvTb, woTb; WMat wqT, wkvT, woT;
   bf16_t* pm_wqT = nullptr; float* pm_wqb = nullptr; bool pm_ready = false;
   DBuf pm_kppb, pm_vppb, pm_csb; bf16_t* pm_kpp = nullptr; bf16_t* pm_vpp = nullptr; float* pm_kcs = nullptr; float* pm_kbs = nullptr;
@@ -93,7 +94,8 @@
   TBF_ATTN2_ROWS32  = 1 << 10,
   TBF_QKV_ROWS64    = 1 << 11,
   TBF_QKV_SCHED2    = 1 << 12,
-  TBF_DEFAULT       = 0x1fff & ~TBF_QKV_640,
+  TBF_ATTN2_FRAG    = 1 << 13,
+  TBF_DEFAULT       = 0x3fff & ~TBF_QKV_640,
 };
 
 struct ProfEv { int cls; double flops, bytes; hipEvent_t a, b; };
@@ -602,6 +604,7 @@
   const IpaLayer* ipa;
   XLayer* xl;
   TbAttn2 attn2; int chain_rows32;
+  bool chain_frag;
   bool daam;
   TbFf ff;
   bool wreg_proj;
@@ -687,6 +690,7 @@
                      c->ctx_T <= 96 && c->rec_mode != 2 && has(t + "attn2.to_q.frag");
   p.attn2 = premul ? ATTN2_PREMUL : chain ? ATTN2_CHAIN : ATTN2_KERNELS;
   p.chain_rows32 = tb(TBF_ATTN2_ROWS32);
+  p.chain_frag = chain && tb(TBF_ATTN2_FRAG) && p.xl->kf;
   if (c->cur.grounded) { auto itf = c->gl_idx.find(pre); if (itf != c->gl_idx.end()) p.fuser = &c->gl_f[itf->second]; }
   if (c->cur.ipa) { auto iti = c->ipa_idx.find(pre); if (iti != c->ipa_idx.end()) p.ipa = &c->ipa_l[iti->second]; }
   const bool lazy = dup && tb(TBF_LAZY_DUP) && chain && C == 320 && (p.ff == FF_FUSED_PROJ || p.ff == FF_FUSED_PREMUL) && !p.fuser && !p.ipa;
@@ -836,6 +840,10 @@
   }
   if (p.dup == DUP_LAZY) ap.src_rows = s.Mshared;
   ap.rows32 = p.chain_rows32;
+  if (p.chain_frag) {
+    const size_t row0 = (size_t)(xl.kv - xl.kvb.as<bf16_t>()) / ((size_t)T * 2 * C);
+    ap.kf = xl.kf + row0 * kv_fragment_elems(C, heads, false); ap.vf = xl.vf + row0 * kv_fragment_elems(C, heads, true);
+  }
   if (p.stats_attn2) {
     s.slots = 1; s.stats = (float*)c->arena.alloc((size_t)M * 2 * sizeof(float)); if (!s.stats) return -1;
     ap.rowstat_out = s.stats;
@@ -1369,7 +1377,7 @@
   hipSetDevice(c->device);
   hipDeviceSynchronize();
   for (void* p : c->owned) hipFree(p);
-  for (auto& xl : c->xl) { xl.kvb.release(); xl.accb.release(); }
+  for (auto& xl : c->xl) { xl.kvb.release(); xl.kvfb.release(); xl.kf = xl.vf = nullptr; xl.accb.release(); }
   c->pano_viewb.release(); c->pano_hmb.release(); c->reg_xb.release(); c->pano_ctxb.release(); c->i2_latb.release();
   c->ctxb.release(); c->hook_sumb.release(); c->hook_scratchb.release(); c->hook_headsb.release(); c->hook_storeb.release(); c->bwd_wsb.release();
   for (auto& xl : c->xl) { xl.wqTb.release(); xl.wkvTb.release(); xl.woTb.release(); xl.pm_kppb.release(); xl.pm_vppb.release(); xl.pm_csb.release(); }
@@ -1928,6 +1936,14 @@
   for (auto& xl : c->xl) {
     GemmOpt o;
     API_CK(c, run_conv(c, st, c->ctx_bf16, Dc, nullptr, 0, 1, 1, batch2 * tokens, xl.wkv, 1, xl.kv, o, c->zero_page));
+    xl.kf = xl.vf = nullptr;
+    if ((xl.C == 320 || xl.C == 640) && xl.heads == 8 && tokens <= 96) {
+      const size_t ke = kv_fragment_elems(xl.C, xl.heads, false), ve = kv_fragment_elems(xl.C, xl.heads, true);
+      API_CK(c, xl.kvfb.ensure((size_t)batch2 * (ke + ve) * 2));
+      bf16_t* kf = xl.kvfb.as<bf16_t>(); bf16_t* vf = kf + (size_t)batch2 * ke;
+      API_CK(c, launch_kv_fragments(xl.kv, 2 * xl.C, (long long)tokens * 2 * xl.C, batch2, tokens, xl.C, xl.heads, kf, vf, st));
+      xl.kf = kf; xl.vf = vf;
+    }
     xl.pm_ready = false;
     if (c->opt_xpre && xl.pm_wqT && tokens <= XATTN_TP && ((c->opt_xpre & 2) || xl.heads * XATTN_TP * 2 <= xl.C)) {
       const std::string t = xl.name.substr(0, xl.name.size() - 5);
@@ -3315,7 +3331,7 @@
 AGD_API int agd_op_attn_chain(const float* x, const float* gamma, const float* beta, const float* wq, const float* kv, const float* wo,
                               const float* bo, float* y, float* probs_sum, int B, int HW, int T, int C, int heads, float eps, void* stream) {
   hipStream_t st = S(stream);
-  const int rows32 = (heads >> 8) & 1; heads &= 255;
+  const int rows32 = (heads >> 8) & 3; heads &= 255;
   if (probs_sum && B > 0 && T > 0 && HW > 0 && hipMemsetAsync(probs_sum, 0, (size_t)B * T * HW * 4, st) != hipSuccess) { agd_set_error("memset probs"); return -1; }
   return agd_op_attn_chain_ex(x, gamma, beta, wq, kv, wo, bo, y, B, HW, T, C, heads, eps, nullptr, nullptr, nullptr, nullptr, 0, nullptr, probs_sum, 8, 0, T, T,
                               rows32, 0, stream);
@@ -3340,7 +3356,14 @@
   CK(launch_convert_weight(wq, wqb, C, C, 1, C, 0, st)); CK(launch_frag_order_w(wqb, wqf, C, C, 5, C, st));
   CK(launch_convert_weight(wo, wob, C, C, 1, C, 0, st)); CK(launch_frag_order_w(wob, wof, C, C, 5, C, st));
   AttnChainP ap{}; ap.h = xb; ap.out = inplace ? xb : yb; ap.gamma = gamma; ap.beta = beta; ap.ln_eps = eps; ap.wqf = wqf; ap.wof = wof; ap.bo = bo;
-  ap.rows32 = rows32; ap.src_rows = src_rows;
+  ap.rows32 = rows32 & 1; ap.src_rows = src_rows;
+  if ((rows32 & 2) && T >= 1 && T <= 96) {
+    const size_t ke = kv_fragment_elems(C, 8, false), ve = kv_fragment_elems(C, 8, true);
+    bf16_t* kf = tmp.get<bf16_t>((size_t)B * ke); bf16_t* vf = tmp.get<bf16_t>((size_t)B * ve);
+    if (!kf || !vf) return -1;
+    CK(launch_kv_fragments(kvb, 2 * C, (long long)T * 2 * C, B, T, C, heads, kf, vf, st));
+    ap.kf = kf; ap.vf = vf;
+  }
   ap.kv = kvb; ap.ldkv = 2 * C; ap.skv = (long long)T * 2 * C; ap.M = (int)M; ap.HW = HW; ap.T = T; ap.scale = 1.0f / sqrtf((float)(heads > 0 ? C / heads : C));
   if (o1) {
     bf16_t* o1b = tmp.get<bf16_t>((size_t)Min * C); bf16_t* w1b = tmp.get<bf16_t>((size_t)C * C); bf16_t* w1f = tmp.get<bf16_t>((size_t)C * C);
@@ -3365,6 +3388,19 @@
   }
   CK(launch_attn_chain(ap, C, heads, st));
   CK(launch_bf16_to_f32(ap.out, y, M * C, st));
+  hipStreamSynchronize(st);
+  return 0;
+}
+
+AGD_API int agd_op_kv_fragments(const float* kv, int B, int T, int C, float* kf, float* vf, void* stream) {
+  hipStream_t st = S(stream); Tmp tmp;
+  if ((C != 320 && C != 640) || B < 1 || T < 1 || T > 96 || !kv || !kf || !vf) { agd_set_error("op_kv_fragments: bad arguments (B %d T %d C %d)", B, T, C); return -1; }
+  const size_t ke = kv_fragment_elems(C, 8, false), ve = kv_fragment_elems(C, 8, true);
+  bf16_t* kvb = tmp.get<bf16_t>((size_t)B * T * 2 * C); bf16_t* kfb = tmp.get<bf16_t>((size_t)B * ke); bf16_t* vfb = tmp.get<bf16_t>((size_t)B * ve);
+  if (!kvb || !kfb || !vfb) return -1;
+  CK(launch_f32_to_bf16(kv, kvb, (long long)B * T * 2 * C, st));
+  CK(launch_kv_fragments(kvb, 2 * C, (long long)T * 2 * C, B, T, C, 8, kfb, vfb, st));
+  CK(launch_bf16_to_f32(kfb, kf, (long long)B * ke, st)); CK(launch_bf16_to_f32(vfb, vf, (long long)B * ve, st));
   hipStreamSynchronize(st);
   return 0;
 }
@@ -3761,6 +3797,9 @@
 
 AGD_API int agd_bench_tblock(int kind, int B, int HW, int iters, double* ms_out) {
   Tmp tmp;
+  const bool frag = (kind & 32) != 0; kind &= 31;
+  const bool r32 = kind == 10 || kind == 11;
+  if (r32) kind -= 6;
   const int C = (kind == 4 || kind == 5) ? 640 : 320, T = 77; const long long M = (long long)B * HW;
   if (kind == 4 || kind == 5) kind = kind == 4 ? 1 : 3;
   bf16_t* h = tmp.get<bf16_t>((size_t)M * C); bf16_t* o = tmp.get<bf16_t>((size_t)M * C);
@@ -3781,6 +3820,13 @@
     ap.h = h; ap.out = o; ap.gamma = vec; ap.beta = vec; ap.ln_eps = 1e-5f; ap.wqf = w1f; ap.wof = w2f; ap.bo = vec; ap.kv = kv; ap.ldkv = 2 * C; ap.skv = (long long)T * 2 * C;
     ap.M = (int)M; ap.HW = HW; ap.T = T; ap.scale = 1.0f / sqrtf((float)(C / 8));
     ap.record = 1; ap.rec = rec; ap.rec_b0 = B / 2; ap.rec_T = T; ap.rec_hpb = 8 / rslices; ap.rec_head_stride = (long long)T * HW; ap.rec_img_stride = (long long)rslices * T * HW;
+    ap.rows32 = r32;
+    if (frag) {
+      const size_t ke = kv_fragment_elems(C, 8, false), ve = kv_fragment_elems(C, 8, true);
+      bf16_t* kf = tmp.get<bf16_t>((size_t)B * ke); bf16_t* vf = tmp.get<bf16_t>((size_t)B * ve); if (!kf || !vf) return -1;
+      CK(launch_kv_fragments(kv, 2 * C, (long long)T * 2 * C, B, T, C, 8, kf, vf, 0));
+      ap.kf = kf; ap.vf = vf;
+    }
   }
   bf16_t* o2 = nullptr; float* cst = nullptr;
   if (kind == 2) {
diff --git a/agenda_amd/csrc/tblock.hip b/agenda_amd/csrc/tblock.hip
--- a/agenda_amd/csrc/tblock.hip
+++ b/agenda_amd/csrc/tblock.hip
@@ -60,6 +60,49 @@
 int launch_frag_order_w(const bf16_t* src, bf16_t* dst, int N, int K, int NI, int KC, hipStream_t st) {
   if (N % (NI * 16) || K % KC || KC % 32) { agd_set_error("frag_order_w: N %d K %d NI %d KC %d", N, K, NI, KC); return -1; }
   hipLaunchKernelGGL(frag_order_w_kernel, dim3(1024), dim3(256), 0, st, src, dst, N, K, NI, KC);
+  HIP_CHECK_RET(hipGetLastError());
+  return 0;
+}
+
+__global__ __launch_bounds__(256) void kv_fragments_kernel(const bf16_t* __restrict__ kv, int ldkv, long long skv, int B, int T, int C, int H,
+                                                           bf16_t* __restrict__ kf, bf16_t* __restrict__ vf) {
+  const int D = C / H, KSTEPS = (D + 15) / 16, DBLK = (D + 31) / 32, NKF = 3 * KSTEPS, NVF = 6 * DBLK;
+  const long long total = (long long)B * H * (NKF + NVF) * 64;
+  for (long long idx = (long long)blockIdx.x * 256 + threadIdx.x; idx < total; idx += (long long)gridDim.x * 256) {
+    const int l = (int)(idx & 63); long long r = idx >> 6;
+    const int f = (int)(r % (NKF + NVF)); r /= (NKF + NVF);
+    const int h = (int)(r % H), b = (int)(r / H);
+    const int c = l & 31, hh = l >> 5;
+    const bf16_t* src = kv + (long long)b * skv + h * D;
+    u32x4 v = u32x4{0, 0, 0, 0};
+    if (f < NKF) {
+      const int kb = f / KSTEPS, s = f - kb * KSTEPS, key = 32 * kb + c, d0 = 16 * s + 8 * hh;
+      if (key < T && d0 < D) v = *(const u32x4*)(src + (long long)key * ldkv + d0);
+      *(u32x4*)(kf + ((((long long)b * H + h) * NKF + f) * 64 + l) * 8) = v;
+    } else {
+      const int g = f - NKF, db = g % DBLK, ks = g / DBLK, d = 32 * db + c;
+      if (d < D) {
+        unsigned short e[8];
+#pragma unroll
+        for (int j = 0; j < 8; ++j) {
+          const int key = 16 * ks + 4 * hh + (j & 3) + 8 * (j >> 2);
+          e[j] = key < T ? *(const unsigned short*)(src + C + (long long)key * ldkv + d) : (unsigned short)0;
+        }
+        v = u32x4{(unsigned)e[0] | ((unsigned)e[1] << 16), (unsigned)e[2] | ((unsigned)e[3] << 16), (unsigned)e[4] | ((unsigned)e[5] << 16), (unsigned)e[6] | ((unsigned)e[7] << 16)};
+      }
+      *(u32x4*)(vf + ((((long long)b * H + h) * NVF + g) * 64 + l) * 8) = v;
+    }
+  }
+}
+size_t kv_fragment_elems(int C, int heads, bool v) {
+  const int D = C / heads;
+  return (size_t)heads * (v ? 6 * ((D + 31) / 32) : 3 * ((D + 15) / 16)) * 512;
+}
+int launch_kv_fragments(const bf16_t* kv, int ldkv, long long skv, int B, int T, int C, int heads, bf16_t* kf, bf16_t* vf, hipStream_t st) {
+  if ((C != 320 && C != 640) || heads != 8 || B < 1 || T < 1 || T > 96 || ldkv % 8 || skv % 8) { agd_set_error("kv_fragments: C %d heads %d B %d T %d ldkv %d", C, heads, B, T, ldkv); return -1; }
+  const long long total = (long long)B * (long long)(kv_fragment_elems(C, heads, false) + kv_fragment_elems(C, heads, true)) / 8;
+  const int grid = (int)((total + 255) / 256 < 2048 ? (total + 255) / 256 : 2048);
+  hipLaunchKernelGGL(kv_fragments_kernel, dim3(grid), dim3(256), 0, st, kv, ldkv, skv, B, T, C, heads, kf, vf);
   HIP_CHECK_RET(hipGetLastError());
   return 0;
 }
@@ -491,7 +534,7 @@
   return 0;
 }
 
-template <int C, int PRE, int MI = 4>
+template <int C, int PRE, int MI = 4, int FRAG = 0>
 __global__ __launch_bounds__(512, 2) void attn_chain_kernel(const AttnChainP p) {
   TB_TS_DECL
   TB_TS(0);
@@ -515,7 +558,7 @@
   const int mh = wid / NQ, nq = wid % NQ;
   const int q = lane >> 4, px = lane & 15;
   const int qb = wid & (QBN - 1), hhalf = wid >> 2;
-  const bool attn_wave = QBN == 4 || (wid & 3) < QBN;
+  const bool attn_wave = FRAG || QBN == 4 || (wid & 3) < QBN;
   const int c = lane & 31, hh = lane >> 5;
   const int m0 = blockIdx.x * BM;
   const int b = m0 / p.HW, pix0 = m0 - b * p.HW;
@@ -530,6 +573,7 @@
   char* sV = sK + KEYS * KPITCH;
   const int t4 = tid & 255;
   constexpr int KPADC = KPITCH / 16 - CH;
+  if constexpr (!FRAG)
   for (int i = t4; i < KEYS * KPADC; i += 256) { const int r = i / KPADC, cc = CH + i % KPADC; *(u32x4*)(sK + r * KPITCH + cc * 16) = u32x4{0, 0, 0, 0}; }
   TB_TS(41);
   u32x4 kreg[LD_IT], vreg[LD_IT];
@@ -557,7 +601,7 @@
       if (idx < NCHUNK) { *(u32x4*)(sK + r * KPITCH + cc * 16) = kreg[it]; *(u32x4*)(sV + r * VPITCH + cc * 16) = vreg[it]; }
     }
   };
-  kv_load(4 * hhalf);
+  if constexpr (!FRAG) kv_load(4 * hhalf);
   TB_TS(42);
 
   const int rbase = 16 * MI * mh + px;
@@ -578,7 +622,7 @@
   if (tid < C / 2) *(f32x4*)(gbs + 4 * tid) = gbv;
   __syncthreads();
   TB_TS(3);
-  kv_store();
+  if constexpr (!FRAG) kv_store();
   if constexpr (!PRE) {
     panel_row_stats<C, BM>(panel, lnst, tid, p.ln_eps);
     __syncthreads();
@@ -666,6 +710,29 @@
   TB_TS(7);
   gemm_body(p.wqf);
   TB_TS(8);
+  constexpr int NH = FRAG ? QBN : 4, NKF = KB * KSTEPS, NVF = 2 * KB * DBLK;
+  constexpr bool VWITHK = NH == 1 || D == 40;
+  const int hfirst = FRAG ? QBN * (wid / QBN) : 4 * hhalf;
+  u32x4 kfr[FRAG ? NKF : 1], vfr[FRAG ? NVF : 1];
+  auto kf_load = [&](int h) __attribute__((always_inline)) {
+    if constexpr (FRAG) {
+      const auto rs = __builtin_amdgcn_make_buffer_rsrc((void*)(p.kf + (long long)b * (H * NKF * 512)), 0, H * NKF * 1024, 0x00020000);
+      __builtin_amdgcn_sched_barrier(0);
+#pragma unroll
+      for (int f = 0; f < NKF; ++f) kfr[f] = __builtin_bit_cast(u32x4, __builtin_amdgcn_raw_buffer_load_b128(rs, lane16, (unsigned)(h * NKF + f) * 1024u, 0));
+      __builtin_amdgcn_sched_barrier(0);
+    }
+  };
+  auto vf_load = [&](int h) __attribute__((always_inline)) {
+    if constexpr (FRAG) {
+      const auto rs = __builtin_amdgcn_make_buffer_rsrc((void*)(p.vf + (long long)b * (H * NVF * 512)), 0, H * NVF * 1024, 0x00020000);
+      __builtin_amdgcn_sched_barrier(0);
+#pragma unroll
+      for (int f = 0; f < NVF; ++f) vfr[f] = __builtin_bit_cast(u32x4, __builtin_amdgcn_raw_buffer_load_b128(rs, lane16, (unsigned)(h * NVF + f) * 1024u, 0));
+      __builtin_amdgcn_sched_barrier(0);
+    }
+  };
+  if constexpr (MI == 2) { kf_load(hfirst); vf_load(hfirst); }
   __syncthreads();
 #pragma unroll
   for (int i = 0; i < MI; ++i) {
@@ -677,6 +744,7 @@
       *(u32x2*)(panel + row * PITCH + panel_swz<C>(n >> 3, row) * 16 + (n & 7) * 2) = pk;
     }
   }
+  if constexpr (MI != 2) { kf_load(hfirst); if constexpr (VWITHK) vf_load(hfirst); }
   __syncthreads();
   TB_TS(9);
 
@@ -714,9 +782,10 @@
                                                 voff0 + (unsigned)(kb * 32 + (i & 3) + 8 * (i >> 2)) * rowb, 0, 0);
     };
 
-    for (int hi = 0; hi < 4; ++hi) {
-      const int h = 4 * hhalf + hi;
-      if (hi + 1 < 4) kv_load(h + 1);
+#pragma unroll 1
+    for (int hi = 0; hi < NH; ++hi) {
+      const int h = hfirst + hi;
+      if constexpr (!FRAG) { if (hi + 1 < 4) kv_load(h + 1); }
       if (attn_wave) {
       bf16x8 qf[KSTEPS];
 #pragma unroll
@@ -731,11 +800,14 @@
       for (int kb = 0; kb < KB; ++kb)
 #pragma unroll
         for (int s = 0; s < KSTEPS; ++s) {
-          const bf16x8 a = *(const bf16x8*)(sK + (kb * 32 + c) * KPITCH + (2 * s + hh) * 16);
+          bf16x8 a;
+          if constexpr (FRAG) a = __builtin_bit_cast(bf16x8, kfr[kb * KSTEPS + s]);
+          else a = *(const bf16x8*)(sK + (kb * 32 + c) * KPITCH + (2 * s + hh) * 16);
           if (s == 0) { const f32x16 z = {0.f, 0.f, 0.f, 0.f, 0.f, 0.f, 0.f, 0.f, 0.f, 0.f, 0.f, 0.f, 0.f, 0.f, 0.f, 0.f};
                         sacc[kb] = __builtin_amdgcn_mfma_f32_32x32x16_bf16(a, qf[s], z, 0, 0, 0); }
           else sacc[kb] = __builtin_amdgcn_mfma_f32_32x32x16_bf16(a, qf[s], sacc[kb], 0, 0, 0);
         }
+      if constexpr (FRAG && !VWITHK) vf_load(h);
 #pragma unroll
       for (int kb = 0; kb < KB; ++kb)
 #pragma unroll
@@ -776,6 +848,10 @@
           const char* vb = sV + (kb * 32 + 16 * s + tr_row) * VPITCH + tr_col * 2;
 #pragma unroll
           for (int db = 0; db < DBLK; ++db) {
+            if constexpr (FRAG) {
+              oacc[db] = __builtin_amdgcn_mfma_f32_32x32x16_bf16(__builtin_bit_cast(bf16x8, vfr[(kb * 2 + s) * DBLK + db]), pf, oacc[db], 0, 0, 0);
+              continue;
+            }
             const s16x4 lo = __builtin_amdgcn_ds_read_tr16_b64_v4i16((__attribute__((address_space(3))) s16x4*)(vb + db * 64));
             const s16x4 hi2 = __builtin_amdgcn_ds_read_tr16_b64_v4i16((__attribute__((address_space(3))) s16x4*)(vb + 8 * VPITCH + db * 64));
             const u32x2 l2 = __builtin_bit_cast(u32x2, lo), h2 = __builtin_bit_cast(u32x2, hi2);
@@ -783,6 +859,7 @@
             oacc[db] = __builtin_amdgcn_mfma_f32_32x32x16_bf16(__builtin_bit_cast(bf16x8, a4), pf, oacc[db], 0, 0, 0);
           }
         }
+      if constexpr (FRAG && NH > 1) { const int hn = hi + 1 < NH ? h + 1 : h; kf_load(hn); if constexpr (VWITHK) vf_load(hn); }
 #pragma unroll
       for (int db = 0; db < DBLK; ++db)
 #pragma unroll
@@ -804,9 +881,11 @@
       }
       }
       TB_TS(10 + hi);
+      if constexpr (!FRAG) {
       __syncthreads();
       if (hi + 1 < 4) { kv_store(); __syncthreads(); }
       TB_TS(20 + hi);
+      }
     }
     gemm_head(p.wof);
     if (p.record && hpb == H) {
@@ -903,13 +982,19 @@
   const bool pre = p.o1 != nullptr;
   if (pre && (!p.wo1f || !p.bo1 || p.out == p.h)) { agd_set_error("attn_chain: the to_out prologue needs its weights and out != h"); return -1; }
   if (p.src_rows > 0 && (p.src_rows % BM || p.M % p.src_rows || p.out == p.h)) { agd_set_error("attn_chain: src_rows %d must divide M, be a multiple of %d and out != h", p.src_rows, BM); return -1; }
-  const void* kfn = C == 320 ? (pre ? (const void*)attn_chain_kernel<320, 1> : (const void*)attn_chain_kernel<320, 0>)
-                    : r32    ? (pre ? (const void*)attn_chain_kernel<640, 1, 2> : (const void*)attn_chain_kernel<640, 0, 2>)
-                             : (pre ? (const void*)attn_chain_kernel<640, 1> : (const void*)attn_chain_kernel<640, 0>);
-  static std::atomic<bool> attr[AGD_MAX_DEVICES][6] = {};
+  if ((p.kf != nullptr) != (p.vf != nullptr)) { agd_set_error("attn_chain: K and V fragments come together"); return -1; }
+  const int nh = BM / 32;
+  const bool frag = p.kf && (!p.record || p.rec_hpb <= nh || (p.rec_hpb == 8 && nh == 4));
+  const void* kfn = !frag ? (C == 320 ? (pre ? (const void*)attn_chain_kernel<320, 1> : (const void*)attn_chain_kernel<320, 0>)
+                             : r32    ? (pre ? (const void*)attn_chain_kernel<640, 1, 2> : (const void*)attn_chain_kernel<640, 0, 2>)
+                                      : (pre ? (const void*)attn_chain_kernel<640, 1> : (const void*)attn_chain_kernel<640, 0>))
+                          : (C == 320 ? (pre ? (const void*)attn_chain_kernel<320, 1, 4, 1> : (const void*)attn_chain_kernel<320, 0, 4, 1>)
+                             : r32    ? (pre ? (const void*)attn_chain_kernel<640, 1, 2, 1> : (const void*)attn_chain_kernel<640, 0, 2, 1>)
+                                      : (pre ? (const void*)attn_chain_kernel<640, 1, 4, 1> : (const void*)attn_chain_kernel<640, 0, 4, 1>));
+  static std::atomic<bool> attr[AGD_MAX_DEVICES][12] = {};
   int dev = 0; HIP_CHECK_RET(hipGetDevice(&dev));
   if (dev < 0 || dev >= AGD_MAX_DEVICES) { agd_set_error("attn_chain: device ordinal %d out of range", dev); return -1; }
-  const int slot = (C == 640 ? (r32 ? 4 : 2) : 0) + (pre ? 1 : 0);
+  const int slot = (C == 640 ? (r32 ? 4 : 2) : 0) + (pre ? 1 : 0) + (frag ? 6 : 0);
   if (!attr[dev][slot]) { HIP_CHECK_RET(hipFuncSetAttribute(kfn, hipFuncAttributeMaxDynamicSharedMemorySize, lds)); attr[dev][slot] = true; }
   AttnChainP pp = p;
   void* args[] = {&pp};
diff --git a/agenda_amd/ops.py b/agenda_amd/ops.py
--- a/agenda_amd/ops.py
+++ b/agenda_amd/ops.py
@@ -216,7 +216,7 @@
     return y.reshape(x.shape)
 
 
-def attn_chain(x, gamma, beta, wq, kv, wo, bo, heads=8, eps=1e-5, return_probs=False, rows32=False):
+def attn_chain(x, gamma, beta, wq, kv, wo, bo, heads=8, eps=1e-5, return_probs=False, rows32=False, frags=False):
     lib = _lib.load()
     x, kv = _f32c(x), _f32c(kv)
     B, HW, Cc = x.shape
@@ -224,7 +224,7 @@
     y = torch.empty_like(x)
     pr = torch.empty(B, T, HW, device=x.device, dtype=torch.float32) if return_probs else None
     _lib.check(lib.agd_op_attn_chain(_lib.ptr(x), _lib.ptr(_f32c(gamma)), _lib.ptr(_f32c(beta)), _lib.ptr(_f32c(wq)), _lib.ptr(kv), _lib.ptr(_f32c(wo)),
-                                     _lib.ptr(_f32c(bo)), _lib.ptr(y), _lib.ptr(pr), B, HW, T, Cc, heads | (256 if rows32 else 0), float(eps), _lib.current_stream_ptr()),
+                                     _lib.ptr(_f32c(bo)), _lib.ptr(y), _lib.ptr(pr), B, HW, T, Cc, heads | (256 if rows32 else 0) | (512 if frags else 0), float(eps), _lib.current_stream_ptr()),
                None, "agd_op_attn_chain")
     return (y, pr) if return_probs else y
 
@@ -264,7 +264,7 @@
 
 
 def attn_chain_ex(x, gamma, beta, wq, kv, wo, bo, heads=8, eps=1e-5, *, hw=None, o1=None, wo1=None, bo1=None, src_rows=0, rowstat=False, rec=None,
-                  rec_hpb=8, rec_b0=0, rec_T=None, rows32=False, inplace=False):
+                  rec_hpb=8, rec_b0=0, rec_T=None, rows32=False, inplace=False, frags=False):
     lib = _lib.load()
     x, kv = _f32c(x), _f32c(kv)
     Cc = x.shape[-1]
@@ -294,9 +294,21 @@
     _lib.check(lib.agd_op_attn_chain_ex(_lib.ptr(x), _lib.ptr(_f32c(gamma)), _lib.ptr(_f32c(beta)), _lib.ptr(_f32c(wq)), _lib.ptr(_given(kv)), _lib.ptr(_f32c(wo)),
                                         _lib.ptr(_f32c(bo)), _lib.ptr(out["y"]), B, HW, T, Cc, int(heads), float(eps), _lib.ptr(o1),
                                         _lib.ptr(_f32c(wo1) if pre else None), _lib.ptr(_f32c(bo1) if pre else None), _lib.ptr(out.get("h1")), int(src_rows),
-                                        _lib.ptr(out.get("rowstat")), _lib.ptr(rec), int(rec_hpb), int(rec_b0), int(rec_T or 0), int(rec_rows), int(bool(rows32)),
+                                        _lib.ptr(out.get("rowstat")), _lib.ptr(rec), int(rec_hpb), int(rec_b0), int(rec_T or 0), int(rec_rows), int(bool(rows32)) | (2 if frags else 0),
                                         int(bool(inplace)), _lib.current_stream_ptr()), None, "agd_op_attn_chain_ex")
     return out
+
+
+def kv_fragments(kv, C):
+    lib = _lib.load()
+    kv = _f32c(kv)
+    B, T = kv.shape[:2]
+    d = C // 8
+    ksteps, dblk = (d + 15) // 16, (d + 31) // 32
+    kf = torch.full((B, 8, 3 * ksteps, 64, 8), float("nan"), device=kv.device, dtype=torch.float32)
+    vf = torch.full((B, 8, 6 * dblk, 64, 8), float("nan"), device=kv.device, dtype=torch.float32)
+    _lib.check(lib.agd_op_kv_fragments(_lib.ptr(kv), B, T, int(C), _lib.ptr(kf), _lib.ptr(vf), _lib.current_stream_ptr()), None, "agd_op_kv_fragments")
+    return kf, vf
 
 
 def qkv_chain(x, hw, gn_gamma, gn_beta, groups, part, bm, w_in, b_in, gamma, beta, wqkv, *, gn_eps=1e-6, ln_eps=1e-5, inside=False, rows64=False, sched2=False):
diff --git a/include/agenda_hip.h b/include/agenda_hip.h
--- a/include/agenda_hip.h
+++ b/include/agenda_hip.h
@@ -204,6 +204,7 @@
                          const float* bo, float* y, int B, int HW, int T, int C, int heads, float eps, const float* o1, const float* wo1,
                          const float* bo1, float* h1, int src_rows, float* rowstat, float* rec, int rec_hpb, int rec_b0, int rec_T,
                          int rec_rows, int rows32, int inplace, void* stream);
+int agd_op_kv_fragments(const float* kv, int B, int T, int C, float* kf, float* vf, void* stream);
 int agd_op_qkv_chain(const float* x, const float* gn_gamma, const float* gn_beta, int groups, float gn_eps, const float* part, int bm,
                      const float* w_in, const float* b_in, const float* gamma, const float* beta, float ln_eps, const float* wqkv, float* h,
                      float* qkv, int M, int HW, int C, int flags, void* stream);
```

Measured after the change: 9.175, median of 6. No clear change (+0.7%).
